# multimodallearning/convexAdam

Hardware: AMD Instinct MI355X
Metric: volume-pairs/sec (160x192x224 MIND convex+Adam(80it)) (higher is better)
Workload: dtype f32

## Files before the change

### convexadam_amd/csrc/certify.hip

```cpp
#include <hip/hip_runtime.h>
#include <stdlib.h>

#include "cvx_common.h"

namespace cvx {

#define CERT_CLO ((float)((1.0 - 1.0 / 65536.0) / 729.0))
#define CERT_CHI ((float)((1.0 + 1.0 / 65536.0) / 729.0))
#define CERT_TINY 1.0e-40f
__device__ __forceinline__ float cert_lower(float s) { return fmaxf(__builtin_fmaf(s, CERT_CLO, -CERT_TINY), 0.0f); }
__device__ __forceinline__ float cert_upper(float s) { return __builtin_fmaf(s, CERT_CHI, fminf(s, CERT_TINY)); }

__device__ __forceinline__ unsigned ordered_bits(float v) {
    unsigned b = __float_as_uint(v);
    b = (b & 0x80000000u) ? ~b : (b | 0x80000000u);
    if (v != v) b = 0u;
    return b;
}
__device__ __forceinline__ float from_ordered_bits(unsigned b) { return __uint_as_float((b & 0x80000000u) ? (b & 0x7fffffffu) : ~b); }

struct CertRec { unsigned x, box; int kp; float bound, slo, uc, ub, ua; };

struct CertProb {
    const float* ssdu; const float* fix; const float* mov; const float* tail;
    unsigned long long* key; unsigned* sec;
    int* idx0; int* idxA; int* idxB;
    float* smin;
    unsigned* list; int* counts;
    unsigned long long* work; unsigned work_cap;
    struct CertRec* rec;
    float* u;
    int64_t* argmin_out;
};
struct CertGeo { int C, h, w, d, hw, n, K, ntail; long long tail_from; };
struct CertArgs { CertProb p[2]; CertGeo g; const float* mesh; float coef; int pass; };

template <bool WAVE>
__device__ __forceinline__ void cert_sync() {
    if (WAVE) { __builtin_amdgcn_fence(__ATOMIC_RELEASE, "wavefront"); __builtin_amdgcn_s_waitcnt(0xC07F); __builtin_amdgcn_wave_barrier(); __builtin_amdgcn_fence(__ATOMIC_ACQUIRE, "wavefront"); }
    else __syncthreads();
}
template <bool WAVE>
__device__ float cert_exact_entry_t(const CertGeo& G, const CertProb& P, int k, int xlin, float* sm, int lane) {
    const int n = G.n, nn = n * n, h = G.h, w = G.w, d = G.d, hw = G.hw;
    const int iH = k % n, iW = (k / n) % n, iD = k / nn;
    const int x = xlin % d, y = (xlin / d) % w, z = xlin / (d * w);
    const size_t v = (size_t)h * w * d;
    for (int t = lane; t < 125; t += 64) {
        const int a = t / 25 - 2, b = (t / 5) % 5 - 2, c = t % 5 - 2;
        const int pz = z + a, py = y + b, px = x + c;
        float val = 0.0f;
        if (pz >= 0 && pz < h && py >= 0 && py < w && px >= 0 && px < d) {
            const long long flat = (((long long)pz * nn + iW * n + iD) * w + py) * d + px;
            if (G.ntail > 0 && flat >= G.tail_from) val = P.tail[iH * 32 + (int)(flat - G.tail_from)];
            else {
                const int mz = pz + iH - hw, my = py + iW - hw, mx = px + iD - hw;
                const bool inb = mz >= 0 && mz < h && my >= 0 && my < w && mx >= 0 && mx < d;
                const float* fp = P.fix + ((size_t)pz * w + py) * d + px;
                const float* mp = P.mov + ((size_t)(inb ? mz : 0) * w + (inb ? my : 0)) * d + (inb ? mx : 0);
                float a0 = 0.0f, a1 = 0.0f;
                for (int c0 = 0; c0 < G.C; c0 += 16) {
                    float fv[16], mv[16];
#pragma unroll
                    for (int i = 0; i < 16; ++i) {
                        const bool on = c0 + i < G.C;
                        fv[i] = on ? fp[(size_t)(c0 + i) * v] : 0.0f;
                        mv[i] = (on && inb) ? mp[(size_t)(c0 + i) * v] : 0.0f;
                    }
#pragma unroll
                    for (int i = 0; i < 16; ++i) {
                        if (c0 + i < G.C) {
                            const float df = fv[i] - mv[i];
                            a0 += df * df;
                        }
                    }
                    if (c0 + 16 <= G.C) { a1 += a0; a0 = 0.0f; }
                }
                val = G.C >= 16 ? a0 + a1 : a0;
            }
        }
        sm[t] = val;
    }
    cert_sync<WAVE>();
    if (lane < 27) {
        const int a = lane / 9 - 1, b = (lane / 3) % 3 - 1, c = lane % 3 - 1;
        const int pz = z + a, py = y + b, px = x + c;
        float s = 0.0f;
        const bool in = pz >= 0 && pz < h && py >= 0 && py < w && px >= 0 && px < d;
        if (in) {
            for (int aa = -1; aa <= 1; ++aa)
                for (int bb = -1; bb <= 1; ++bb)
                    for (int cc = -1; cc <= 1; ++cc) {
                        const int qz = pz + aa, qy = py + bb, qx = px + cc;
                        if (qz >= 0 && qz < h && qy >= 0 && qy < w && qx >= 0 && qx < d) s += sm[((a + aa + 2) * 5 + (b + bb + 2)) * 5 + (c + cc + 2)];
                    }
            s = div_exact<27>(s);
        }
        sm[128 + lane] = in ? s : -1.0f;
    }
    cert_sync<WAVE>();
    float s = 0.0f;
    for (int t = 0; t < 27; ++t) {
        const float b = sm[128 + t];
        if (b >= 0.0f || b != b) s += b;
    }
    cert_sync<WAVE>();
    return div_exact<27>(s);
}

__device__ float cert_exact_entry(const CertGeo& G, const CertProb& P, int k, int xlin, float* sm, int lane) { return cert_exact_entry_t<false>(G, P, k, xlin, sm, lane); }
__device__ float cert_exact_entry_wave(const CertGeo& G, const CertProb& P, int k, int xlin, float* sm, int lane) { return cert_exact_entry_t<true>(G, P, k, xlin, sm, lane); }

__global__ __launch_bounds__(256) void k_cert_plain_stream(CertArgs A, int kslice, int vec4) {
    const CertProb& P = A.p[blockIdx.z];
    const size_t v = (size_t)A.g.h * A.g.w * A.g.d;
    const int K = A.g.K;
    const size_t x0 = ((size_t)blockIdx.x * blockDim.x + threadIdx.x) * 4;
    const int k0 = blockIdx.y * kslice, k1 = min(k0 + kslice, K);
    if (x0 >= v) return;
    const int nv = (int)min((size_t)4, v - x0);
    const float INF = __uint_as_float(0x7f800000u);
    float best[4], second[4];
    int bi[4];
    bool tiny[4] = {false, false, false, false};
    const float* p = P.ssdu + (size_t)k0 * v + x0;
    auto load4 = [&](const float* q, float (&c4)[4]) {
        if (vec4) { const float4 t = *reinterpret_cast<const float4*>(q); c4[0] = t.x; c4[1] = t.y; c4[2] = t.z; c4[3] = t.w; }
        else {
#pragma unroll
            for (int j = 0; j < 4; ++j) c4[j] = j < nv ? q[j] : 0.0f;
        }
    };
    {
        float c4[4];
        load4(p, c4);
#pragma unroll
        for (int j = 0; j < 4; ++j) { best[j] = c4[j]; bi[j] = k0; second[j] = INF; tiny[j] = (c4[j] > 0.0f) & (c4[j] < 1.0e-36f); }
        p += v;
    }
#pragma unroll 8
    for (int k = k0 + 1; k < k1; ++k, p += v) {
        float c4[4];
        load4(p, c4);
#pragma unroll
        for (int j = 0; j < 4; ++j) {
            const float c = c4[j];
            tiny[j] = tiny[j] | ((c > 0.0f) & (c < 1.0e-36f));
            const bool lt = argmin_better(c, best[j]);
            second[j] = fminf(second[j], lt ? best[j] : c);
            best[j] = lt ? c : best[j];
            bi[j] = lt ? k : bi[j];
        }
    }
#pragma unroll
    for (int j = 0; j < 4; ++j) {
        if (j >= nv) continue;
        const unsigned long long mine = pack_min_key(best[j], (unsigned)bi[j]);
        const unsigned long long old = atomicMin(&P.key[x0 + j], mine);
        unsigned cand = second[j] == INF ? 0xffffffffu : ordered_bits(second[j]);
        if (old != ~0ull) {
            const unsigned loser = (unsigned)((old < mine ? mine : old) >> 32);
            cand = loser < cand ? loser : cand;
        }
        if (tiny[j]) cand = 0u;
        if (cand != 0xffffffffu) atomicMin(&P.sec[x0 + j], cand);
    }
}

__global__ __launch_bounds__(256) void k_cert_plain_finalize(CertArgs A) {
    const CertProb& P = A.p[blockIdx.y];
    const size_t v = (size_t)A.g.h * A.g.w * A.g.d;
    const size_t x = (size_t)blockIdx.x * blockDim.x + threadIdx.x;
    if (x >= v) return;
    const unsigned long long key = P.key[x];
    const unsigned b1 = (unsigned)(key >> 32), b2 = P.sec[x];
    const int k1 = (int)(unsigned)(key & 0xffffffffull);
    const float s1 = b1 == 0u ? __uint_as_float(0x7fc00000u) : from_ordered_bits(b1);
    P.smin[x] = s1;
    P.idx0[x] = k1;
    if (P.argmin_out) P.argmin_out[x] = k1;
    bool certain = b1 == 0u || b2 == 0xffffffffu;
    if (!certain && b2 != 0u) certain = s1 == 0.0f || cert_lower(from_ordered_bits(b2)) > cert_upper(s1);
    if (!certain) P.list[atomicAdd(&P.counts[0], 1)] = (unsigned)x;
}

__global__ __launch_bounds__(64) void k_cert_plain_resolve(CertArgs A) {
    __shared__ float sm[160];
    const CertProb& P = A.p[blockIdx.y];
    const size_t v = (size_t)A.g.h * A.g.w * A.g.d;
    const int K = A.g.K, lane = threadIdx.x;
    const int cnt = P.counts[0];
    for (int e = blockIdx.x; e < cnt; e += gridDim.x) {
        const unsigned x = P.list[e];
        const float* col = P.ssdu + x;
        const float U = cert_upper(P.smin[x]);
        unsigned long long bestkey = ~0ull;
        for (int kb = 0; kb < K; kb += 1024) {
            float s[16];
#pragma unroll
            for (int i = 0; i < 16; ++i) { const int k = kb + 64 * i + lane; s[i] = k < K ? col[(size_t)k * v] : __uint_as_float(0x7f800000u); }
#pragma unroll
            for (int i = 0; i < 16; ++i) {
                const unsigned long long mz = __ballot(s[i] == 0.0f);
                if (mz) {
                    const unsigned long long key = pack_min_key(0.0f, (unsigned)(kb + 64 * i + __ffsll((long long)mz) - 1));
                    bestkey = key < bestkey ? key : bestkey;
                }
                const bool mine = s[i] != 0.0f && cert_lower(s[i]) <= U;
                const unsigned long long m = __ballot(mine);
                if (m) {
                    const int nm = __popcll(m);
                    int base = 0;
                    if (lane == 0) base = atomicAdd(&P.counts[8], nm);
                    base = __shfl(base, 0);
                    const int slot = base + __popcll(m & ((1ull << lane) - 1ull));
                    if (mine && (unsigned)slot < P.work_cap) P.work[slot] = ((unsigned long long)x << 32) | (unsigned)(kb + 64 * i + lane);
                    unsigned long long rest = __ballot(mine && (unsigned)slot >= P.work_cap);
                    while (rest) {
                        const int l = __ffsll((long long)rest) - 1;
                        rest &= rest - 1;
                        const int kk = kb + 64 * i + l;
                        const float ex = cert_exact_entry(A.g, P, kk, (int)x, sm, lane);
                        const unsigned long long key = pack_min_key(ex, (unsigned)kk);
                        bestkey = key < bestkey ? key : bestkey;
                    }
                }
            }
        }
        if (lane == 0) P.key[x] = bestkey;
    }
}
__global__ __launch_bounds__(256) void k_cert_plain_eval(CertArgs A) {
    __shared__ float smem[4][160];
    const CertProb& P = A.p[blockIdx.y];
    const int lane = threadIdx.x & 63, wv = threadIdx.x >> 6;
    const int n = min(P.counts[8], (int)P.work_cap);
    for (int e = blockIdx.x * 4 + wv; e < n; e += gridDim.x * 4) {
        const unsigned long long it = P.work[e];
        const unsigned x = (unsigned)(it >> 32);
        const int kk = (int)(unsigned)(it & 0xffffffffull);
        const float ex = cert_exact_entry_wave(A.g, P, kk, (int)x, smem[wv], lane);
        if (lane == 0) atomicMin(&P.key[x], pack_min_key(ex, (unsigned)kk));
    }
}
__global__ __launch_bounds__(256) void k_cert_plain_commit(CertArgs A) {
    const CertProb& P = A.p[blockIdx.y];
    const int cnt = P.counts[0];
    for (int e = blockIdx.x * blockDim.x + threadIdx.x; e < cnt; e += gridDim.x * blockDim.x) {
        const unsigned x = P.list[e];
        const int kw = (int)(unsigned)(P.key[x] & 0xffffffffull);
        P.idx0[x] = kw;
        if (P.argmin_out) P.argmin_out[x] = kw;
    }
}

struct CertMesh {
    const float* ax;
    int n; float rn;
    __device__ __forceinline__ void split(int k, int& ic, int& ib, int& ia) const {
        const int q = (int)(((float)k + 0.5f) * rn);
        ic = k - q * n;
        ia = (int)(((float)q + 0.5f) * rn);
        ib = q - ia * n;
    }
};
__device__ __forceinline__ CertMesh cert_mesh_load(float* lds96, const float* __restrict__ mesh, int K, int n) {
    const int t = threadIdx.x;
    if (t < n) { lds96[t] = mesh[t]; lds96[32 + t] = mesh[K + t * n]; lds96[64 + t] = mesh[2 * K + t * n * n]; }
    __syncthreads();
    return CertMesh{lds96, n, 1.0f / (float)n};
}

__device__ __forceinline__ void cert_smooth_winner(const int* __restrict__ idx, const CertMesh& M, int h, int w, int d, size_t i,
                                                   float& o0, float& o1, float& o2) {
    const int x = (int)(i % d), y = (int)((i / d) % w), z = (int)(i / ((size_t)d * w));
    float s0 = 0.f, s1 = 0.f, s2 = 0.f;
#pragma unroll
    for (int a = -1; a <= 1; ++a) {
        const int za = z + a;
        const bool zok = za >= 0 && za < h;
        const int zc = zok ? za : z;
        int kk[9];
        bool ok[9];
#pragma unroll
        for (int b = -1; b <= 1; ++b)
#pragma unroll
            for (int c = -1; c <= 1; ++c) {
                const int yb = y + b, xc = x + c;
                const bool in = zok && yb >= 0 && yb < w && xc >= 0 && xc < d;
                const int t = (b + 1) * 3 + (c + 1);
                ok[t] = in;
                kk[t] = idx[((size_t)zc * w + (in ? yb : y)) * d + (in ? xc : x)];
            }
        float m0[9], m1[9], m2[9];
#pragma unroll
        for (int t = 0; t < 9; ++t) {
            int ic, ib, ia;
            M.split(kk[t], ic, ib, ia);
            m0[t] = M.ax[ic]; m1[t] = M.ax[32 + ib]; m2[t] = M.ax[64 + ia];
        }
#pragma unroll
        for (int t = 0; t < 9; ++t) {
            s0 += ok[t] ? m0[t] : 0.0f;
            s1 += ok[t] ? m1[t] : 0.0f;
            s2 += ok[t] ? m2[t] : 0.0f;
        }
    }
    o0 = fdiv(s0, 27.0f);
    o1 = fdiv(s1, 27.0f);
    o2 = fdiv(s2, 27.0f);
}

__device__ __forceinline__ float cert_pen(const CertMesh& M, int k, float uc, float ub, float ua, float coef) {
    int ic, ib, ia;
    M.split(k, ic, ib, ia);
    const float e0 = M.ax[ic] - uc, e1 = M.ax[32 + ib] - ub, e2 = M.ax[64 + ia] - ua;
    float q = e0 * e0;
    q += e1 * e1;
    q += e2 * e2;
    return coef * q;
}

struct CertBox {
    float uc, ub, ua, slo, bound;
    int c_lo, c_hi, b_lo, b_hi, a_lo, a_hi;
    long long vol;
    bool degenerate;
};
__device__ __forceinline__ CertBox cert_box(const CertMesh& M, float uc, float ub, float ua, float coef, int K, int n, int kp,
                                            float ssdu_kp, float smin_u, const float* __restrict__ col, size_t v, int refine_above) {
    CertBox c;
    c.uc = uc; c.ub = ub; c.ua = ua;
    c.slo = cert_lower(smin_u);
    c.bound = cert_upper(ssdu_kp) + cert_pen(M, kp, uc, ub, ua, coef);
    const float hwf = (float)((n - 1) / 2);
    auto close_box = [&]() {
        const float qmax = fdiv((c.bound - c.slo) + fabsf(c.bound) * 2.384185791015625e-07f, coef) * 1.00001f;
        const float R = fsqrt(fmaxf(qmax, 0.0f)) * 1.00001f + 1.0e-4f;
        c.c_lo = max((int)ceilf(c.uc - R + hwf), 0); c.c_hi = min((int)floorf(c.uc + R + hwf), n - 1);
        c.b_lo = max((int)ceilf(c.ub - R + hwf), 0); c.b_hi = min((int)floorf(c.ub + R + hwf), n - 1);
        c.a_lo = max((int)ceilf(c.ua - R + hwf), 0); c.a_hi = min((int)floorf(c.ua + R + hwf), n - 1);
        c.vol = (long long)max(c.c_hi - c.c_lo + 1, 0) * max(c.b_hi - c.b_lo + 1, 0) * max(c.a_hi - c.a_lo + 1, 0);
        c.degenerate = !(coef > 0.0f) || !(R == R) || c.vol <= 0;
    };
    close_box();
    if (!c.degenerate && c.vol > refine_above && uc == uc && ub == ub && ua == ua) {
        const int kn = (min(max((int)rintf(ua + hwf), 0), n - 1) * n + min(max((int)rintf(ub + hwf), 0), n - 1)) * n + min(max((int)rintf(uc + hwf), 0), n - 1);
        if (kn != kp) {
            const float near_hi = cert_upper(col[(size_t)kn * v]) + cert_pen(M, kn, uc, ub, ua, coef);
            if (near_hi < c.bound) { c.bound = near_hi; close_box(); }
        }
    }
    if (c.degenerate) { c.c_lo = c.b_lo = c.a_lo = 0; c.c_hi = c.b_hi = c.a_hi = n - 1; c.vol = (long long)n * n * n; }
    return c;
}

__global__ __launch_bounds__(64) void k_cert_voxel(CertArgs A, int refine) {
    const CertProb& P = A.p[blockIdx.y];
    const int h = A.g.h, w = A.g.w, d = A.g.d, K = A.g.K, n = A.g.n;
    const size_t v = (size_t)h * w * d;
    const size_t x = (size_t)blockIdx.x * blockDim.x + threadIdx.x;
    __shared__ float axes[96];
    const CertMesh M = cert_mesh_load(axes, A.mesh, K, n);
    if (x >= v) return;
    const int* prev = A.pass == 1 ? P.idx0 : ((A.pass & 1) ? P.idxB : P.idxA);
    int* next = (A.pass & 1) ? P.idxA : P.idxB;
    const int kp = prev[x];
    const float s_kp = P.ssdu[(size_t)kp * v + x];
    const float sm_x = P.smin[x];
    float uc, ub, ua;
    cert_smooth_winner(prev, M, h, w, d, x, uc, ub, ua);
    P.u[x] = uc; P.u[v + x] = ub; P.u[2 * v + x] = ua;
    if (sm_x != sm_x) { next[x] = P.idx0[x]; return; }
    const CertBox c = cert_box(M, uc, ub, ua, A.coef, K, n, kp, s_kp, sm_x, P.ssdu + x, v, refine);
    constexpr int NB = 8;
    const unsigned boxpack = (unsigned)c.c_lo | ((unsigned)c.c_hi << 5) | ((unsigned)c.b_lo << 10) | ((unsigned)c.b_hi << 15) | ((unsigned)c.a_lo << 20) | ((unsigned)c.a_hi << 25) | (c.degenerate ? 1u << 30 : 0u);
    const CertRec rec = {(unsigned)x, boxpack, kp, c.bound, c.slo, c.uc, c.ub, c.ua};
    if (c.vol > NB) { P.rec[atomicAdd(&P.counts[A.pass], 1)] = rec; return; }
    int kk[NB];
    float pen[NB], val[NB];
    bool need[NB];
    {
        int ic = c.c_lo, ib = c.b_lo, ia = c.a_lo;
#pragma unroll
        for (int j = 0; j < NB; ++j) {
            const bool in = j < (int)c.vol;
            kk[j] = (ia * n + ib) * n + ic;
            pen[j] = cert_pen(M, kk[j], c.uc, c.ub, c.ua, A.coef);
            need[j] = in && !(c.slo + pen[j] > c.bound);
            if (j + 1 < (int)c.vol) {
                if (++ic > c.c_hi) { ic = c.c_lo; if (++ib > c.b_hi) { ib = c.b_lo; ++ia; } }
            }
        }
    }
#pragma unroll
    for (int j = 0; j < NB; ++j) val[j] = need[j] ? P.ssdu[(size_t)kk[j] * v + x] : 0.0f;
    float lo1 = 0.f, lo2 = 0.f, U = __uint_as_float(0x7f800000u);
    int k1 = -1, cnt = 0;
#pragma unroll
    for (int j = 0; j < NB; ++j) {
        if (!need[j]) continue;
        const float lo = cert_lower(val[j]) + pen[j], hi = cert_upper(val[j]) + pen[j];
        U = fminf(U, hi);
        if (cnt == 0) { lo1 = lo; k1 = kk[j]; }
        else if (lo < lo1) { lo2 = lo1; lo1 = lo; k1 = kk[j]; }
        else if (cnt == 1 || lo < lo2) lo2 = lo;
        ++cnt;
    }
    if (cnt == 0) { next[x] = kp; return; }
    if (cnt == 1 || lo2 > U) { next[x] = k1; return; }
    P.rec[atomicAdd(&P.counts[A.pass], 1)] = rec;
}

__global__ __launch_bounds__(256) void k_cert_wave(CertArgs A) {
    __shared__ float smem[4][160];
    __shared__ float axes[96];
    const CertProb& P = A.p[blockIdx.y];
    const int h = A.g.h, w = A.g.w, d = A.g.d, K = A.g.K, n = A.g.n;
    const size_t v = (size_t)h * w * d;
    const int lane = threadIdx.x & 63, wv = threadIdx.x >> 6;
    float* sm = smem[wv];
    const CertMesh M = cert_mesh_load(axes, A.mesh, K, n);
    int* next = (A.pass & 1) ? P.idxA : P.idxB;
    const int cnt = P.counts[A.pass];
    const float INF = __uint_as_float(0x7f800000u);
    for (int e = blockIdx.x * 4 + wv; e < cnt; e += gridDim.x * 4) {
        const CertRec r = P.rec[e];
        const size_t x = r.x;
        const int kp = r.kp;
        const float* col = P.ssdu + x;
        CertBox c;
        c.uc = r.uc; c.ub = r.ub; c.ua = r.ua; c.slo = r.slo; c.bound = r.bound;
        c.c_lo = r.box & 31; c.c_hi = (r.box >> 5) & 31; c.b_lo = (r.box >> 10) & 31; c.b_hi = (r.box >> 15) & 31; c.a_lo = (r.box >> 20) & 31; c.a_hi = (r.box >> 25) & 31;
        c.degenerate = ((r.box >> 30) & 1u) != 0;
        c.vol = (long long)(c.c_hi - c.c_lo + 1) * (c.b_hi - c.b_lo + 1) * (c.a_hi - c.a_lo + 1);
        const int nc = c.c_hi - c.c_lo + 1, nb = c.b_hi - c.b_lo + 1, ncb = nc * nb;
        const float rc = 1.0f / (float)nc, rab = 1.0f / (float)ncb;
        unsigned long long key = ~0ull;
        float lo2 = INF, U = INF;
        constexpr int NL = 12;
        for (long long i0 = 0; i0 < c.vol; i0 += 64 * NL) {
            int kk[NL];
            float pen[NL], val[NL];
            bool need[NL];
#pragma unroll
            for (int j = 0; j < NL; ++j) {
                need[j] = false; kk[j] = 0; pen[j] = 0.0f;
                if (i0 + 64 * j < c.vol) {
                    const int i = (int)i0 + lane + 64 * j;
                    need[j] = i < (int)c.vol;
                    const int ii = need[j] ? i : 0;
                    const int qa = (int)(((float)ii + 0.5f) * rab), ra = ii - qa * ncb;
                    const int qb = (int)(((float)ra + 0.5f) * rc);
                    const int ic = c.c_lo + ra - qb * nc, ib = c.b_lo + qb, ia = c.a_lo + qa;
                    kk[j] = (ia * n + ib) * n + ic;
                    pen[j] = cert_pen(M, kk[j], c.uc, c.ub, c.ua, A.coef);
                    need[j] = need[j] && (c.degenerate || !(c.slo + pen[j] > c.bound));
                }
            }
#pragma unroll
            for (int j = 0; j < NL; ++j) val[j] = need[j] ? col[(size_t)kk[j] * v] : 0.0f;
#pragma unroll
            for (int j = 0; j < NL; ++j) {
                if (!need[j]) continue;
                const float lo = cert_lower(val[j]) + pen[j], hi = cert_upper(val[j]) + pen[j];
                U = fminf(U, hi);
                const unsigned long long kx = pack_min_key(lo, (unsigned)kk[j]);
                if (kx < key) { if (key != ~0ull) lo2 = fminf(lo2, from_ordered_bits((unsigned)(key >> 32))); key = kx; }
                else lo2 = fminf(lo2, lo);
            }
        }
        unsigned long long gkey = key;
        for (int o = 32; o > 0; o >>= 1) { const unsigned long long t = __shfl_xor(gkey, o); gkey = t < gkey ? t : gkey; }
        float mine2 = key == gkey ? lo2 : fminf(lo2, key != ~0ull ? from_ordered_bits((unsigned)(key >> 32)) : INF);
        for (int o = 32; o > 0; o >>= 1) { mine2 = fminf(mine2, __shfl_xor(mine2, o)); U = fminf(U, __shfl_xor(U, o)); }
        if (gkey == ~0ull) { if (lane == 0) next[x] = kp; continue; }
        if (mine2 > U) { if (lane == 0) next[x] = (int)(unsigned)(gkey & 0xffffffffull); continue; }
        if (lane == 0) atomicAdd(&P.counts[7], 1);
        unsigned long long bestkey = ~0ull;
        for (long long i0 = 0; i0 < c.vol; i0 += 64 * NL) {
            int kk[NL];
            float pen[NL], val[NL];
            bool need[NL];
#pragma unroll
            for (int j = 0; j < NL; ++j) {
                need[j] = false; kk[j] = 0; pen[j] = 0.0f;
                if (i0 + 64 * j < c.vol) {
                    const int i = (int)i0 + lane + 64 * j;
                    need[j] = i < (int)c.vol;
                    const int ii = need[j] ? i : 0;
                    const int qa = (int)(((float)ii + 0.5f) * rab), ra = ii - qa * ncb;
                    const int qb = (int)(((float)ra + 0.5f) * rc);
                    kk[j] = ((c.a_lo + qa) * n + c.b_lo + qb) * n + c.c_lo + ra - qb * nc;
                    pen[j] = cert_pen(M, kk[j], c.uc, c.ub, c.ua, A.coef);
                    need[j] = need[j] && (c.degenerate || !(c.slo + pen[j] > c.bound));
                }
            }
#pragma unroll
            for (int j = 0; j < NL; ++j) val[j] = need[j] ? col[(size_t)kk[j] * v] : 0.0f;
#pragma unroll
            for (int j = 0; j < NL; ++j) {
                if (!(i0 + 64 * j < c.vol)) continue;
                unsigned long long m = __ballot(need[j] && cert_lower(val[j]) + pen[j] <= U);
                while (m) {
                    const int l = __ffsll((long long)m) - 1;
                    m &= m - 1;
                    const int k2 = __shfl(kk[j], l);
                    const float sk = __shfl(val[j], l), pk = __shfl(pen[j], l);
                    const float ex = sk == 0.0f ? 0.0f : cert_exact_entry_wave(A.g, P, k2, (int)x, sm, lane);
                    const unsigned long long kx = pack_min_key(ex + pk, (unsigned)k2);
                    bestkey = kx < bestkey ? kx : bestkey;
                }
            }
        }
        if (lane == 0) next[x] = (int)(unsigned)(bestkey & 0xffffffffull);
    }
}

__global__ __launch_bounds__(256) void k_cert_gather(CertArgs A) {
    const CertProb& P = A.p[blockIdx.y];
    const size_t v = (size_t)A.g.h * A.g.w * A.g.d;
    const size_t i = (size_t)blockIdx.x * blockDim.x + threadIdx.x;
    __shared__ float axes[96];
    const CertMesh M = cert_mesh_load(axes, A.mesh, A.g.K, A.g.n);
    if (i >= v) return;
    const int* prev = A.pass == 1 ? P.idx0 : ((A.pass & 1) ? P.idxB : P.idxA);
    float o0, o1, o2;
    cert_smooth_winner(prev, M, A.g.h, A.g.w, A.g.d, i, o0, o1, o2);
    P.u[i] = o0; P.u[v + i] = o1; P.u[2 * v + i] = o2;
}

__global__ __launch_bounds__(256) void k_cert_arm(CertArgs A, int nprob) {
    const size_t v = (size_t)A.g.h * A.g.w * A.g.d;
    const size_t i = (size_t)blockIdx.x * blockDim.x + threadIdx.x;
    for (int q = 0; q < nprob; ++q) {
        if (i < v) { A.p[q].key[i] = ~0ull; A.p[q].sec[i] = 0xffffffffu; }
        if (i < 16) A.p[q].counts[i] = 0;
    }
}

void launch_corr_tail_compact(const float* fix, const float* mov, int C, int h, int w, int d, int hw, int sad, float* tail, hipStream_t s);

static size_t cert_work_cap(size_t v) { return 4 * v + 65536; }
struct CertCarve { unsigned long long* key; unsigned* sec; int* idx0; int* idxA; int* idxB; float* smin; unsigned* list; CertRec* rec; int* counts; float* tail; unsigned long long* work; unsigned work_cap; };
static CertCarve cert_layout(Carver& cv, int h, int w, int d, int hw, bool plain) {
    const size_t v = (size_t)h * w * d;
    const int n = 2 * hw + 1;
    CertCarve c{};
    c.key = cv.take<unsigned long long>(v);
    c.sec = cv.take<unsigned>(v);
    c.idx0 = cv.take<int>(v);
    c.smin = cv.take<float>(v);
    c.list = cv.take<unsigned>(v);
    c.counts = cv.take<int>(16);
    c.work_cap = (unsigned)cert_work_cap(v);
    c.work = cv.take<unsigned long long>(c.work_cap);
    c.tail = cv.take<float>((size_t)32 * n);
    if (!plain) {
        c.idxA = cv.take<int>(v); c.idxB = cv.take<int>(v);
        c.rec = cv.take<CertRec>(v);
    }
    return c;
}
size_t corr_certify_workspace_bytes(int, int h, int w, int d, int hw, bool plain) { Carver m; cert_layout(m, h, w, d, hw, plain); return ws_query(m); }
static CertGeo cert_geo(int C, int h, int w, int d, int hw) {
    CertGeo g;
    g.C = C; g.h = h; g.w = w; g.d = d; g.hw = hw; g.n = 2 * hw + 1; g.K = g.n * g.n * g.n;
    const long long ncols = (long long)h * g.n * g.n * w * d;
    g.tail_from = (ncols / 32) * 32;
    g.ntail = (int)(ncols - g.tail_from);
    return g;
}
static CertProb cert_prob(const float* ssdu, const float* fix, const float* mov, const CertCarve& c, float* u, int64_t* argmin_out) {
    return CertProb{ssdu, fix, mov, c.tail, c.key, c.sec, c.idx0, c.idxA, c.idxB, c.smin, c.list, c.counts, c.work, c.work_cap, c.rec, u, argmin_out};
}

static void cert_arm(CertArgs& A, int nprob, hipStream_t s) {
    const CertGeo& g = A.g;
    const size_t v = (size_t)g.h * g.w * g.d;
    hipLaunchKernelGGL(k_cert_arm, dim3((unsigned)cdiv64((int64_t)(v > 16 ? v : 16), 256)), dim3(256), 0, s, A, nprob);
    for (int q = 0; q < nprob; ++q)
        if (g.ntail > 0) launch_corr_tail_compact(A.p[q].fix, A.p[q].mov, g.C, g.h, g.w, g.d, g.hw, 0, const_cast<float*>(A.p[q].tail), s);
}
static void cert_stream(CertArgs A, int q0, int nq, hipStream_t s) {
    const CertGeo& g = A.g;
    const size_t v = (size_t)g.h * g.w * g.d;
    const int K = g.K;
    if (q0) { A.p[0] = A.p[q0]; }
    bool vec4 = v % 4 == 0;
    for (int q = 0; q < nq; ++q) vec4 = vec4 && (reinterpret_cast<uintptr_t>(A.p[q].ssdu) & 15) == 0;
    const int xb = (int)cdiv64((int64_t)cdiv64((int64_t)v, 4), 256);
    int nslices = cdiv(512, xb);
    if (nslices > K) nslices = K;
    if (nslices < 1) nslices = 1;
    const int kslice = cdiv(K, nslices);
    nslices = cdiv(K, kslice);
    hipLaunchKernelGGL(k_cert_plain_stream, dim3(xb, nslices, nq), dim3(256), 0, s, A, kslice, vec4 ? 1 : 0);
}
static int cert_finish(CertArgs& A, int nprob, hipStream_t s) {
    const size_t v = (size_t)A.g.h * A.g.w * A.g.d;
    hipLaunchKernelGGL(k_cert_plain_finalize, dim3((unsigned)cdiv64((int64_t)v, 256), nprob), dim3(256), 0, s, A);
    hipLaunchKernelGGL(k_cert_plain_resolve, dim3(256, nprob), dim3(64), 0, s, A);
    hipLaunchKernelGGL(k_cert_plain_eval, dim3(256, nprob), dim3(256), 0, s, A);
    hipLaunchKernelGGL(k_cert_plain_commit, dim3(8, nprob), dim3(256), 0, s, A);
    return check_last("certified argmin");
}
static int cert_plain(CertArgs& A, int nprob, bool arm, hipStream_t s) {
    if (arm) cert_arm(A, nprob, s);
    cert_stream(A, 0, nprob, s);
    return cert_finish(A, nprob, s);
}

int corr_certified_argmin(const float* ssdu, const float* fix, const float* mov, int C, int h, int w, int d, int hw, int64_t* argmin,
                          void* workspace, size_t workspace_bytes, hipStream_t s) {
    if (workspace_bytes < corr_certify_workspace_bytes(C, h, w, d, hw, true)) return fail(CVX_ERR_WORKSPACE, "certified argmin: workspace too small");
    Carver cv(workspace);
    const CertCarve c = cert_layout(cv, h, w, d, hw, true);
    CertArgs A{};
    A.g = cert_geo(C, h, w, d, hw);
    A.p[0] = cert_prob(ssdu, fix, mov, c, nullptr, argmin);
    A.p[1] = A.p[0];
    return cert_plain(A, 1, true, s);
}

int coupled_convex_cert_impl(const float* ssduA, const float* fixA, const float* movA, float* outA, void* wsA, const float* ssduB, const float* fixB,
                             const float* movB, float* outB, void* wsB, const float* mesh, int C, int h, int w, int d, int hw, size_t workspace_bytes,
                             hipStream_t s, int stage) {
    if (workspace_bytes < corr_certify_workspace_bytes(C, h, w, d, hw, false)) return fail(CVX_ERR_WORKSPACE, "certified coupled convex: workspace too small");
    const int nprob = ssduB ? 2 : 1;
    CertArgs A{};
    A.g = cert_geo(C, h, w, d, hw);
    A.mesh = mesh;
    Carver cva(wsA), cvb(wsB);
    const CertCarve ca = cert_layout(cva, h, w, d, hw, false);
    A.p[0] = cert_prob(ssduA, fixA, movA, ca, outA, nullptr);
    A.p[1] = A.p[0];
    if (ssduB) { const CertCarve cb = cert_layout(cvb, h, w, d, hw, false); A.p[1] = cert_prob(ssduB, fixB, movB, cb, outB, nullptr); }
    if (stage == 1) { cert_arm(A, nprob, s); return check_last("certified argmin"); }
    if (stage == 2) { cert_stream(A, 0, 1, s); return check_last("certified argmin"); }
    if (stage == 3) { if (nprob > 1) cert_stream(A, 1, 1, s); return check_last("certified argmin"); }
    if (stage == 4) return cert_finish(A, nprob, s);
    if (stage == 0) { const int rc = cert_plain(A, nprob, true, s); if (rc) return rc; }
    const size_t v = (size_t)h * w * d;
    const int refine = options().prune_refine != 0 ? 8 : 0x7fffffff;
    static const float coeffs[6] = {0.003f, 0.01f, 0.03f, 0.1f, 0.3f, 1.0f};
    for (int it = 0; it < 6; ++it) {
        A.coef = coeffs[it]; A.pass = it + 1;
        hipLaunchKernelGGL(k_cert_voxel, dim3((unsigned)cdiv64((int64_t)v, 64), nprob), dim3(64), 0, s, A, refine);
        hipLaunchKernelGGL(k_cert_wave, dim3(512, nprob), dim3(256), 0, s, A);
    }
    if (getenv("CVX_CERT_TRACE")) {
        for (int q = 0; q < nprob; ++q) {
            int cnt[8];
            (void)hipStreamSynchronize(s);
            (void)hipMemcpy(cnt, A.p[q].counts, sizeof(cnt), hipMemcpyDeviceToHost);
            fprintf(stderr, "cert trace: problem %d: plain flagged %d; listed per coupled pass %d %d %d %d %d %d, %d of them evaluated exactly (of %zu voxels)\n", q, cnt[0], cnt[1], cnt[2], cnt[3], cnt[4], cnt[5], cnt[6], cnt[7], v);
        }
    }
    A.pass = 7;
    hipLaunchKernelGGL(k_cert_gather, dim3((unsigned)cdiv64((int64_t)v, 256), nprob), dim3(256), 0, s, A);
    return check_last("certified coupled convex");
}

}
```

### convexadam_amd/csrc/correlate.hip

```cpp

#include <algorithm>

#include "cvx_common.h"

namespace cvx {

struct CorrGeom {
    int C, h, w, d, hw, n;
    int px;
    int PL;
    int dq;
    int hq, wq;
    int mpad;
};
static CorrGeom corr_geom(int C, int h, int w, int d, int hw) {
    CorrGeom g;
    g.C = C; g.h = h; g.w = w; g.d = d; g.hw = hw; g.n = 2 * hw + 1;
    g.px = (d + 3 + 3) / 4 * 4;
    g.PL = (hw + 3) / 4 * 4;
    g.dq = g.px + 2 * g.PL;
    g.hq = h + 2 * hw; g.wq = w + 2 * hw;
    g.mpad = 0;
    return g;
}

__global__ __launch_bounds__(256) void k_corr_prep(const float* __restrict__ fix, const float* __restrict__ mov, CorrGeom g,
                                                   float* __restrict__ Fp, float* __restrict__ Mp) {
    const size_t nF = (size_t)g.C * g.h * g.w * g.px, nM = (size_t)g.C * g.hq * g.wq * g.dq;
    const size_t i = (size_t)blockIdx.x * blockDim.x + threadIdx.x;
    if (i < nF) {
        const int x = (int)(i % g.px) - 1;
        const size_t r = i / g.px;
        Fp[i] = (x >= 0 && x < g.d) ? fix[r * g.d + x] : 0.0f;
    }
    if (i < nM) {
        const int xq = (int)(i % g.dq), yq = (int)((i / g.dq) % g.wq), zq = (int)((i / ((size_t)g.dq * g.wq)) % g.hq);
        const int c = (int)(i / ((size_t)g.dq * g.wq * g.hq));
        const int x = xq - g.PL - 1, y = yq - g.hw, z = zq - g.hw;
        const bool in = x >= 0 && x < g.d && y >= 0 && y < g.w && z >= 0 && z < g.h;
        Mp[i] = in ? mov[(((size_t)c * g.h + z) * g.w + y) * g.d + x] : 0.0f;
    } else if (i < nM + (size_t)g.mpad) Mp[i] = 0.0f;
}

template <int HW, bool CASCADE, bool FAST = false>
__global__ __launch_bounds__(256) void k_corr_raw(const float* __restrict__ Fp, const float* __restrict__ Mp, CorrGeom g,
                                                  float* __restrict__ raw) {
    static_assert(!(CASCADE && FAST), "the fast arithmetic has no cascade");
    constexpr int N = 2 * HW + 1;
    constexpr int PL = (HW + 3) / 4 * 4;
    constexpr int NCH = (2 * PL + 4) / 4;
    const int runs_per_row = g.px / 4;
    const int nruns = g.h * g.w * runs_per_row;
    const int r = blockIdx.x * blockDim.x + threadIdx.x;
    if (r >= nruns) return;
    const int i0 = 4 * (r % runs_per_row), y = (r / runs_per_row) % g.w, z = r / (runs_per_row * g.w);
    const int iH = blockIdx.y % N, iW = blockIdx.y / N;

    float acc[N][4];
    float acc1[CASCADE ? N : 1][4];
#pragma unroll
    for (int k = 0; k < N; ++k)
#pragma unroll
        for (int j = 0; j < 4; ++j) acc[k][j] = 0.0f;
    if (CASCADE) {
#pragma unroll
        for (int k = 0; k < N; ++k)
#pragma unroll
            for (int j = 0; j < 4; ++j) acc1[k][j] = 0.0f;
    }
    const size_t fstride = (size_t)g.h * g.w * g.px, mstride = (size_t)g.hq * g.wq * g.dq;
    const float* fp = Fp + ((size_t)z * g.w + y) * g.px + i0;
    const float* mp = Mp + ((size_t)(z + iH) * g.wq + (y + iW)) * g.dq + i0;

    float4 fq[2];
    float4 mq[2][NCH];
    fq[0] = *reinterpret_cast<const float4*>(fp);
#pragma unroll
    for (int q = 0; q < NCH; ++q) mq[0][q] = *reinterpret_cast<const float4*>(mp + 4 * q);
    auto consume = [&](const float4& f4, const float4 (&mv)[NCH], int c) {
        const float f[4] = {f4.x, f4.y, f4.z, f4.w};
        float m[4 * NCH];
#pragma unroll
        for (int q = 0; q < NCH; ++q) { m[4 * q] = mv[q].x; m[4 * q + 1] = mv[q].y; m[4 * q + 2] = mv[q].z; m[4 * q + 3] = mv[q].w; }
#pragma unroll
        for (int k = 0; k < N; ++k)
#pragma unroll
            for (int j = 0; j < 4; ++j) {
                const float df = f[j] - m[PL + j + k - HW];
                if (FAST) acc[k][j] = __builtin_fmaf(df, df, acc[k][j]);
                else acc[k][j] += df * df;
            }
        if (CASCADE && ((c & 15) == 15)) {
#pragma unroll
            for (int k = 0; k < N; ++k)
#pragma unroll
                for (int j = 0; j < 4; ++j) { acc1[k][j] += acc[k][j]; acc[k][j] = 0.0f; }
        }
    };
#pragma unroll 1
    for (int c = 0; c < g.C; c += 2) {
        if (c + 1 < g.C) {
            fq[1] = *reinterpret_cast<const float4*>(fp + (size_t)(c + 1) * fstride);
#pragma unroll
            for (int q = 0; q < NCH; ++q) mq[1][q] = *reinterpret_cast<const float4*>(mp + (size_t)(c + 1) * mstride + 4 * q);
        }
        consume(fq[0], mq[0], c);
        if (c + 1 < g.C) {
            if (c + 2 < g.C) {
                fq[0] = *reinterpret_cast<const float4*>(fp + (size_t)(c + 2) * fstride);
#pragma unroll
                for (int q = 0; q < NCH; ++q) mq[0][q] = *reinterpret_cast<const float4*>(mp + (size_t)(c + 2) * mstride + 4 * q);
            }
            consume(fq[1], mq[1], c + 1);
        }
    }
    const size_t v = (size_t)g.h * g.w * g.px;
    bool inx[4];
#pragma unroll
    for (int j = 0; j < 4; ++j) inx[j] = (i0 + j >= 1) && (i0 + j <= g.d);
#pragma unroll
    for (int k = 0; k < N; ++k) {
        float o[4];
#pragma unroll
        for (int j = 0; j < 4; ++j) {
            const float s = CASCADE ? acc[k][j] + acc1[k][j] : acc[k][j];
            o[j] = inx[j] ? s : 0.0f;
        }
        const size_t kk = ((size_t)k * N + iW) * N + iH;
        *reinterpret_cast<float4*>(raw + kk * v + ((size_t)z * g.w + y) * g.px + i0) = make_float4(o[0], o[1], o[2], o[3]);
    }
}

__device__ float sum_cascade_strided(const float* v, int stride, int size) {
    float a0 = 0.f, a1 = 0.f;
    int i = 0;
    for (; i + 16 <= size; i += 16) {
        for (int j = 0; j < 16; ++j) a0 += v[(i + j) * stride];
        a1 += a0; a0 = 0.f;
    }
    for (; i < size; ++i) a0 += v[i * stride];
    return a0 + a1;
}
__global__ void k_corr_tail(const float* __restrict__ fix, const float* __restrict__ mov, CorrGeom g, int64_t tail_from,
                            int ntail, float* __restrict__ raw) {
    const int t = blockIdx.x * blockDim.x + threadIdx.x;
    if (t >= ntail * g.n) return;
    const int iH = t / ntail;
    const int64_t flat = tail_from + (t % ntail);
    const int x = (int)(flat % g.d), y = (int)((flat / g.d) % g.w);
    const int jj = (int)((flat / ((int64_t)g.d * g.w)) % (g.n * g.n)), z = (int)(flat / ((int64_t)g.d * g.w * g.n * g.n));
    const int iW = jj / g.n, iD = jj % g.n;
    const int mz = z + iH - g.hw, my = y + iW - g.hw, mx = x + iD - g.hw;
    const bool inb = mz >= 0 && mz < g.h && my >= 0 && my < g.w && mx >= 0 && mx < g.d;
    const size_t v = (size_t)g.h * g.w * g.d;
    float sq[256];
    for (int c = 0; c < g.C; ++c) {
        const float f = fix[(size_t)c * v + ((size_t)z * g.w + y) * g.d + x];
        const float m = inb ? mov[(size_t)c * v + ((size_t)mz * g.w + my) * g.d + mx] : 0.0f;
        const float df = f - m;
        sq[c] = df * df;
    }
    const int n4 = g.C / 4;
    float p[4];
    for (int k = 0; k < 4; ++k) p[k] = sum_cascade_strided(sq + k, 4, n4);
    for (int i = n4 * 4; i < g.C; ++i) p[0] += sq[i];
    p[0] += p[1]; p[0] += p[2]; p[0] += p[3];
    const size_t kk = ((size_t)iD * g.n + iW) * g.n + iH;
    raw[kk * ((size_t)g.h * g.w * g.px) + ((size_t)z * g.w + y) * g.px + x + 1] = p[0];
}

__global__ void k_corr_tail_compact(const float* __restrict__ fix, const float* __restrict__ mov, CorrGeom g, int64_t tail_from,
                                    int ntail, int sad, float* __restrict__ tail) {
    const int t = blockIdx.x * blockDim.x + threadIdx.x;
    if (t >= ntail * g.n) return;
    const int iH = t / ntail;
    const int64_t flat = tail_from + (t % ntail);
    const int x = (int)(flat % g.d), y = (int)((flat / g.d) % g.w);
    const int jj = (int)((flat / ((int64_t)g.d * g.w)) % (g.n * g.n)), z = (int)(flat / ((int64_t)g.d * g.w * g.n * g.n));
    const int iW = jj / g.n, iD = jj % g.n;
    const int mz = z + iH - g.hw, my = y + iW - g.hw, mx = x + iD - g.hw;
    const bool inb = mz >= 0 && mz < g.h && my >= 0 && my < g.w && mx >= 0 && mx < g.d;
    const size_t v = (size_t)g.h * g.w * g.d;
    float sq[256];
    for (int c = 0; c < g.C; ++c) {
        const float f = fix[(size_t)c * v + ((size_t)z * g.w + y) * g.d + x];
        const float m = inb ? mov[(size_t)c * v + ((size_t)mz * g.w + my) * g.d + mx] : 0.0f;
        const float df = f - m;
        sq[c] = sad ? fabsf(df) : df * df;
    }
    const int n4 = g.C / 4;
    float p[4];
    for (int k = 0; k < 4; ++k) p[k] = sum_cascade_strided(sq + k, 4, n4);
    for (int i = n4 * 4; i < g.C; ++i) p[0] += sq[i];
    p[0] += p[1]; p[0] += p[2]; p[0] += p[3];
    tail[iH * 32 + (t % ntail)] = p[0];
}

void launch_corr_prep_generic(const float* fix, const float* mov, int C, int h, int w, int d, int hw, int px, int PL, int dq, float* Fp,
                              float* Mp, hipStream_t s) {
    CorrGeom g = corr_geom(C, h, w, d, hw);
    g.px = px; g.PL = PL; g.dq = dq; g.mpad = 8;
    const size_t nprep = std::max((size_t)C * g.hq * g.wq * g.dq + g.mpad, (size_t)C * h * w * g.px);
    hipLaunchKernelGGL(k_corr_prep, dim3((unsigned)cdiv64((int64_t)nprep, 256)), dim3(256), 0, s, fix, mov, g, Fp, Mp);
}

void launch_corr_tail_compact(const float* fix, const float* mov, int C, int h, int w, int d, int hw, int sad, float* tail, hipStream_t s) {
    const CorrGeom g = corr_geom(C, h, w, d, hw);
    const int64_t ncols = (int64_t)h * g.n * g.n * w * d, tail_from = (ncols / 32) * 32;
    const int ntail = (int)(ncols - tail_from);
    if (ntail > 0) hipLaunchKernelGGL(k_corr_tail_compact, dim3(cdiv(ntail * g.n, 64)), dim3(64), 0, s, fix, mov, g, tail_from, ntail, sad, tail);
}

template <int HW>
static void corr_raw_dispatch(const float* Fp, const float* Mp, const CorrGeom& g, float* raw, hipStream_t s, bool fast = false) {
    const int nruns = g.h * g.w * (g.px / 4);
    const dim3 grid(cdiv(nruns, 256), g.n * g.n);
    if (fast) hipLaunchKernelGGL((k_corr_raw<HW, false, true>), grid, dim3(256), 0, s, Fp, Mp, g, raw);
    else if (g.C >= 16) hipLaunchKernelGGL((k_corr_raw<HW, true>), grid, dim3(256), 0, s, Fp, Mp, g, raw);
    else hipLaunchKernelGGL((k_corr_raw<HW, false>), grid, dim3(256), 0, s, Fp, Mp, g, raw);
}

CorrPlan corr_plan(int C, int h, int w, int d, int hw, CorrUse use) {
    const Options& o = options();
    const CorrGeom g = corr_geom(C, h, w, d, hw);
    const double K = (double)g.n * g.n * g.n;
    const bool fused_ok = corr_fused_supported(C, h, w, d, hw), staged_ok = corr_cert_supported(C, h, w, d, hw);
    const bool round1_fits = hw <= 8 && corr_box2_supported(h, w, d, g.px) && (size_t)g.n * g.n * g.n * h * w * g.px * sizeof(float) <= ((size_t)2 << 30);
    const bool role_good = fused_ok && C <= 32 && corr_fused_items(C, h, w, d, hw) >= 384 && !corr_fused_tiled(C, h, w, d, hw);
    const bool role_ok = fused_ok && C <= 128;
    const bool unfused_ok = C >= 16 && C <= 128 && round1_fits && o.corr_cert != 2 && o.cert_unfused != 0 && (K * h * w * d * C >= 1e9 || o.cert_unfused == 2);

    CorrPlan p{};
    p.exact = (!fused_ok || (!use.variant && o.corr_fused_all == 0 && C >= 16 && round1_fits)) ? CorrKernel::Round1 : CorrKernel::Fused;
    p.cert = unfused_ok && !role_good                            ? CorrKernel::CertRound1
             : staged_ok && (o.corr_cert == 2 || !role_ok)       ? CorrKernel::CertStaged
             : role_ok                                           ? CorrKernel::CertRole
                                                                 : CorrKernel::None;
    p.cert_supported = staged_ok || role_ok || unfused_ok;
    p.fused_ws = fused_ok; p.staged_ws = staged_ok; p.cert_round1_ws = unfused_ok;
    p.pair_cert = o.corr_cert != 0 && !use.variant && !use.no_prune && p.cert_supported &&
                  (o.corr_cert == 2 || C < 16 || p.cert == CorrKernel::CertRound1 || role_good);
    p.pair_dual = use.ic && o.corr_dual != 0 && p.exact == CorrKernel::Fused;
    p.pair_dual_ws = use.ic && o.corr_dual != 0 && fused_ok;
    return p;
}

struct Round1Ws { float *Fp, *Mp, *raw; unsigned long long* keys; };
static Round1Ws round1_layout(Carver& cv, int C, int h, int w, int d, int hw, bool keys) {
    const CorrGeom g = corr_geom(C, h, w, d, hw);
    Round1Ws r{};
    r.Fp = cv.take<float>((size_t)C * h * w * g.px);
    r.Mp = cv.take<float>((size_t)C * g.hq * g.wq * g.dq);
    r.raw = cv.take<float>((size_t)g.n * g.n * g.n * h * w * g.px);
    if (keys) r.keys = cv.take<unsigned long long>((size_t)h * w * d);
    return r;
}
static int launch_round1(const float* fix, const float* mov, const CorrGeom& g, const Round1Ws& r, bool fast, float* ssd, hipStream_t s) {
    const size_t nprep = (size_t)g.C * g.hq * g.wq * g.dq;
    hipLaunchKernelGGL(k_corr_prep, dim3((unsigned)cdiv64((int64_t)nprep, 256)), dim3(256), 0, s, fix, mov, g, r.Fp, r.Mp);
    if (fast) corr_call_prep_hook(s);
    switch (g.hw) {
        case 0: corr_raw_dispatch<0>(r.Fp, r.Mp, g, r.raw, s, fast); break;
        case 1: corr_raw_dispatch<1>(r.Fp, r.Mp, g, r.raw, s, fast); break;
        case 2: corr_raw_dispatch<2>(r.Fp, r.Mp, g, r.raw, s, fast); break;
        case 3: corr_raw_dispatch<3>(r.Fp, r.Mp, g, r.raw, s, fast); break;
        case 4: corr_raw_dispatch<4>(r.Fp, r.Mp, g, r.raw, s, fast); break;
        case 5: corr_raw_dispatch<5>(r.Fp, r.Mp, g, r.raw, s, fast); break;
        case 6: corr_raw_dispatch<6>(r.Fp, r.Mp, g, r.raw, s, fast); break;
        case 7: corr_raw_dispatch<7>(r.Fp, r.Mp, g, r.raw, s, fast); break;
        default: corr_raw_dispatch<8>(r.Fp, r.Mp, g, r.raw, s, fast); break;
    }
    const int64_t ncols = (int64_t)g.h * g.n * g.n * g.w * g.d, tail_from = (ncols / 32) * 32;
    const int ntail = (int)(ncols - tail_from);
    if (!fast && ntail > 0)
        hipLaunchKernelGGL(k_corr_tail, dim3(cdiv(ntail * g.n, 64)), dim3(64), 0, s, fix, mov, g, tail_from, ntail, r.raw);
    return launch_corr_box2(r.raw, g.n * g.n * g.n, g.h, g.w, g.d, g.px, ssd, s, fast);
}

size_t corr_certfast_workspace_bytes(int C, int h, int w, int d, int hw) {
    const CorrPlan p = corr_plan(C, h, w, d, hw);
    Carver round1;
    if (p.cert_round1_ws) round1_layout(round1, C, h, w, d, hw, false);
    return std::max({p.staged_ws ? corr_cert_workspace_bytes(C, h, w, d, hw) : 0, p.fused_ws ? corr_fused_workspace_bytes(C, h, w, d, hw) : 0, ws_query(round1)});
}
int launch_corr_certfast(const float* fix, const float* mov, int C, int h, int w, int d, int hw, float* ssdu, void* workspace, size_t workspace_bytes,
                         hipStream_t s) {
    switch (corr_plan(C, h, w, d, hw).cert) {
        case CorrKernel::CertRound1: {
            Carver cv(workspace);
            const Round1Ws r = round1_layout(cv, C, h, w, d, hw, false);
            if (workspace_bytes < ws_query(cv)) return fail(CVX_ERR_WORKSPACE, "correlate (certified-fast, two kernels): workspace too small");
            return launch_round1(fix, mov, corr_geom(C, h, w, d, hw), r, true, ssdu, s);
        }
        case CorrKernel::CertStaged: return launch_corr_cert(fix, mov, C, h, w, d, hw, ssdu, workspace, workspace_bytes, s);
        default:
            return launch_corr_fused(fix, mov, C, h, w, d, hw, 0, 2, 2, 0, ssdu, workspace, workspace_bytes, s);
    }
}

}

using namespace cvx;

struct PartsWs { void* a; size_t a_bytes; void* b; size_t b_bytes; };
static PartsWs parts_layout(Carver& cv, size_t a_bytes, size_t b_bytes) {
    PartsWs p{nullptr, a_bytes, nullptr, b_bytes};
    p.a = cv.take<char>(a_bytes);
    p.b = cv.take<char>(b_bytes);
    return p;
}
static PartsWs fused_keys_layout(Carver& cv, int C, int h, int w, int d, int hw) {
    return parts_layout(cv, corr_fused_workspace_bytes(C, h, w, d, hw), sizeof(unsigned long long) * (size_t)h * w * d);
}
static PartsWs certified_layout(Carver& cv, int C, int h, int w, int d, int hw) {
    return parts_layout(cv, corr_certfast_workspace_bytes(C, h, w, d, hw), corr_certify_workspace_bytes(C, h, w, d, hw, true));
}
extern "C" size_t cvx_correlate_workspace_bytes(int C, int h, int w, int d, int disp_hw) {
    const CorrPlan p = corr_plan(C, h, w, d, disp_hw);
    Carver fused, round1, cert;
    if (p.fused_ws) fused_keys_layout(fused, C, h, w, d, disp_hw);
    if (p.exact == CorrKernel::Round1) round1_layout(round1, C, h, w, d, disp_hw, true);
    if (p.cert_supported) certified_layout(cert, C, h, w, d, disp_hw);
    return std::max({ws_query(fused), ws_query(round1), ws_query(cert)});
}

extern "C" int cvx_correlate_f32(const float* fix, const float* mov, int C, int h, int w, int d, int disp_hw, float* ssd,
                                 int64_t* argmin, void* workspace, size_t workspace_bytes, void* stream) {
    return cvx_correlate_ex_f32(fix, mov, C, h, w, d, disp_hw, nullptr, ssd, argmin, workspace, workspace_bytes, stream);
}

extern "C" int cvx_correlate_ex_f32(const float* fix, const float* mov, int C, int h, int w, int d, int disp_hw, const cvx_corr_opts* opts,
                                    float* ssd, int64_t* argmin, void* workspace, size_t workspace_bytes, void* stream) {
    const int cost = opts ? opts->cost : 0, n_box = opts ? opts->n_box : 2, fast = opts ? opts->fast : 0, f16 = opts ? opts->f16 : 0;
    CVX_REQUIRE((cost == 0 || cost == 1) && (n_box == 1 || n_box == 2) && (fast == 0 || fast == 1 || fast == 2) && f16 >= 0 && f16 <= 2, "cvx_correlate_ex_f32: bad options");
    CVX_REQUIRE(!(f16 && (cost != 0 || n_box != 2)), "cvx_correlate_ex_f32: fp16 storage exists for the SSD cost with two boxes only");
    CVX_REQUIRE(!(fast && (cost != 0 || n_box != 2)), "cvx_correlate_ex_f32: the fast mode exists for the SSD cost with two boxes only");
    CVX_REQUIRE(fix && mov && ssd && workspace, "cvx_correlate_f32: null pointer");
    CVX_REQUIRE(C > 0 && C < 256 && h > 0 && w > 0 && d > 0, "cvx_correlate_f32: bad extent C=%d %dx%dx%d", C, h, w, d);
    CVX_REQUIRE(disp_hw >= 0, "cvx_correlate_f32: negative disp_hw");
    if (disp_hw > CVX_MAX_DISP_HW) return fail(CVX_ERR_UNSUPPORTED, "cvx_correlate_f32: disp_hw %d > %d not built", disp_hw, CVX_MAX_DISP_HW);
    if (workspace_bytes < cvx_correlate_workspace_bytes(C, h, w, d, disp_hw))
        return fail(CVX_ERR_WORKSPACE, "cvx_correlate_f32: workspace too small");
    hipStream_t s = as_stream(stream);
    const CorrGeom g = corr_geom(C, h, w, d, disp_hw);
    const size_t K = (size_t)g.n * g.n * g.n;
    const bool variant = cost != 0 || n_box != 2 || fast || f16;
    const CorrPlan plan = corr_plan(C, h, w, d, disp_hw, CorrUse{variant, false, false});
    Carver cv(workspace);
    if (fast == 2) {
        if (f16) return fail(CVX_ERR_UNSUPPORTED, "cvx_correlate_ex_f32: the certified-fast volume is float32");
        if (!plan.cert_supported) return fail(CVX_ERR_UNSUPPORTED, "cvx_correlate_ex_f32: certified-fast correlation not built for this geometry");
        const PartsWs c = certified_layout(cv, C, h, w, d, disp_hw);
        int rc = launch_corr_certfast(fix, mov, C, h, w, d, disp_hw, ssd, c.a, c.a_bytes, s);
        if (rc || !argmin) return rc;
        return corr_certified_argmin(ssd, fix, mov, C, h, w, d, disp_hw, argmin, c.b, c.b_bytes, s);
    }
    if (plan.exact == CorrKernel::Fused) {
        const PartsWs f = fused_keys_layout(cv, C, h, w, d, disp_hw);
        int rc = launch_corr_fused(fix, mov, C, h, w, d, disp_hw, cost, n_box, fast, f16, ssd, f.a, f.a_bytes, s);
        if (rc) return rc;
        if (argmin)
            return launch_argmin(ssd, f16 == 2, nullptr, nullptr, 0.0f, false, (int)K, (size_t)h * w * d, static_cast<unsigned long long*>(f.b), argmin, s);
        return CVX_OK;
    }
    if (variant)
        return fail(CVX_ERR_UNSUPPORTED, "cvx_correlate_ex_f32: cost / n_box / fast / fp16 variants need the fused kernel (option corr_unfused is set, or the grid is outside its range: the fused kernel covers rows of d <= ~1270 voxels when the plane has w <= 320 / ceil((d + 6) / 4) rows, else (y tiles) d <= ~250)");
    if (disp_hw > 8) return fail(CVX_ERR_UNSUPPORTED, "cvx_correlate_f32: disp_hw %d > 8 needs the fused kernel (option corr_unfused is set, or the grid is outside its range: the fused kernel covers rows of d <= ~1270 voxels when the plane has w <= 320 / ceil((d + 6) / 4) rows, else (y tiles) d <= ~250)", disp_hw);
    if (!corr_box2_supported(h, w, d, g.px))
        return fail(CVX_ERR_UNSUPPORTED, "cvx_correlate_f32: coarse rows of %d voxels are too long for the LDS box kernel", d);
    const Round1Ws r = round1_layout(cv, C, h, w, d, disp_hw, true);
    int rc = launch_round1(fix, mov, g, r, false, ssd, s);
    if (rc) return rc;
    if (argmin) return launch_argmin(ssd, false, nullptr, nullptr, 0.0f, false, (int)K, (size_t)h * w * d, r.keys, argmin, s);
    return CVX_OK;
}
```

### convexadam_amd/csrc/cvx_common.h

```cpp
#pragma once
#include <hip/hip_runtime.h>
#include <stdint.h>
#include <stdio.h>
#include <stdarg.h>

#include <mutex>

#include "convexadam_hip.h"

namespace cvx {

void set_error(const char* fmt, ...);
int fail(int code, const char* fmt, ...);
int check_last(const char* what);

#define CVX_REQUIRE(cond, ...)                                      \
    do {                                                            \
        if (!(cond)) return ::cvx::fail(CVX_ERR_INVALID_ARG, __VA_ARGS__); \
    } while (0)

static inline hipStream_t as_stream(void* s) { return reinterpret_cast<hipStream_t>(s); }
static inline size_t align_up(size_t v, size_t a) { return (v + a - 1) / a * a; }
static inline int cdiv(int a, int b) { return (a + b - 1) / b; }
static inline int64_t cdiv64(int64_t a, int64_t b) { return (a + b - 1) / b; }

template <typename KernelT>
static inline void ensure_dynamic_lds(KernelT kernel, size_t bytes, size_t& granted) {
    static std::mutex mu;
    std::lock_guard<std::mutex> lock(mu);
    if (bytes > granted) {
        (void)hipFuncSetAttribute(reinterpret_cast<const void*>(kernel), hipFuncAttributeMaxDynamicSharedMemorySize, (int)bytes);
        (void)hipGetLastError();
        granted = bytes;
    }
}

struct Carver {
    char* base = nullptr;
    size_t used = 0;
    Carver() = default;
    explicit Carver(void* p) : base(static_cast<char*>(p)) {}
    size_t take_bytes(size_t bytes) { const size_t off = align_up(used, 256); used = off + bytes; return off; }
    template <typename T> T* take(size_t count) { const size_t off = take_bytes(count * sizeof(T)); return base ? reinterpret_cast<T*>(base + off) : nullptr; }
};
static inline size_t ws_query(const Carver& m) { return m.used ? m.used + 256 : 0; }

#define CVX_OPTIONS(X) \
    X(mind_tiled,          "CVX_MIND_TILED",            0)   \
    X(mind_overlap,        "CVX_MIND_OVERLAP",          0)   \
    X(mm_tx,               "CVX_MM_TX",                 0)   \
    X(mm_slots,            "CVX_MM_SLOTS",            512)   \
    X(box_tiled,           "CVX_BOX_TILED",             0)   \
    X(no_prune,            "CVX_NO_PRUNE",              0)   \
    X(corr_unfused,        "CVX_CORR_UNFUSED",          0)   \
    X(corr_fused_all,      "CVX_CORR_FUSED_ALL",        0)   \
    X(prune_stream_above,  "CVX_PRUNE_STREAM_ABOVE",   -1)   \
    X(cf_census,           "CVX_CF_CENSUS",             0)   \
    X(cf_prio,             "CVX_CF_PRIO",             136)   \
    X(warp_flat,           "CVX_WARP_FLAT",             0)   \
    X(box_yt,              "CVX_BOX_YT",                8)   \
    X(box_wg_target,       "CVX_BOX_WG_TARGET",         0)   \
    X(box_xsplit,          "CVX_BOX_XSPLIT",           -1)   \
    X(box_cpt,             "CVX_BOX_CPT",               4)   \
    X(box_uneven,          "CVX_BOX_UNEVEN",          200)   \
    X(box_adam_role,       "CVX_BOX_ADAM_ROLE",         0)   \
    X(box_dpp,             "CVX_BOX_DPP",               0)   \
    X(box_pk,              "CVX_BOX_PK",                0)   \
    X(box_prio,            "CVX_BOX_PRIO",              0)   \
    X(label_pow_block,     "CVX_LABEL_POW_BLOCK",      32)   \
    X(census_ptr,          nullptr,                     0)   \
    X(mind_mean_threads,   "CVX_MIND_MEAN_THREADS",     0)   \
    X(edt_sequential,      "CVX_EDT_SEQUENTIAL",        0)   \
    X(warp_octant,         "CVX_WARP_OCTANT",           4)   \
    X(box_fwd_tile,        "CVX_BOX_FWD_TILE",         -1)   \
    X(box_bwd_tile,        "CVX_BOX_BWD_TILE",         -1)   \
    X(box_walk,            "CVX_BOX_WALK",              1)   \
    X(corr_dual,           "CVX_CORR_DUAL",             0)   \
    X(prune_refine,        "CVX_PRUNE_REFINE",          1)   \
    X(mind_records,        "CVX_MIND_RECORDS",          1)   \
    X(resize_up2,          "CVX_RESIZE_UP2",            1)   \
    X(mind_blocked,        "CVX_MIND_BLOCKED",          1)   \
    X(corr_cert,           "CVX_CORR_CERT",             1)   \
    X(cc_debug,            "CVX_CC_DEBUG",              0)   \
    X(ic_fused,            "CVX_IC_FUSED",              0)   \
    X(mind_single,         "CVX_MIND_SINGLE",           0)   \
    X(ms_zlen,             "CVX_MS_ZLEN",               0)   \
    X(cf_map,              "CVX_CF_MAP",                1)   \
    X(cert_unfused,        "CVX_CERT_UNFUSED",          0)   \
    X(fbox_tile,           "CVX_FBOX_TILE",             0)   \
    X(box_tile_sync,       "CVX_BOX_TILE_SYNC",         0)   \
    X(box_prediv,          "CVX_BOX_PREDIV",            1)   \
    X(tile_census_ptr,     nullptr,                     0)   \
    X(adam_wt,             "CVX_ADAM_WT",               1)
#define X(name, env, dflt) long long name;
struct Options { CVX_OPTIONS(X) };
#undef X
Options& options();
const unsigned* adam_sqrt_table();
class ContextScope {
public:
    explicit ContextScope(const cvx_context* c);
    ~ContextScope();
    ContextScope(const ContextScope&) = delete;
    ContextScope& operator=(const ContextScope&) = delete;
private:
    void* prev_;
    bool active_;
};

#ifdef CVX_RACE_JITTER
__device__ __forceinline__ void cvx_jitter() {
    unsigned t = (unsigned)__builtin_amdgcn_s_memtime();
    t ^= (unsigned)__builtin_amdgcn_s_getreg((4 << 0) | (0 << 6) | (31 << 11)) * 2654435761u;
    t ^= t >> 13; t *= 0x9E3779B1u; t ^= t >> 15;
    const int n = (int)(t & 15);
    for (int i = 0; i < n; ++i) __builtin_amdgcn_s_sleep(1);
}
__device__ __forceinline__ void cvx_barrier() { cvx_jitter(); __syncthreads(); cvx_jitter(); }
#else
__device__ __forceinline__ void cvx_barrier() { __syncthreads(); }
#endif

__device__ __forceinline__ int clampi(int v, int lo, int hi) { return v < lo ? lo : (v > hi ? hi : v); }

__device__ __forceinline__ float fdiv(float a, float b) { return __fdiv_rn(a, b); }
__device__ __forceinline__ float fsqrt(float a) { return sqrtf(a); }

__device__ __forceinline__ float cvx_expf(float d) {
    const float R_LN2f = 1.442695040888963407359924681001892137426645954152985934135449406931f;
    const float L2Uf = 0.693145751953125f, L2Lf = 1.428606765330187045e-06f;
    const float qf = rintf(d * R_LN2f);
    const int q = (int)qf;
    float s = __builtin_fmaf(qf, -L2Uf, d);
    s = __builtin_fmaf(qf, -L2Lf, s);
    float u = 0.000198527617612853646278381f;
    u = __builtin_fmaf(u, s, 0.00139304355252534151077271f);
    u = __builtin_fmaf(u, s, 0.00833336077630519866943359f);
    u = __builtin_fmaf(u, s, 0.0416664853692054748535156f);
    u = __builtin_fmaf(u, s, 0.166666671633720397949219f);
    u = __builtin_fmaf(u, s, 0.5f);
    u = 1.0f + __builtin_fmaf(s * s, u, s);
    u = __builtin_ldexpf(u, q);
    if (d < -104.0f) u = 0.0f;
    if (d > 100.0f) u = __int_as_float(0x7f800000);
    return u;
}

struct ExpTable { const unsigned char* tbl; unsigned first, count; };
ExpTable mind_exp_table();

typedef float f32x4 __attribute__((ext_vector_type(4)));
typedef __attribute__((address_space(3))) f32x4 lds_f32x4;
__device__ __forceinline__ f32x4 lds_load4(const float* p) { return *(const volatile lds_f32x4*)p; }
__device__ __forceinline__ void lds_store4(float* p, f32x4 v) { *(volatile lds_f32x4*)p = v; }

typedef int i32x4 __attribute__((ext_vector_type(4)));
typedef unsigned u32x4 __attribute__((ext_vector_type(4)));
__device__ __forceinline__ float4 buffer_load16(__amdgpu_buffer_rsrc_t rsrc, unsigned lane_off, unsigned uni_off) {
    const i32x4 v = __builtin_bit_cast(i32x4, __builtin_amdgcn_raw_buffer_load_b128(rsrc, (int)lane_off, (int)uni_off, 0));
    return make_float4(__int_as_float(v.x), __int_as_float(v.y), __int_as_float(v.z), __int_as_float(v.w));
}

template <bool WT>
__device__ __forceinline__ void buffer_store16(__amdgpu_buffer_rsrc_t rsrc, unsigned lane_off, unsigned uni_off, float4 v) {
    __builtin_amdgcn_raw_buffer_store_b128(__builtin_bit_cast(u32x4, v), rsrc, (int)lane_off, (int)uni_off, WT ? 16 : 0);
}
template <bool WT>
__device__ __forceinline__ void buffer_store4(__amdgpu_buffer_rsrc_t rsrc, unsigned lane_off, unsigned uni_off, float v) {
    __builtin_amdgcn_raw_buffer_store_b32(__float_as_uint(v), rsrc, (int)lane_off, (int)uni_off, WT ? 16 : 0);
}
__device__ __forceinline__ void global_store16_wt(float* p, float4 v) {
    asm volatile("global_store_dwordx4 %0, %1, off sc1\n\ts_nop 1" : : "v"(p), "v"(__builtin_bit_cast(f32x4, v)) : "memory");
}

typedef float f32x2 __attribute__((ext_vector_type(2)));
typedef __attribute__((address_space(3))) f32x2 lds_f32x2;
__device__ __forceinline__ f32x2 lds_load2(const float* p) { return *(const volatile lds_f32x2*)p; }
__device__ __forceinline__ void lds_store2(float* p, f32x2 v) { *(volatile lds_f32x2*)p = v; }

template <int D>
__device__ __forceinline__ float div_exact(float x) {
    static_assert(D == 8 || D == 27 || D == 64 || D == 125 || D == 343, "divisor not verified");
    constexpr float r = 1.0f / (float)D;
    const float q = x * r;
    const float e = __builtin_fmaf(-(float)D, q, x);
    return __builtin_fmaf(e, r, q);
}
template <int D>
__device__ __forceinline__ float div_exact_inf(float x) { return __builtin_isinf(x) ? x : div_exact<D>(x); }

struct ConstDiv { float d, r; int ok; };
constexpr float kConstDivLo = 0x1p-76f, kConstDivHi = 0x1p76f;
ConstDiv const_div_ieee(float d);
ConstDiv const_div_make(float d);
ConstDiv const_div(float d);
ConstDiv const_div_if_proven(float d);
bool const_div_enumerate(float d, float r);
void const_div_prove(const float* ds, int n, int budget);
__device__ __forceinline__ float div_const_seq(float x, const ConstDiv& cd) {
    const float q = x * cd.r;
    const float e = __builtin_fmaf(-cd.d, q, x);
    return __builtin_fmaf(e, cd.r, q);
}
__device__ __forceinline__ bool div_const_inside(float x) { const float a = __builtin_fabsf(x); return a >= kConstDivLo && a <= kConstDivHi; }
__device__ __forceinline__ bool div_const_inside_root(float x) { return x <= kConstDivHi; }
__device__ __forceinline__ bool wave_all(bool inside) { return __builtin_amdgcn_ballot_w64(!inside) == 0; }
__device__ __forceinline__ float div_const(float x, const ConstDiv& cd) {
    if (cd.ok && wave_all(div_const_inside(x))) return div_const_seq(x, cd);
    return fdiv(x, cd.d);
}

template <int N>
__device__ __forceinline__ float cascade_seq(const float (&v)[N]) {
    static_assert(N < 256, "two cascade levels");
    float a0 = 0.f, a1 = 0.f;
    int i = 0;
#pragma unroll
    for (; i + 16 <= N; i += 16) {
#pragma unroll
        for (int j = 0; j < 16; ++j) a0 += v[i + j];
        a1 += a0;
        a0 = 0.f;
    }
#pragma unroll
    for (; i < N; ++i) a0 += v[i];
    a0 += a1;
    return a0;
}
template <int N>
__device__ __forceinline__ float outer_sum_ilp(const float (&v)[N]) {
    static_assert(N / 4 < 16, "single cascade level inside the interleaved sums");
    float p[4] = {0.f, 0.f, 0.f, 0.f};
#pragma unroll
    for (int i = 0; i < N / 4; ++i)
#pragma unroll
        for (int k = 0; k < 4; ++k) p[k] += v[4 * i + k];
#pragma unroll
    for (int i = (N / 4) * 4; i < N; ++i) p[0] += v[i];
    p[0] += p[1];
    p[0] += p[2];
    p[0] += p[3];
    return p[0];
}

__device__ __forceinline__ unsigned long long pack_min_key(float v, unsigned idx) {
    unsigned b = __float_as_uint(v);
    b = (b & 0x80000000u) ? ~b : (b | 0x80000000u);
    if (v != v) b = 0u;
    return ((unsigned long long)b << 32) | idx;
}

struct Tri {
    float ix, iy, iz;
    int x0, y0, z0;
    float tnw, tne, tsw, tse, bnw, bne, bsw, bse;
};
__device__ __forceinline__ float unnormalize(float g, int S) { return ((g + 1.0f) * (float)S - 1.0f) * 0.5f; }
__device__ __forceinline__ void tri_setup(Tri& t, float gx, float gy, float gz, int h, int w, int d) {
    t.ix = unnormalize(gx, d);
    t.iy = unnormalize(gy, w);
    t.iz = unnormalize(gz, h);
    const float fx = floorf(t.ix), fy = floorf(t.iy), fz = floorf(t.iz);
    t.x0 = (int)fmaxf(fminf(fx, 1.0e9f), -1.0e9f);
    t.y0 = (int)fmaxf(fminf(fy, 1.0e9f), -1.0e9f);
    t.z0 = (int)fmaxf(fminf(fz, 1.0e9f), -1.0e9f);
    const float x1 = (float)(t.x0 + 1), y1 = (float)(t.y0 + 1), z1 = (float)(t.z0 + 1);
    const float x0f = (float)t.x0, y0f = (float)t.y0, z0f = (float)t.z0;
    t.tnw = (x1 - t.ix) * (y1 - t.iy) * (z1 - t.iz);
    t.tne = (t.ix - x0f) * (y1 - t.iy) * (z1 - t.iz);
    t.tsw = (x1 - t.ix) * (t.iy - y0f) * (z1 - t.iz);
    t.tse = (t.ix - x0f) * (t.iy - y0f) * (z1 - t.iz);
    t.bnw = (x1 - t.ix) * (y1 - t.iy) * (t.iz - z0f);
    t.bne = (t.ix - x0f) * (y1 - t.iy) * (t.iz - z0f);
    t.bsw = (x1 - t.ix) * (t.iy - y0f) * (t.iz - z0f);
    t.bse = (t.ix - x0f) * (t.iy - y0f) * (t.iz - z0f);
}
__device__ __forceinline__ bool inb3(int z, int y, int x, int h, int w, int d) {
    return z >= 0 && z < h && y >= 0 && y < w && x >= 0 && x < d;
}
__device__ __forceinline__ float tri_sample(const Tri& t, const float* __restrict__ vol, int h, int w, int d) {
    const int x0 = t.x0, y0 = t.y0, z0 = t.z0, x1 = x0 + 1, y1 = y0 + 1, z1 = z0 + 1;
    const bool zi0 = (unsigned)z0 < (unsigned)h, zi1 = (unsigned)z1 < (unsigned)h, yi0 = (unsigned)y0 < (unsigned)w,
               yi1 = (unsigned)y1 < (unsigned)w, xi0 = (unsigned)x0 < (unsigned)d, xi1 = (unsigned)x1 < (unsigned)d;
    const int zc0 = clampi(z0, 0, h - 1), zc1 = clampi(z1, 0, h - 1), yc0 = clampi(y0, 0, w - 1), yc1 = clampi(y1, 0, w - 1),
              xc0 = clampi(x0, 0, d - 1), xc1 = clampi(x1, 0, d - 1);
    const size_t r00 = ((size_t)zc0 * w + yc0) * d, r01 = ((size_t)zc0 * w + yc1) * d, r10 = ((size_t)zc1 * w + yc0) * d,
                 r11 = ((size_t)zc1 * w + yc1) * d;
    const float v0 = vol[r00 + xc0], v1 = vol[r00 + xc1], v2 = vol[r01 + xc0], v3 = vol[r01 + xc1], v4 = vol[r10 + xc0],
                v5 = vol[r10 + xc1], v6 = vol[r11 + xc0], v7 = vol[r11 + xc1];
    float o = 0.0f, n;
    n = o + v0 * t.tnw; o = (zi0 && yi0 && xi0) ? n : o;
    n = o + v1 * t.tne; o = (zi0 && yi0 && xi1) ? n : o;
    n = o + v2 * t.tsw; o = (zi0 && yi1 && xi0) ? n : o;
    n = o + v3 * t.tse; o = (zi0 && yi1 && xi1) ? n : o;
    n = o + v4 * t.bnw; o = (zi1 && yi0 && xi0) ? n : o;
    n = o + v5 * t.bne; o = (zi1 && yi0 && xi1) ? n : o;
    n = o + v6 * t.bsw; o = (zi1 && yi1 && xi0) ? n : o;
    n = o + v7 * t.bse; o = (zi1 && yi1 && xi1) ? n : o;
    return o;
}

__device__ __forceinline__ void lin_coef(int o, int in, int out, int& i0, int& i1, float& l0, float& l1) {
    if (in == out) { i0 = o; i1 = o; l0 = 1.0f; l1 = 0.0f; return; }
    const float ratio = fdiv((float)in, (float)out);
    float src = __builtin_fmaf(ratio, (float)o + 0.5f, -0.5f);
    src = src < 0.0f ? 0.0f : src;
    int a = (int)floorf(src);
    a = a > in - 1 ? in - 1 : a;
    float l = src - (float)a;
    l = l < 0.f ? 0.f : (l > 1.f ? 1.f : l);
    i0 = a;
    i1 = a + ((a < in - 1) ? 1 : 0);
    l1 = l;
    l0 = 1.0f - l;
}
__device__ __forceinline__ float resize_chain(const float (&v)[8], float pre_mul, float lx0, float lx1, float ly0, float ly1, float lz0,
                                              float lz1) {
    const float a0 = __builtin_fmaf(v[0] * pre_mul, lx0, (v[1] * pre_mul) * lx1);
    const float a1 = __builtin_fmaf(v[2] * pre_mul, lx0, (v[3] * pre_mul) * lx1);
    const float b0 = __builtin_fmaf(v[4] * pre_mul, lx0, (v[5] * pre_mul) * lx1);
    const float b1 = __builtin_fmaf(v[6] * pre_mul, lx0, (v[7] * pre_mul) * lx1);
    const float l0 = __builtin_fmaf(a0, ly0, a1 * ly1);
    const float l1 = __builtin_fmaf(b0, ly0, b1 * ly1);
    return __builtin_fmaf(l0, lz0, l1 * lz1);
}

struct FastDiv { unsigned d, m; };
static inline FastDiv fastdiv_make(int d) { FastDiv f; f.d = (unsigned)d; f.m = d <= 1 ? 0u : (unsigned)((((unsigned long long)1 << 32) + (unsigned)d - 1) / (unsigned)d); return f; }
__device__ __forceinline__ int fastdiv(int n, FastDiv f) { return f.d <= 1 ? n : (int)__umulhi((unsigned)n, f.m); }

void profile_mark_kernel(const char* name, hipStream_t s);

int launch_box_zero(const float* in, float* out, int C, int H, int W, int D, int k, bool backward, hipStream_t s);
int launch_smoother(const float* in, float* out, float* tmp, int C, int H, int W, int D, const cvx_smoother& sm, bool backward,
                    hipStream_t s);
int launch_argmin_keys(const void* ssd, bool f16, int K, size_t v, unsigned long long* keys, bool arm, hipStream_t s);
struct CoupledWs { unsigned long long* keys[3]; int* idx; float* smin; unsigned long long* list; int* counts; };
CoupledWs coupled_layout(Carver& cv, int h, int w, int d, int disp_hw);
int launch_argmin(const void* ssd, bool f16, const float* mesh, const float* u, float coef, bool coupled, int K, size_t v,
                  unsigned long long* keys, int64_t* argmin_out, hipStream_t s);
int launch_resize(const float* in, int C, int h, int w, int d, float* out, int H, int W, int D, float pre_mul,
                  float post_div, hipStream_t s);
int launch_resize2(const float* in, int C, int h, int w, int d, int H, int W, int D, float* scratch, float* out, int h2, int w2,
                   int d2, float post_div, hipStream_t s);
struct AdamConsts { float w1, b2, omb2; ConstDiv bc2s; float neg_step; const unsigned* sqrt_tbl; };
__device__ __forceinline__ float adam_sqrt(float x, const unsigned* __restrict__ tbl) {
    float r = fsqrt(x);
    if (tbl) {
        const unsigned b = __float_as_uint(x), e = b >> 23, mant = b & 0x7fffffu;
        if (b != 0 && e < 255) {
            const unsigned key = e ? (((e & 1u) << 23) | mant) : ((1u << 24) | mant);
            const unsigned code = (tbl[key >> 4] >> ((key & 15u) * 2u)) & 3u;
            if (code) r = __uint_as_float(__float_as_uint(r) + (code == 1u ? 1u : 0xffffffffu));
        }
    }
    return r;
}
__device__ __forceinline__ bool argmin_better(float cost, float best) { return (cost < best) | ((cost != cost) & (best == best)); }
template <int N>
__device__ __forceinline__ void adam_update_n(const float (&g)[N], float (&P)[N], float (&m)[N], float (&v)[N], const AdamConsts& ac) {
    float root[N];
    bool inside = true;
#pragma unroll
    for (int j = 0; j < N; ++j) {
        m[j] = __builtin_fmaf(ac.w1, g[j] - m[j], m[j]);
        float vv = v[j] * ac.b2;
        vv = __builtin_fmaf(ac.omb2 * g[j], g[j], vv);
        v[j] = vv;
        root[j] = adam_sqrt(vv, ac.sqrt_tbl);
        inside &= div_const_inside_root(root[j]);
    }
    if (ac.bc2s.ok && wave_all(inside)) {
#pragma unroll
        for (int j = 0; j < N; ++j) root[j] = div_const_seq(root[j], ac.bc2s);
    } else {
#pragma unroll
        for (int j = 0; j < N; ++j) root[j] = fdiv(root[j], ac.bc2s.d);
    }
#pragma unroll
    for (int j = 0; j < N; ++j) {
        const float den = root[j] + 1e-8f;
        P[j] = P[j] + fdiv(ac.neg_step * m[j], den);
    }
}
__device__ __forceinline__ void adam_update(float g, float& P, float& m, float& v, const AdamConsts& ac) {
    const float g1[1] = {g};
    float P1[1] = {P}, m1[1] = {m}, v1[1] = {v};
    adam_update_n<1>(g1, P1, m1, v1, ac);
    P = P1[0]; m = m1[0]; v = v1[0];
}
struct AdamRun {
    const float *F2, *M2; int C, h, w, d; float *P, *m, *v; float lambda_weight; int niter, step0; float cost_scale;
    const float *base_h, *base_w, *base_d; float *U, *grad_out; const int* snapshot_iters_host; int n_snap; float* snapshots;
    void* workspace; size_t workspace_bytes; void* stream;
    const cvx_smoother* sm = nullptr;
    bool keep_state = true;
    bool f16_features = false;
    int fast = 0;
    bool features_are_records = false;
    bool ieee_div = false;
};
int adam_run_impl(const AdamRun& r);
size_t adam_record_floats(int C, size_t V);
int coupled_convex_impl(const void* ssd, bool f16, const int64_t* argmin, const float* mesh, int h, int w, int d, int disp_hw, float* out,
                        bool argmin_is_exact, void* workspace, size_t workspace_bytes, void* stream,
                        const unsigned char* cmask = nullptr);
int coupled_convex_dual_impl(const void* ssdA, const int64_t* argminA, float* outA, void* wsA, const void* ssdB, bool f16, const int64_t* argminB,
                             float* outB, void* wsB, const float* mesh, int h, int w, int d, int disp_hw, size_t workspace_bytes,
                             void* stream, bool counts_zeroed = false);
int launch_label_pooled(const float* lab, int H, int W, int D, int C, const int* present, const float* weights, float mult, int g1, float* out1,
                        int g2, float* out2, hipStream_t s);
bool corr_box2_supported(int h, int w, int d, int px);
int launch_corr_box2(const float* raw, int K, int h, int w, int d, int px, float* ssd, hipStream_t s, bool fast = false);
bool corr_fused_supported(int C, int h, int w, int d, int hw);
void corr_fused_set_prep_hook(void (*hook)(hipStream_t));
int corr_fused_items(int C, int h, int w, int d, int hw);
bool corr_fused_tiled(int C, int h, int w, int d, int hw);
void corr_call_prep_hook(hipStream_t s);
size_t corr_fused_workspace_bytes(int C, int h, int w, int d, int hw);
int launch_corr_fused(const float* fix, const float* mov, int C, int h, int w, int d, int hw, int cost, int n_box, int fast, int f16,
                      void* ssd, void* workspace, size_t workspace_bytes, hipStream_t s);
int launch_corr_fused_dual(const float* fix, const float* mov, int C, int h, int w, int d, int hw, int cost, int n_box, int fast, int f16,
                           void* ssd, void* ssd_rev, void* workspace, size_t workspace_bytes, void* workspace_rev, hipStream_t s);
bool corr_cert_supported(int C, int h, int w, int d, int hw);
size_t corr_cert_workspace_bytes(int C, int h, int w, int d, int hw);
int launch_corr_cert(const float* fix, const float* mov, int C, int h, int w, int d, int hw, float* ssdu, void* workspace, size_t workspace_bytes,
                     hipStream_t s);
enum class CorrKernel { None, Fused, Round1, CertRole, CertStaged, CertRound1 };
struct CorrUse { bool variant, ic, no_prune; };
struct CorrPlan {
    CorrKernel exact;
    CorrKernel cert;
    bool cert_supported;
    bool fused_ws, staged_ws, cert_round1_ws;
    bool pair_cert;
    bool pair_dual, pair_dual_ws;
};
CorrPlan corr_plan(int C, int h, int w, int d, int hw, CorrUse use = CorrUse{false, false, false});
size_t corr_certfast_workspace_bytes(int C, int h, int w, int d, int hw);
int launch_corr_certfast(const float* fix, const float* mov, int C, int h, int w, int d, int hw, float* ssdu, void* workspace, size_t workspace_bytes,
                         hipStream_t s);
size_t corr_certify_workspace_bytes(int C, int h, int w, int d, int hw, bool plain = false);
int corr_certified_argmin(const float* ssdu, const float* fix, const float* mov, int C, int h, int w, int d, int hw, int64_t* argmin,
                          void* workspace, size_t workspace_bytes, hipStream_t s);
int coupled_convex_cert_impl(const float* ssduA, const float* fixA, const float* movA, float* outA, void* wsA, const float* ssduB, const float* fixB,
                             const float* movB, float* outB, void* wsB, const float* mesh, int C, int h, int w, int d, int hw, size_t workspace_bytes,
                             hipStream_t s, int stage = 0);
bool box3_march_supported(int d);
int launch_box3_march(const float* in, float* out, int h, int w, int d, bool backward, float* P, float* m, float* v,
                      AdamConsts ac, float* gsave, hipStream_t s);
bool box3_tile_fwd_supported(const float* in, const float* out, int h, int w, int d);
int launch_box3_tile_fwd(const float* in, float* out, int h, int w, int d, int variant, hipStream_t s);
int box3_tile_fwd_auto(int h, int w, int d);
bool box3_tile_supported(const float* in, const float* out, int h, int w, int d, const float* P, const float* m, const float* v, const float* gsave);
int launch_box3_tile(const float* in, float* out, int h, int w, int d, int variant, bool backward, float* P, float* m, float* v, AdamConsts ac,
                     float* gsave, bool prediv, bool wt, hipStream_t s);
int launch_to_chunked(const float* in, int C, size_t V, float* out, bool half, hipStream_t s);
int launch_warp_grad(const float* Fcl, const float* Mcl, int C, int h, int w, int d, const float* U, const float* bh,
                     const float* bw, const float* bd, float gsc, float cH, float cW, float cD, float* gU, bool half, bool prediv, bool wt, bool constdiv, hipStream_t s);
int launch_warp_grad_fast(const float* Fcl, const float* Mcl, int C, int h, int w, int d, const float* U, const float* bh,
                          const float* bw, const float* bd, float gsc, float cH, float cW, float cD, float* gU, bool half, bool wt, hipStream_t s);
int launch_box3_fast(const float* in, float* out, int h, int w, int d, float* P, float* m, float* v, double bc1, double bc2,
                     float* gsave, bool wt, hipStream_t s);
bool boxchain_fast_supported(const cvx_smoother& sm, int h, int w, int d);
int launch_boxchain_fast(const float* in, float* out, int h, int w, int d, const cvx_smoother& sm, bool reverse, hipStream_t s);
int launch_adam_update_fast(const float* G, float* P, float* m, float* v, size_t n, double bc1, double bc2, hipStream_t s);

}
```

### convexadam_amd/csrc/pipeline.hip

```cpp
#include <vector>

#include "cvx_common.h"
#include "mind_common.h"

namespace cvx {

__device__ __forceinline__ float linspace_pm1_at(int S, int i) {
    if (S == 1) return -1.0f;
    const float step = fdiv(1.0f - (-1.0f), (float)(S - 1));
    return (i < S / 2) ? __builtin_fmaf(step, (float)i, -1.0f) : __builtin_fmaf(-step, (float)(S - 1 - i), 1.0f);
}
struct BaseTables { int S[6]; float* out[6]; };
__global__ void k_affine_bases(BaseTables t) {
    const int S = t.S[blockIdx.y];
    float* out = t.out[blockIdx.y];
    for (int i = blockIdx.x * blockDim.x + threadIdx.x; out && i < S; i += gridDim.x * blockDim.x)
        out[i] = fdiv(linspace_pm1_at(S, i) * (float)(S - 1), (float)S);
}
__global__ void k_disp_mesh(int hw, float* out) {
    const int n = 2 * hw + 1, K = n * n * n;
    const int k = blockIdx.x * blockDim.x + threadIdx.x;
    if (k >= K) return;
    const int c = k % n, b = (k / n) % n, a = k / (n * n);
    const float la = n == 1 ? 0.f : linspace_pm1_at(n, a), lb = n == 1 ? 0.f : linspace_pm1_at(n, b),
                lc = n == 1 ? 0.f : linspace_pm1_at(n, c);
    out[k] = lc * (float)hw;
    out[K + k] = lb * (float)hw;
    out[2 * K + k] = la * (float)hw;
}

struct PairSetup {
    BaseTables t;
    int hw; float* mesh;
    unsigned long long* keys[2]; size_t v;
    int* counts[2];
    float4* zero[2]; size_t nzero4;
};
__global__ __launch_bounds__(256) void k_pair_setup(PairSetup a) {
    const size_t gid = (size_t)blockIdx.x * blockDim.x + threadIdx.x, gsz = (size_t)gridDim.x * blockDim.x;
#pragma unroll
    for (int t = 0; t < 6; ++t) {
        const int S = a.t.S[t];
        float* out = a.t.out[t];
        for (size_t i = gid; out && i < (size_t)S; i += gsz) out[i] = fdiv(linspace_pm1_at(S, (int)i) * (float)(S - 1), (float)S);
    }
    const int n = 2 * a.hw + 1, K = n * n * n;
    for (size_t k = gid; k < (size_t)K; k += gsz) {
        const int c = (int)k % n, b = ((int)k / n) % n, aa = (int)k / (n * n);
        const float la = n == 1 ? 0.f : linspace_pm1_at(n, aa), lb = n == 1 ? 0.f : linspace_pm1_at(n, b), lc = n == 1 ? 0.f : linspace_pm1_at(n, c);
        a.mesh[k] = lc * (float)a.hw;
        a.mesh[K + k] = lb * (float)a.hw;
        a.mesh[2 * K + k] = la * (float)a.hw;
    }
#pragma unroll
    for (int q = 0; q < 2; ++q) {
        if (a.keys[q]) for (size_t x = gid; x < a.v; x += gsz) a.keys[q][x] = ~0ull;
        if (a.counts[q] && gid < 2) a.counts[q][gid] = 0;
        if (a.zero[q]) for (size_t i = gid; i < a.nzero4; i += gsz) a.zero[q][i] = make_float4(0.f, 0.f, 0.f, 0.f);
    }
}

__global__ __launch_bounds__(256) void k_ic_prepare(const float* __restrict__ soft, const float* __restrict__ soft_rev, int h, int w, int d,
                                                    float* __restrict__ out, float* __restrict__ out_rev) {
    const size_t v = (size_t)h * w * d;
    const size_t p = (size_t)blockIdx.x * blockDim.x + threadIdx.x;
    if (p >= v) return;
    if (blockIdx.y) { soft = soft_rev; out = out_rev; }
    const float sc[3] = {(float)(h - 1) / 2.0f, (float)(w - 1) / 2.0f, (float)(d - 1) / 2.0f};
#pragma unroll
    for (int c = 0; c < 3; ++c) out[(size_t)c * v + p] = fdiv(soft[(size_t)(2 - c) * v + p], sc[2 - c]);
}
__global__ __launch_bounds__(256) void k_ic_finish(const float* __restrict__ ice, int h, int w, int d, float gs, float* __restrict__ out) {
    const size_t v = (size_t)h * w * d;
    const size_t p = (size_t)blockIdx.x * blockDim.x + threadIdx.x;
    if (p >= v) return;
    const float sc[3] = {(float)(h - 1) / 2.0f, (float)(w - 1) / 2.0f, (float)(d - 1) / 2.0f};
#pragma unroll
    for (int a = 0; a < 3; ++a) out[(size_t)a * v + p] = (ice[(size_t)(2 - a) * v + p] * sc[a]) * gs;
}

struct PairLayout {
    int H, W, D, h, w, d, h2, w2, d2, C, K;
    size_t V, v, V2;
    size_t featF, featM, mind_ws, mind_ws2, fs, ms, corr_ws, corr_ws2, ssd, argmin, mesh, conv_ws, ssd2, argmin2, conv_ws2, cert_ws, cert_ws2, soft, soft2, in1, in2, ic1, ic2, ic_ws,
        upin, disp_hr, F2, M2, P, m, v_, U, adam_ws, smooth_ws, smooth_ws2, snaps, bh, bw, bd, bh2, bw2, bd2, total;
};

static PairLayout pair_layout(const cvx_pair_params& p, int n_snap = 0, int max_smooth = 0) {
    PairLayout L{};
    L.H = p.H; L.W = p.W; L.D = p.D;
    L.h = p.H / p.grid_sp; L.w = p.W / p.grid_sp; L.d = p.D / p.grid_sp;
    L.h2 = p.H / p.grid_sp_adam; L.w2 = p.W / p.grid_sp_adam; L.d2 = p.D / p.grid_sp_adam;
    L.C = p.n_feat > 0 ? p.n_feat : 12;
    const int n = 2 * p.disp_hw + 1;
    L.K = n * n * n;
    L.V = (size_t)p.H * p.W * p.D; L.v = (size_t)L.h * L.w * L.d; L.V2 = (size_t)L.h2 * L.w2 * L.d2;
    Carver cv; cv.take_bytes(1);
    const size_t f = sizeof(float);
    if (p.n_feat == 0) {
        const size_t raw_floats = mind_plan(MindUse{p.H, p.W, p.D, p.mind_r, p.mind_d, p.grid_sp, p.lambda_weight > 0 ? p.grid_sp_adam : 0, 0, true, true}).raw_floats;
        L.featF = cv.take_bytes(f * raw_floats);
        L.featM = cv.take_bytes(f * raw_floats);
        L.mind_ws = cv.take_bytes(cvx_mindssc_workspace_bytes(p.H, p.W, p.D, p.mind_r, p.mind_d));
        L.mind_ws2 = cv.take_bytes(cvx_mindssc_workspace_bytes(p.H, p.W, p.D, p.mind_r, p.mind_d));
    }
    L.fs = cv.take_bytes(f * L.C * L.v);
    L.ms = cv.take_bytes(f * L.C * L.v);
    const size_t convex_scratch = align_up(cv.used, 256);
    L.corr_ws = cv.take_bytes(cvx_correlate_workspace_bytes(L.C, L.h, L.w, L.d, p.disp_hw));
    L.corr_ws2 = corr_plan(L.C, L.h, L.w, L.d, p.disp_hw, CorrUse{false, p.ic != 0, false}).pair_dual_ws ? cv.take_bytes(corr_fused_workspace_bytes(L.C, L.h, L.w, L.d, p.disp_hw)) : 0;
    const size_t ssd_elem = p.fp16_storage ? 2 : f;
    L.ssd = cv.take_bytes(ssd_elem * (size_t)L.K * L.v);
    L.argmin = cv.take_bytes(sizeof(int64_t) * L.v);
    L.mesh = cv.take_bytes(f * 3 * (size_t)L.K);
    L.conv_ws = cv.take_bytes(cvx_coupled_convex_workspace_bytes(L.h, L.w, L.d, p.disp_hw));
    L.cert_ws = cv.take_bytes(corr_certify_workspace_bytes(L.C, L.h, L.w, L.d, p.disp_hw));
    if (p.ic) {
        L.cert_ws2 = cv.take_bytes(corr_certify_workspace_bytes(L.C, L.h, L.w, L.d, p.disp_hw));
        L.ssd2 = cv.take_bytes(ssd_elem * (size_t)L.K * L.v);
        L.argmin2 = cv.take_bytes(sizeof(int64_t) * L.v);
        L.conv_ws2 = cv.take_bytes(cvx_coupled_convex_workspace_bytes(L.h, L.w, L.d, p.disp_hw));
    }
    if (p.lambda_weight > 0) {
        Carver over; over.used = convex_scratch;
        L.adam_ws = over.take_bytes(cvx_adam_workspace_bytes(L.C, L.h2, L.w2, L.d2));
        if (over.used > cv.used) cv.used = over.used;
    }
    L.soft = cv.take_bytes(f * 3 * L.v);
    L.bh = cv.take_bytes(f * L.h); L.bw = cv.take_bytes(f * L.w); L.bd = cv.take_bytes(f * L.d);
    if (p.ic) {
        L.soft2 = cv.take_bytes(f * 3 * L.v);
        L.in1 = cv.take_bytes(f * 3 * L.v); L.in2 = cv.take_bytes(f * 3 * L.v);
        L.ic1 = cv.take_bytes(f * 3 * L.v); L.ic2 = cv.take_bytes(f * 3 * L.v);
        L.ic_ws = cv.take_bytes(cvx_inverse_consistency_workspace_bytes(L.h, L.w, L.d));
        L.upin = cv.take_bytes(f * 3 * L.v);
        L.disp_hr = cv.take_bytes(f * 3 * L.V);
    }
    if (p.lambda_weight > 0) {
        const size_t f2_bytes = f * adam_record_floats(L.C, L.V2);
        L.F2 = cv.take_bytes(f2_bytes);
        L.M2 = cv.take_bytes(f2_bytes);
        L.P = cv.take_bytes(f * 3 * L.V2); L.m = cv.take_bytes(f * 3 * L.V2); L.v_ = cv.take_bytes(f * 3 * L.V2); L.U = cv.take_bytes(f * 3 * L.V2);
        L.bh2 = cv.take_bytes(f * L.h2); L.bw2 = cv.take_bytes(f * L.w2); L.bd2 = cv.take_bytes(f * L.d2);
        if (p.selected_smooth > 0 || max_smooth > 0) { L.smooth_ws = cv.take_bytes(f * 3 * L.V); L.smooth_ws2 = cv.take_bytes(f * 3 * L.V); }
        if (n_snap > 0) L.snaps = cv.take_bytes(f * 3 * L.V2 * (size_t)n_snap);
    }
    L.total = ws_query(cv);
    return L;
}

static thread_local int g_profiling = 0;
struct StageMark { const char* name; hipEvent_t ev; };
static thread_local std::vector<StageMark> g_marks;
static thread_local std::vector<hipEvent_t> g_pool;
static thread_local size_t g_pool_used = 0;

static void mark(const char* name, hipStream_t s) {
    if (!g_profiling) return;
    if (g_pool_used == g_pool.size()) {
        hipEvent_t e;
        if (hipEventCreate(&e) != hipSuccess) return;
        g_pool.push_back(e);
    }
    hipEvent_t e = g_pool[g_pool_used++];
    (void)hipEventRecord(e, s);
    g_marks.push_back({name, e});
}
void profile_mark_kernel(const char* name, hipStream_t s) {
    if (g_profiling == 3) mark(name, s);
}

struct SidePool {
    std::vector<hipStream_t> streams;
    std::vector<hipEvent_t> fork, join;
    int device = -1;
};
static thread_local SidePool g_side;
static thread_local int g_side_slot = 0;
static bool side_stream(hipStream_t* side, hipEvent_t* fork, hipEvent_t* join) {
    int dev = 0;
    (void)hipGetDevice(&dev);
    SidePool& P = g_side;
    if (P.device != dev) { P.streams.clear(); P.fork.clear(); P.join.clear(); P.device = dev; }
    while ((int)P.streams.size() <= g_side_slot) {
        hipStream_t st; hipEvent_t a, b;
        if (hipStreamCreateWithFlags(&st, hipStreamNonBlocking) != hipSuccess || hipEventCreateWithFlags(&a, hipEventDisableTiming) != hipSuccess ||
            hipEventCreateWithFlags(&b, hipEventDisableTiming) != hipSuccess) { (void)hipGetLastError(); return false; }
        P.streams.push_back(st); P.fork.push_back(a); P.join.push_back(b);
    }
    *side = P.streams[g_side_slot]; *fork = P.fork[g_side_slot]; *join = P.join[g_side_slot];
    return true;
}

static int validate(const cvx_pair_params* p) {
    CVX_REQUIRE(p, "cvx_register_pair: null params");
    CVX_REQUIRE(p->H > 0 && p->W > 0 && p->D > 0, "cvx_register_pair: bad extent");
    CVX_REQUIRE(p->grid_sp >= 1 && p->grid_sp_adam >= 1, "cvx_register_pair: grid spacing must be >= 1");
    CVX_REQUIRE(p->H / p->grid_sp >= 2 && p->W / p->grid_sp >= 2 && p->D / p->grid_sp >= 2,
                "cvx_register_pair: volume too small for grid_sp %d", p->grid_sp);
    CVX_REQUIRE(p->disp_hw >= 0 && p->disp_hw <= CVX_MAX_DISP_HW, "cvx_register_pair: disp_hw %d not in 0..%d", p->disp_hw, CVX_MAX_DISP_HW);
    CVX_REQUIRE(p->n_feat >= 0 && p->n_feat < 256, "cvx_register_pair: n_feat out of range");
    CVX_REQUIRE(p->selected_smooth == 0 || (p->selected_smooth & 1), "cvx_register_pair: selected_smooth must be odd "
                "(an even kernel changes the volume size in the reference, convex_adam_MIND.py:185-191)");
    CVX_REQUIRE((p->cost == 0 || p->cost == 1) && (p->n_box == 0 || p->n_box == 1 || p->n_box == 2) &&
                (p->n_spline_pools == 0 || p->n_spline_pools == 2 || p->n_spline_pools == 3) && (p->corr_fast == 0 || p->corr_fast == 1) &&
                (p->fp16_storage == 0 || p->fp16_storage == 1), "cvx_register_pair: bad variant fields (cost, n_box, n_spline_pools, corr_fast, fp16_storage)");
    CVX_REQUIRE((p->adam_fast == 0 || p->adam_fast == 1 || p->adam_fast == 2) && p->reserved_[0] == 0 && p->reserved_[1] == 0 && p->reserved_[2] == 0,
                "cvx_register_pair: adam_fast must be 0, 1 or 2 and the reserved fields zero (struct laid out by an older header? check cvx_version())");
    CVX_REQUIRE(!p->adam_fast || p->n_spline_pools != 2, "cvx_register_pair: adam_fast needs the packaged smoother (three 3^3 boxes)");
    if (p->lambda_weight > 0) {
        CVX_REQUIRE(p->selected_niter >= 1, "cvx_register_pair: selected_niter must be >= 1 when lambda_weight > 0 "
                    "(the reference raises UnboundLocalError, convex_adam_MIND.py:181)");
        CVX_REQUIRE(p->H / p->grid_sp_adam >= 2 && p->W / p->grid_sp_adam >= 2 && p->D / p->grid_sp_adam >= 2,
                    "cvx_register_pair: volume too small for grid_sp_adam %d", p->grid_sp_adam);
    }
    return CVX_OK;
}

}

using namespace cvx;

extern "C" int cvx_disp_mesh_f32(int disp_hw, float* out_device, void* stream) {
    CVX_REQUIRE(out_device && disp_hw >= 0 && disp_hw <= CVX_MAX_DISP_HW, "cvx_disp_mesh_f32: bad arguments (disp_hw 0 .. %d)", CVX_MAX_DISP_HW);
    const int n = 2 * disp_hw + 1, K = n * n * n;
    hipLaunchKernelGGL(k_disp_mesh, dim3(cdiv(K, 256)), dim3(256), 0, as_stream(stream), disp_hw, out_device);
    return check_last("disp_mesh");
}
extern "C" int cvx_affine_base_f32(int S, float* out_device, void* stream) {
    CVX_REQUIRE(out_device && S >= 1, "cvx_affine_base_f32: bad arguments");
    BaseTables t = {{S, 0, 0, 0, 0, 0}, {out_device, nullptr, nullptr, nullptr, nullptr, nullptr}};
    hipLaunchKernelGGL(k_affine_bases, dim3(cdiv(S, 64) > 4 ? cdiv(S, 64) : 4, 6), dim3(64), 0, as_stream(stream), t);
    return check_last("affine_base");
}

extern "C" void cvx_set_profiling(int enabled) {
    g_profiling = enabled < 0 ? 0 : (enabled > 3 ? 3 : enabled);
    g_marks.clear();
    g_pool_used = 0;
}

extern "C" int cvx_last_pair_profile(const char** names_host, float* ms_host, int max_stages) {
    if (g_marks.size() < 2) return 0;
    (void)hipEventSynchronize(g_marks.back().ev);
    int n = 0;
    for (size_t i = 1; i < g_marks.size() && n < max_stages; ++i) {
        if (g_marks[i].name[0] == 's' && g_marks[i].name[1] == 't' && g_marks[i].name[2] == 'a') continue;
        float ms = 0.f;
        (void)hipEventElapsedTime(&ms, g_marks[i - 1].ev, g_marks[i].ev);
        names_host[n] = g_marks[i].name;
        ms_host[n] = ms;
        ++n;
    }
    return n;
}

extern "C" size_t cvx_register_pair_workspace_bytes(const cvx_pair_params* p) {
    if (validate(p) != CVX_OK) return 0;
    const ContextScope scope(p->ctx);
    return pair_layout(*p).total;
}

namespace cvx {
static int smooth_max(const int* smooth_host, int n_smooth) {
    int m = 0;
    for (int i = 0; i < n_smooth; ++i) m = smooth_host[i] > m ? smooth_host[i] : m;
    return m;
}

struct IcScratch { float *in1, *in2, *ic1, *ic2; void* ws; size_t ws_bytes; };
static int ic_tail(const float* soft, const float* soft2, int h, int w, int d, int iters, const float* bh, const float* bw, const float* bd,
                   const IcScratch& t, float gs, float* dst, hipStream_t s) {
    const dim3 gv((unsigned)cdiv64((int64_t)h * w * d, 256));
    hipLaunchKernelGGL(k_ic_prepare, dim3(gv.x, 2), dim3(256), 0, s, soft, soft2, h, w, d, t.in1, t.in2);
    const int rc = cvx_inverse_consistency_f32(t.in1, t.in2, h, w, d, iters, bh, bw, bd, t.ic1, t.ic2, t.ws, t.ws_bytes, s);
    if (rc) return rc;
    hipLaunchKernelGGL(k_ic_finish, gv, dim3(256), 0, s, t.ic1, h, w, d, gs, dst);
    return CVX_OK;
}

struct LabelPair { const float *fixed, *moving; const int* present; const float* weights; float mult; };

namespace {
struct PairRun {
    const cvx_pair_params* p;
    const PairLayout& L;
    char* ws;
    hipStream_t s;
    const float *featF, *featM;
    const LabelPair* labels;
    bool pooled_mind = false, mind_records = false;
    CoupledWs cw1{}, cw2{};

    bool pooled() const { return pooled_mind || labels != nullptr; }
    bool no_prune() const { return options().no_prune != 0; }
    bool f16() const { return p->fp16_storage != 0; }
    float* F(size_t off) const { return reinterpret_cast<float*>(ws + off); }
    int64_t* am() const { return reinterpret_cast<int64_t*>(ws + L.argmin); }
    int64_t* am2() const { return p->ic ? reinterpret_cast<int64_t*>(ws + L.argmin2) : nullptr; }

    int features(const float* img_fixed, const float* img_moving) {
        int rc;
        const bool adam = p->lambda_weight > 0;
        const int g2 = adam ? p->grid_sp_adam : 0, want_records = adam && options().mind_records != 0 ? (p->fp16_storage ? 2 : 1) : 0;
        if (p->n_feat == 0) {
            auto plan_of = [&](const float* img, const float* raw) {
                return mind_plan(MindUse{p->H, p->W, p->D, p->mind_r, p->mind_d, p->grid_sp, g2, want_records, aligned16(img), aligned16(raw)});
            };
            const MindPlan plF = plan_of(img_fixed, F(L.featF)), plM = plan_of(img_moving, F(L.featM));
            pooled_mind = plF.T != 0; mind_records = plF.records != 0;
            const size_t mws = cvx_mindssc_workspace_bytes(p->H, p->W, p->D, p->mind_r, p->mind_d);
            if (pooled_mind) {
                hipStream_t side = s; hipEvent_t ev_fork = nullptr, ev_join = nullptr;
                const bool overlap = options().mind_overlap != 0 && side_stream(&side, &ev_fork, &ev_join);
                if (overlap) { (void)hipEventRecord(ev_fork, s); (void)hipStreamWaitEvent(side, ev_fork, 0); }
                else side = s;
                if ((rc = launch_mind_pooled(plF, img_fixed, F(L.fs), adam ? F(L.F2) : nullptr, F(L.featF), ws + L.mind_ws, mws, s))) return rc;
                rc = launch_mind_pooled(plM, img_moving, F(L.ms), adam ? F(L.M2) : nullptr, F(L.featM), ws + (overlap ? L.mind_ws2 : L.mind_ws), mws, side);
                if (overlap) { (void)hipEventRecord(ev_join, side); (void)hipStreamWaitEvent(s, ev_join, 0); }
                if (rc) return rc;
            } else {
                if ((rc = cvx_mindssc_f32(img_fixed, p->H, p->W, p->D, p->mind_r, p->mind_d, F(L.featF), ws + L.mind_ws, mws, s))) return rc;
                if ((rc = cvx_mindssc_f32(img_moving, p->H, p->W, p->D, p->mind_r, p->mind_d, F(L.featM), ws + L.mind_ws, mws, s))) return rc;
            }
            featF = F(L.featF); featM = F(L.featM);
        }
        if (labels) {
            if ((rc = launch_label_pooled(labels->fixed, p->H, p->W, p->D, L.C, labels->present, labels->weights, labels->mult, p->grid_sp, F(L.fs), g2,
                                          adam ? F(L.F2) : nullptr, s))) return rc;
            if ((rc = launch_label_pooled(labels->moving, p->H, p->W, p->D, L.C, labels->present, labels->weights, labels->mult, p->grid_sp, F(L.ms), g2,
                                          adam ? F(L.M2) : nullptr, s))) return rc;
        }
        mark(labels ? "label_features" : "mind", s);
        if (!pooled()) {
            if ((rc = cvx_avgpool_f32(featF, L.C, p->H, p->W, p->D, p->grid_sp, F(L.fs), s))) return rc;
            if ((rc = cvx_avgpool_f32(featM, L.C, p->H, p->W, p->D, p->grid_sp, F(L.ms), s))) return rc;
        }
        return CVX_OK;
    }
    void setup() {
        Carver cv1(ws + L.conv_ws), cv2(p->ic ? ws + L.conv_ws2 : nullptr);
        cw1 = coupled_layout(cv1, L.h, L.w, L.d, p->disp_hw); cw2 = coupled_layout(cv2, L.h, L.w, L.d, p->disp_hw);
        const bool adam_tables = p->lambda_weight > 0;
        const bool zero_state = adam_tables && (3 * L.V2) % 4 == 0;
        PairSetup a = {{{L.h, L.w, L.d, L.h2, L.w2, L.d2},
                        {F(L.bh), F(L.bw), F(L.bd), adam_tables ? F(L.bh2) : nullptr, adam_tables ? F(L.bw2) : nullptr, adam_tables ? F(L.bd2) : nullptr}},
                       p->disp_hw, F(L.mesh), {cw1.keys[0], cw2.keys[0]}, L.v,
                       {no_prune() ? nullptr : cw1.counts, no_prune() ? nullptr : cw2.counts},
                       {zero_state ? reinterpret_cast<float4*>(ws + L.m) : nullptr, zero_state ? reinterpret_cast<float4*>(ws + L.v_) : nullptr}, 3 * L.V2 / 4};
        hipLaunchKernelGGL(k_pair_setup, dim3(zero_state ? 1024 : 64), dim3(256), 0, s, a);
        if (adam_tables && !zero_state) {
            (void)hipMemsetAsync(F(L.m), 0, sizeof(float) * 3 * L.V2, s);
            (void)hipMemsetAsync(F(L.v_), 0, sizeof(float) * 3 * L.V2, s);
        }
    }
    int plain_argmin(const float* ssd, unsigned long long* keys, int64_t* argmin, const char* done) {
        const int rc = no_prune() ? launch_argmin(ssd, f16(), nullptr, nullptr, 0.0f, false, L.K, L.v, keys, argmin, s)
                                : launch_argmin_keys(ssd, f16(), L.K, L.v, keys, false, s);
        if (rc == CVX_OK) mark(done, s);
        return rc;
    }
    int exact_direction(const float* fix, const float* mov, const cvx_corr_opts* copt, float* ssd, unsigned long long* keys, int64_t* argmin,
                        const char* correlated, const char* done) {
        const int rc = cvx_correlate_ex_f32(fix, mov, L.C, L.h, L.w, L.d, p->disp_hw, copt, ssd, nullptr, ws + L.corr_ws,
                                            cvx_correlate_workspace_bytes(L.C, L.h, L.w, L.d, p->disp_hw), s);
        if (rc) return rc;
        mark(correlated, s);
        return plain_argmin(ssd, keys, argmin, done);
    }
    int convex() {
        int rc;
        const cvx_corr_opts copt = {p->cost, p->n_box == 1 ? 1 : 2, p->corr_fast, f16() ? 2 : 0};
        const bool variant = copt.cost || copt.n_box == 1 || copt.fast || copt.f16;
        if (p->fp16_storage) {
            if ((rc = cvx_round_f16_f32(F(L.fs), (int64_t)L.C * L.v, s)) || (rc = cvx_round_f16_f32(F(L.ms), (int64_t)L.C * L.v, s))) return rc;
        }
        const CorrPlan plan = corr_plan(L.C, L.h, L.w, L.d, p->disp_hw, CorrUse{variant, p->ic != 0, no_prune()});
        if (plan.pair_cert) {
            const size_t fws = corr_certfast_workspace_bytes(L.C, L.h, L.w, L.d, p->disp_hw), qws = corr_certify_workspace_bytes(L.C, L.h, L.w, L.d, p->disp_hw);
            auto cert_stage = [&](int stage) {
                return coupled_convex_cert_impl(F(L.ssd), F(L.fs), F(L.ms), F(L.soft), ws + L.cert_ws, p->ic ? F(L.ssd2) : nullptr, F(L.ms), F(L.fs),
                                                p->ic ? F(L.soft2) : nullptr, p->ic ? ws + L.cert_ws2 : nullptr, F(L.mesh), L.C, L.h, L.w, L.d, p->disp_hw, qws, s, stage);
            };
            if ((rc = cert_stage(1))) return rc;
            if ((rc = launch_corr_certfast(F(L.fs), F(L.ms), L.C, L.h, L.w, L.d, p->disp_hw, F(L.ssd), ws + L.corr_ws, fws, s))) return rc;
            mark("correlate", s);
            if ((rc = cert_stage(2))) return rc;
            mark("argmin", s);
            if (p->ic) {
                if ((rc = launch_corr_certfast(F(L.ms), F(L.fs), L.C, L.h, L.w, L.d, p->disp_hw, F(L.ssd2), ws + L.corr_ws, fws, s))) return rc;
                mark("correlate_rev", s);
                if ((rc = cert_stage(3))) return rc;
                mark("argmin_rev", s);
            }
            if ((rc = cert_stage(4))) return rc;
            return cert_stage(5);
        }
        if (plan.pair_dual) {
            const size_t fws = corr_fused_workspace_bytes(L.C, L.h, L.w, L.d, p->disp_hw);
            if ((rc = launch_corr_fused_dual(F(L.fs), F(L.ms), L.C, L.h, L.w, L.d, p->disp_hw, copt.cost, copt.n_box, copt.fast, copt.f16, F(L.ssd), F(L.ssd2),
                                             ws + L.corr_ws, fws, ws + L.corr_ws2, s))) return rc;
            mark("correlate", s);
            if ((rc = plain_argmin(F(L.ssd), cw1.keys[0], am(), "argmin"))) return rc;
            if ((rc = plain_argmin(F(L.ssd2), cw2.keys[0], am2(), "argmin_rev"))) return rc;
        } else {
            if ((rc = exact_direction(F(L.fs), F(L.ms), variant ? &copt : nullptr, F(L.ssd), cw1.keys[0], am(), "correlate", "argmin"))) return rc;
            if (p->ic && (rc = exact_direction(F(L.ms), F(L.fs), variant ? &copt : nullptr, F(L.ssd2), cw2.keys[0], am2(), "correlate_rev", "argmin_rev"))) return rc;
        }
        return coupled_convex_dual_impl(F(L.ssd), no_prune() ? am() : nullptr, F(L.soft), ws + L.conv_ws, p->ic ? F(L.ssd2) : nullptr, f16(), no_prune() ? am2() : nullptr,
                                        p->ic ? F(L.soft2) : nullptr, p->ic ? ws + L.conv_ws2 : nullptr, F(L.mesh), L.h, L.w, L.d,
                                        p->disp_hw, cvx_coupled_convex_workspace_bytes(L.h, L.w, L.d, p->disp_hw), s, !no_prune());
    }
    int upsample_smoothed(const float* src, int k, float* dst) {
        int rc;
        if (k <= 0) return launch_resize(src, 3, L.h2, L.w2, L.d2, dst, p->H, p->W, p->D, (float)p->grid_sp_adam, 1.0f, s);
        float *tmp = F(L.smooth_ws), *tmp2 = F(L.smooth_ws2);
        if ((rc = launch_resize(src, 3, L.h2, L.w2, L.d2, tmp, p->H, p->W, p->D, (float)p->grid_sp_adam, 1.0f, s))) return rc;
        if ((rc = launch_box_zero(tmp, tmp2, 3, p->H, p->W, p->D, k, false, s))) return rc;
        if ((rc = launch_box_zero(tmp2, tmp, 3, p->H, p->W, p->D, k, false, s))) return rc;
        return launch_box_zero(tmp, dst, 3, p->H, p->W, p->D, k, false, s);
    }
    int adam_and_output(const int* snap_iters_host, int n_snap, const int* smooth_host, int n_smooth, float* out_field) {
        int rc;
        if (!pooled()) {
            if ((rc = cvx_avgpool_f32(featF, L.C, p->H, p->W, p->D, p->grid_sp_adam, F(L.F2), s))) return rc;
            if ((rc = cvx_avgpool_f32(featM, L.C, p->H, p->W, p->D, p->grid_sp_adam, F(L.M2), s))) return rc;
        }
        if (p->ic) rc = launch_resize2(F(L.upin), 3, L.h, L.w, L.d, p->H, p->W, p->D, F(L.disp_hr), F(L.P), L.h2, L.w2, L.d2, (float)p->grid_sp_adam, s);
        else rc = launch_resize(F(L.soft), 3, L.h, L.w, L.d, F(L.P), L.h2, L.w2, L.d2, 1.0f, (float)p->grid_sp_adam, s);
        if (rc) return rc;
        mark("adam_setup", s);
        const cvx_smoother two_pools = {0, 2, {3, 3, 0, 0}, {0.f, 0.f, 0.f, 0.f, 0.f}};
        if ((rc = adam_run_impl({.F2 = F(L.F2), .M2 = F(L.M2), .C = L.C, .h = L.h2, .w = L.w2, .d = L.d2, .P = F(L.P), .m = F(L.m), .v = F(L.v_),
                                 .lambda_weight = p->lambda_weight, .niter = p->selected_niter, .step0 = 0, .cost_scale = p->cost_scale,
                                 .base_h = F(L.bh2), .base_w = F(L.bw2), .base_d = F(L.bd2), .U = F(L.U), .grad_out = nullptr,
                                 .snapshot_iters_host = snap_iters_host, .n_snap = n_snap, .snapshots = n_snap ? F(L.snaps) : nullptr,
                                 .workspace = ws + L.adam_ws, .workspace_bytes = cvx_adam_workspace_bytes(L.C, L.h2, L.w2, L.d2), .stream = s,
                                 .sm = p->n_spline_pools == 2 ? &two_pools : nullptr, .keep_state = false, .f16_features = f16(),
                                 .fast = p->adam_fast, .features_are_records = mind_records}))) return rc;
        mark("adam", s);
        if (n_snap > 0) {
            for (int i = 0; i < n_snap; ++i)
                for (int j = 0; j < n_smooth; ++j)
                    if ((rc = upsample_smoothed(F(L.snaps) + (size_t)i * 3 * L.V2, smooth_host[j], out_field + ((size_t)i * n_smooth + j) * 3 * L.V))) return rc;
        } else if ((rc = upsample_smoothed(F(L.U), p->selected_smooth, out_field))) return rc;
        mark("upsample", s);
        return CVX_OK;
    }
};
}

static int register_pair_core(const float* img_fixed, const float* img_moving, const float* feat_fixed, const float* feat_moving,
                              const cvx_pair_params* p, float* out_field, int* out_dims_host, const int* snap_iters_host, int n_snap,
                              const int* smooth_host, int n_smooth, void* workspace, size_t workspace_bytes, void* stream, const LabelPair* labels = nullptr) {
    int rc = validate(p);
    if (rc) return rc;
    const ContextScope scope(p->ctx);
    CVX_REQUIRE(out_field && workspace, "cvx_register_pair_f32: null pointer");
    if (labels) CVX_REQUIRE(p->n_feat >= 1 && labels->fixed && labels->moving && labels->present && labels->weights,
                            "cvx_register_label_pair_f32: label maps, channel labels or weights missing, or n_feat == 0 (n_feat = number of channels)");
    else if (p->n_feat == 0) CVX_REQUIRE(img_fixed && img_moving, "cvx_register_pair_f32: images missing");
    else CVX_REQUIRE(feat_fixed && feat_moving, "cvx_register_pair_f32: feature volumes missing");
    const PairLayout L = pair_layout(*p, n_snap, n_snap ? smooth_max(smooth_host, n_smooth) : 0);
    if (workspace_bytes < L.total) return fail(CVX_ERR_WORKSPACE, "cvx_register_pair_f32: workspace %zu < %zu", workspace_bytes, L.total);
    hipStream_t s = as_stream(stream);
    if (g_profiling < 2) { g_marks.clear(); g_pool_used = 0; }
    mark("start", s);
    corr_fused_set_prep_hook(g_profiling ? +[](hipStream_t st) { mark("correlate_prep", st); } : nullptr);
    struct HookReset { ~HookReset() { corr_fused_set_prep_hook(nullptr); } } hook_reset;

    PairRun run = {p, L, static_cast<char*>(workspace), s, feat_fixed, feat_moving, labels};
    const bool adam = p->lambda_weight > 0;
    if ((rc = run.features(img_fixed, img_moving))) return rc;
    run.setup();
    mark("pool", s);
    if ((rc = run.convex())) return rc;
    mark("coupled_convex", s);
    if (p->ic) {
        const IcScratch t = {run.F(L.in1), run.F(L.in2), run.F(L.ic1), run.F(L.ic2), run.ws + L.ic_ws, cvx_inverse_consistency_workspace_bytes(L.h, L.w, L.d)};
        if ((rc = ic_tail(run.F(L.soft), run.F(L.soft2), L.h, L.w, L.d, 15, run.F(L.bh), run.F(L.bw), run.F(L.bd), t, (float)p->grid_sp, run.F(L.upin), s))) return rc;
        if (!adam && (rc = launch_resize(run.F(L.upin), 3, L.h, L.w, L.d, out_field, p->H, p->W, p->D, 1.0f, 1.0f, s))) return rc;
        mark("inverse_consistency", s);
    }
    if (adam) {
        if ((rc = run.adam_and_output(snap_iters_host, n_snap, smooth_host, n_smooth, out_field))) return rc;
    } else if (!p->ic) {
        (void)hipMemcpyAsync(out_field, run.F(L.soft), sizeof(float) * 3 * L.v, hipMemcpyDeviceToDevice, s);
    }
    const bool full = p->ic || adam;
    if (out_dims_host) { out_dims_host[0] = full ? p->H : L.h; out_dims_host[1] = full ? p->W : L.w; out_dims_host[2] = full ? p->D : L.d; }
    return check_last("register_pair");
}
}

extern "C" int cvx_register_pair_f32(const float* img_fixed, const float* img_moving, const float* feat_fixed,
                                     const float* feat_moving, const cvx_pair_params* p, float* out_field,
                                     int* out_dims_host, void* workspace, size_t workspace_bytes, void* stream) {
    return register_pair_core(img_fixed, img_moving, feat_fixed, feat_moving, p, out_field, out_dims_host, nullptr, 0, nullptr, 0, workspace,
                              workspace_bytes, stream);
}

extern "C" size_t cvx_register_label_pair_workspace_bytes(const cvx_pair_params* p) {
    if (validate(p) != CVX_OK) return 0;
    if (p->n_feat < 1) { fail(CVX_ERR_INVALID_ARG, "cvx_register_label_pair: n_feat must be the number of channels (>= 1)"); return 0; }
    const ContextScope scope(p->ctx);
    return pair_layout(*p).total;
}

extern "C" int cvx_register_label_pair_f32(const float* lab_fixed, const float* lab_moving, const int* present, const float* weights, float mult,
                                           const cvx_pair_params* p, float* out_field, int* out_dims_host, void* workspace, size_t workspace_bytes,
                                           void* stream) {
    const LabelPair labels = {lab_fixed, lab_moving, present, weights, mult};
    return register_pair_core(nullptr, nullptr, nullptr, nullptr, p, out_field, out_dims_host, nullptr, 0, nullptr, 0, workspace, workspace_bytes, stream,
                              &labels);
}

extern "C" size_t cvx_register_pair_snapshots_workspace_bytes(const cvx_pair_params* p, int n_snap, const int* smooth_host, int n_smooth) {
    if (validate(p) != CVX_OK || n_snap < 1 || n_smooth < 1 || !smooth_host) return 0;
    const ContextScope scope(p->ctx);
    return pair_layout(*p, n_snap, smooth_max(smooth_host, n_smooth)).total;
}

extern "C" int cvx_register_pair_snapshots_f32(const float* img_fixed, const float* img_moving, const float* feat_fixed,
                                               const float* feat_moving, const cvx_pair_params* p, const int* snapshot_iters_host, int n_snap,
                                               const int* smooth_host, int n_smooth, float* out_fields, void* workspace,
                                               size_t workspace_bytes, void* stream) {
    int rc = validate(p);
    if (rc) return rc;
    CVX_REQUIRE(snapshot_iters_host && n_snap >= 1 && smooth_host && n_smooth >= 1, "cvx_register_pair_snapshots_f32: snapshot / smoothing lists missing");
    CVX_REQUIRE(p->lambda_weight > 0, "cvx_register_pair_snapshots_f32: snapshots exist only with the Adam stage (lambda_weight > 0)");
    for (int i = 0; i < n_snap; ++i)
        CVX_REQUIRE(snapshot_iters_host[i] >= 1 && snapshot_iters_host[i] <= p->selected_niter && (i == 0 || snapshot_iters_host[i] > snapshot_iters_host[i - 1]),
                    "cvx_register_pair_snapshots_f32: snapshot iterations must be ascending and within 1..selected_niter");
    for (int i = 0; i < n_smooth; ++i)
        CVX_REQUIRE(smooth_host[i] == 0 || (smooth_host[i] & 1), "cvx_register_pair_snapshots_f32: smoothing sizes must be 0 or odd");
    return register_pair_core(img_fixed, img_moving, feat_fixed, feat_moving, p, out_fields, nullptr, snapshot_iters_host, n_snap, smooth_host,
                              n_smooth, workspace, workspace_bytes, stream);
}

namespace cvx {
struct StreamPool {
    std::vector<hipStream_t> streams;
    std::vector<hipEvent_t> done;
    hipEvent_t fork = nullptr;
    int device = -1;
};
static thread_local StreamPool g_pool_streams;
static int ensure_streams(int n) {
    int dev = 0;
    (void)hipGetDevice(&dev);
    StreamPool& P = g_pool_streams;
    if (P.device != dev) { P.streams.clear(); P.done.clear(); P.fork = nullptr; P.device = dev; }
    if (!P.fork && hipEventCreateWithFlags(&P.fork, hipEventDisableTiming) != hipSuccess) return fail(CVX_ERR_LAUNCH, "event create failed");
    while ((int)P.streams.size() < n) {
        hipStream_t s; hipEvent_t e;
        if (hipStreamCreateWithFlags(&s, hipStreamNonBlocking) != hipSuccess) return fail(CVX_ERR_LAUNCH, "stream create failed");
        if (hipEventCreateWithFlags(&e, hipEventDisableTiming) != hipSuccess) return fail(CVX_ERR_LAUNCH, "event create failed");
        P.streams.push_back(s); P.done.push_back(e);
    }
    return CVX_OK;
}
}

extern "C" int cvx_register_pairs_f32(int n_pairs, const float* const* img_fixed, const float* const* img_moving,
                                      const float* const* feat_fixed, const float* const* feat_moving,
                                      const cvx_pair_params* p, float* const* out_fields, int* out_dims_host, void* workspace,
                                      size_t workspace_bytes, int n_streams, void* stream) {
    CVX_REQUIRE(n_pairs >= 1 && out_fields && workspace, "cvx_register_pairs_f32: bad arguments");
    CVX_REQUIRE(n_streams >= 1 && n_streams <= 8, "cvx_register_pairs_f32: n_streams must be 1..8");
    if (n_streams > n_pairs) n_streams = n_pairs;
    const size_t per = cvx_register_pair_workspace_bytes(p);
    if (per == 0) return CVX_ERR_INVALID_ARG;
    const size_t per_al = align_up(per, 4096);
    if (workspace_bytes < per_al * (size_t)n_streams) return fail(CVX_ERR_WORKSPACE, "cvx_register_pairs_f32: workspace %zu < %zu", workspace_bytes, per_al * (size_t)n_streams);
    int rc = ensure_streams(n_streams);
    if (rc) return rc;
    StreamPool& P = g_pool_streams;
    hipStream_t user = as_stream(stream);
    const int saved_prof = g_profiling;
    g_profiling = 0;
    (void)hipEventRecord(P.fork, user);
    for (int s = 0; s < n_streams; ++s) (void)hipStreamWaitEvent(P.streams[s], P.fork, 0);
    for (int i = 0; i < n_pairs && rc == CVX_OK; ++i) {
        const int s = i % n_streams;
        g_side_slot = s;
        rc = cvx_register_pair_f32(img_fixed ? img_fixed[i] : nullptr, img_moving ? img_moving[i] : nullptr,
                                   feat_fixed ? feat_fixed[i] : nullptr, feat_moving ? feat_moving[i] : nullptr, p, out_fields[i],
                                   out_dims_host, static_cast<char*>(workspace) + per_al * (size_t)s, per, P.streams[s]);
    }
    for (int s = 0; s < n_streams; ++s) {
        (void)hipEventRecord(P.done[s], P.streams[s]);
        (void)hipStreamWaitEvent(user, P.done[s], 0);
    }
    g_profiling = saved_prof;
    g_side_slot = 0;
    return rc;
}

namespace cvx {
struct StageWs {
    float *ssd, *mesh, *soft, *soft2, *in1, *in2, *ic1, *ic2, *upin, *bh, *bw, *bd;
    int64_t* argmin;
    char *corr_ws, *conv_ws, *ic_ws;
    size_t corr_bytes, conv_bytes, ic_bytes;
};
static StageWs stage_layout(Carver& cv, const cvx_convex_stage_params& p) {
    const int n = 2 * p.disp_hw + 1;
    const size_t v = (size_t)p.h * p.w * p.d, K = (size_t)n * n * n;
    StageWs s{};
    s.ssd = cv.take<float>(K * v);
    s.argmin = cv.take<int64_t>(v);
    s.mesh = cv.take<float>(3 * K);
    s.soft = cv.take<float>(3 * v);
    s.corr_bytes = cvx_correlate_workspace_bytes(p.C, p.h, p.w, p.d, p.disp_hw);
    s.corr_ws = cv.take<char>(s.corr_bytes);
    s.conv_bytes = cvx_coupled_convex_workspace_bytes(p.h, p.w, p.d, p.disp_hw);
    s.conv_ws = cv.take<char>(s.conv_bytes);
    if (p.ic_iters > 0) {
        s.soft2 = cv.take<float>(3 * v);
        s.in1 = cv.take<float>(3 * v); s.in2 = cv.take<float>(3 * v);
        s.ic1 = cv.take<float>(3 * v); s.ic2 = cv.take<float>(3 * v);
        s.upin = cv.take<float>(3 * v);
        s.bh = cv.take<float>(p.h); s.bw = cv.take<float>(p.w); s.bd = cv.take<float>(p.d);
        s.ic_bytes = cvx_inverse_consistency_workspace_bytes(p.h, p.w, p.d);
        s.ic_ws = cv.take<char>(s.ic_bytes);
    }
    return s;
}
static int stage_params_ok(const cvx_convex_stage_params* p) {
    CVX_REQUIRE(p, "cvx_convex_stage_f32: null parameters");
    CVX_REQUIRE(p->reserved_[0] == 0 && p->reserved_[1] == 0 && p->reserved_[2] == 0 && p->reserved_[3] == 0,
                "cvx_convex_stage_f32: reserved fields must be zero (struct laid out by a different header?)");
    CVX_REQUIRE(p->C >= 1 && p->h >= 1 && p->w >= 1 && p->d >= 1 && p->disp_hw >= 0 && p->grid_sp >= 1 && p->ic_iters >= 0,
                "cvx_convex_stage_f32: bad extent, search width, grid spacing or iteration count");
    CVX_REQUIRE((double)(2 * p->disp_hw + 1) * (2 * p->disp_hw + 1) * (2 * p->disp_hw + 1) * ((double)p->h * p->w * p->d) < 2.0e9,
                "cvx_convex_stage_f32: cost volume of more than 2e9 entries");
    return CVX_OK;
}
}

extern "C" size_t cvx_convex_stage_workspace_bytes(const cvx_convex_stage_params* p) {
    if (stage_params_ok(p) != CVX_OK) return 0;
    Carver m;
    stage_layout(m, *p);
    return ws_query(m);
}

extern "C" int cvx_convex_stage_f32(const float* feat_fix, const float* feat_mov, const unsigned char* mask_fix, const unsigned char* mask_mov,
                                    const cvx_convex_stage_params* p, float* coarse_field, float* disp_hr, void* workspace,
                                    size_t workspace_bytes, void* stream) {
    int rc = stage_params_ok(p);
    if (rc) return rc;
    CVX_REQUIRE(feat_fix && feat_mov && workspace && (coarse_field || disp_hr), "cvx_convex_stage_f32: null pointer");
    CVX_REQUIRE(!disp_hr || (p->H >= 1 && p->W >= 1 && p->D >= 1), "cvx_convex_stage_f32: bad full-resolution extent");
    if (workspace_bytes < cvx_convex_stage_workspace_bytes(p)) return fail(CVX_ERR_WORKSPACE, "cvx_convex_stage_f32: workspace too small");
    const ContextScope scope(p->ctx);
    hipStream_t s = as_stream(stream);
    Carver cv(workspace);
    const StageWs L = stage_layout(cv, *p);
    const int h = p->h, w = p->w, d = p->d;
    if ((rc = cvx_disp_mesh_f32(p->disp_hw, L.mesh, stream))) return rc;
    auto direction = [&](const float* a, const float* b, const unsigned char* mask, float* soft) -> int {
        int r = cvx_correlate_ex_f32(a, b, p->C, h, w, d, p->disp_hw, nullptr, L.ssd, L.argmin, L.corr_ws, L.corr_bytes, stream);
        if (r) return r;
        return coupled_convex_impl(L.ssd, false, L.argmin, L.mesh, h, w, d, p->disp_hw, soft, false, L.conv_ws, L.conv_bytes,
                                   stream, mask);
    };
    if (p->ic_iters == 0) {
        float* soft = coarse_field ? coarse_field : L.soft;
        if ((rc = direction(feat_fix, feat_mov, mask_fix, soft))) return rc;
        if (disp_hr && (rc = launch_resize(soft, 3, h, w, d, disp_hr, p->H, p->W, p->D, (float)p->grid_sp, 1.0f, s))) return rc;
        return check_last("convex_stage");
    }
    if ((rc = direction(feat_fix, feat_mov, mask_fix, L.soft))) return rc;
    if ((rc = direction(feat_mov, feat_fix, mask_mov, L.soft2))) return rc;
    if ((rc = cvx_affine_base_f32(h, L.bh, stream)) || (rc = cvx_affine_base_f32(w, L.bw, stream)) || (rc = cvx_affine_base_f32(d, L.bd, stream))) return rc;
    float* up = coarse_field ? coarse_field : L.upin;
    if ((rc = ic_tail(L.soft, L.soft2, h, w, d, p->ic_iters, L.bh, L.bw, L.bd, {L.in1, L.in2, L.ic1, L.ic2, L.ic_ws, L.ic_bytes}, (float)p->grid_sp, up, s))) return rc;
    if (disp_hr && (rc = launch_resize(up, 3, h, w, d, disp_hr, p->H, p->W, p->D, 1.0f, 1.0f, s))) return rc;
    return check_last("convex_stage");
}
```

### convexadam_amd/csrc/pool.hip

```cpp
#include <hip/hip_fp16.h>
#include <math.h>
#include <string.h>

#include "cvx_common.h"

namespace cvx {

__global__ __launch_bounds__(256) void k_avgpool(const float* __restrict__ in, int C, int H, int W, int D, int g,
                                                 float* __restrict__ out) {
    const int Ho = H / g, Wo = W / g, Do = D / g;
    const size_t n = (size_t)C * Ho * Wo * Do;
    const size_t i = (size_t)blockIdx.x * blockDim.x + threadIdx.x;
    if (i >= n) return;
    const int d = (int)(i % Do), w = (int)((i / Do) % Wo), h = (int)((i / ((size_t)Do * Wo)) % Ho);
    const int c = (int)(i / ((size_t)Do * Wo * Ho));
    const float* base = in + (((size_t)c * H + (size_t)h * g) * W + (size_t)w * g) * D + (size_t)d * g;
    float s = 0.0f;
    for (int z = 0; z < g; ++z)
        for (int y = 0; y < g; ++y) {
            const float* row = base + ((size_t)z * W + y) * D;
            for (int x = 0; x < g; ++x) s += row[x];
        }
    out[i] = fdiv(s, (float)(g * g * g));
}

template <int G>
__global__ __launch_bounds__(256) void k_avgpool_even(const float* __restrict__ in, int C, int H, int W, int D,
                                                      float* __restrict__ out) {
    static_assert(G % 2 == 0, "even windows only");
    const int Ho = H / G, Wo = W / G, Do = D / G;
    const size_t n = (size_t)C * Ho * Wo * Do;
    const size_t i = (size_t)blockIdx.x * blockDim.x + threadIdx.x;
    if (i >= n) return;
    const int d = (int)(i % Do), w = (int)((i / Do) % Wo), h = (int)((i / ((size_t)Do * Wo)) % Ho);
    const int c = (int)(i / ((size_t)Do * Wo * Ho));
    const float* base = in + (((size_t)c * H + (size_t)h * G) * W + (size_t)w * G) * D + (size_t)d * G;
    float s = 0.0f;
#pragma unroll
    for (int z = 0; z < G; ++z) {
        float2 v[G][G / 2];
#pragma unroll
        for (int y = 0; y < G; ++y)
#pragma unroll
            for (int x = 0; x < G / 2; ++x) v[y][x] = *reinterpret_cast<const float2*>(base + ((size_t)z * W + y) * D + 2 * x);
#pragma unroll
        for (int y = 0; y < G; ++y)
#pragma unroll
            for (int x = 0; x < G / 2; ++x) { s += v[y][x].x; s += v[y][x].y; }
    }
    out[i] = fdiv(s, (float)(G * G * G));
}

template <bool BACKWARD>
__global__ __launch_bounds__(256) void k_box_zero(const float* __restrict__ in, float* __restrict__ out, int C, int H,
                                                  int W, int D, int k) {
    const size_t n = (size_t)C * H * W * D;
    const size_t i = (size_t)blockIdx.x * blockDim.x + threadIdx.x;
    if (i >= n) return;
    const int d = (int)(i % D), w = (int)((i / D) % W), h = (int)((i / ((size_t)D * W)) % H);
    const int c = (int)(i / ((size_t)D * W * H));
    const int p = k / 2;
    const float div = (float)(k * k * k);
    const int h0 = max(h - p, 0), h1 = min(h + p, H - 1), w0 = max(w - p, 0), w1 = min(w + p, W - 1),
              d0 = max(d - p, 0), d1 = min(d + p, D - 1);
    const float* ic = in + (size_t)c * H * W * D;
    float s = 0.0f;
    for (int z = h0; z <= h1; ++z)
        for (int y = w0; y <= w1; ++y)
            for (int x = d0; x <= d1; ++x) {
                const float v = ic[((size_t)z * W + y) * D + x];
                s += BACKWARD ? fdiv(v, div) : v;
            }
    out[i] = BACKWARD ? s : fdiv(s, div);
}

__global__ __launch_bounds__(256) void k_box_grow(const float* __restrict__ in, float* __restrict__ out, int C, int H, int W, int D, int k) {
    const int Ho = H + 1, Wo = W + 1, Do = D + 1;
    const size_t n = (size_t)C * Ho * Wo * Do;
    const size_t i = (size_t)blockIdx.x * blockDim.x + threadIdx.x;
    if (i >= n) return;
    const int d = (int)(i % Do), w = (int)((i / Do) % Wo), h = (int)((i / ((size_t)Do * Wo)) % Ho);
    const int c = (int)(i / ((size_t)Do * Wo * Ho));
    const int p = k / 2;
    const int h0 = max(h - p, 0), h1 = min(h - p + k, H), w0 = max(w - p, 0), w1 = min(w - p + k, W), d0 = max(d - p, 0), d1 = min(d - p + k, D);
    const float* ic = in + (size_t)c * H * W * D;
    float s = 0.0f;
    for (int z = h0; z < h1; ++z)
        for (int y = w0; y < w1; ++y)
            for (int x = d0; x < d1; ++x) s += ic[((size_t)z * W + y) * D + x];
    out[i] = fdiv(s, (float)(k * k * k));
}

template <int R, int CPT>
__global__ __launch_bounds__(256) void k_box_walk(const float* __restrict__ in, float* __restrict__ out, int C, int H, int W, int D, int L, int nq) {
    constexpr int K = 2 * R + 1, WC = CPT + 2 * R;
    const size_t item = (size_t)blockIdx.x * blockDim.x + threadIdx.x;
    if (item >= (size_t)C * W * nq) return;
    const int lane = threadIdx.x & 63;
    const int q = (int)(item % nq), y = (int)((item / nq) % W), c = (int)(item / ((size_t)nq * W));
    const int x0 = q * CPT, z0 = (int)blockIdx.y * L, zend = min(z0 + L, H);
    const size_t plane = (size_t)W * D;
    const float* ic = in + (size_t)c * H * plane;
    float* oc = out + (size_t)c * H * plane;
    bool rok[K];
    unsigned roff[K];
#pragma unroll
    for (int i = 0; i < K; ++i) { const int yy = y - R + i; rok[i] = yy >= 0 && yy < W; roff[i] = (unsigned)((rok[i] ? yy : 0) * D + x0); }
    bool cl[R], cr[R];
#pragma unroll
    for (int t = 0; t < R; ++t) { cl[t] = x0 - R + t >= 0; cr[t] = x0 + CPT + t < D; }
    float sum[K][CPT];
#pragma unroll
    for (int r = 0; r < K; ++r)
#pragma unroll
        for (int j = 0; j < CPT; ++j) sum[r][j] = 0.0f;
    constexpr float DIVF = (float)(K * K * K);
    for (int p = z0 - R; p < zend + R; ++p) {
        if (p >= 0 && p < H) {
            const float* pp = ic + (size_t)p * plane;
            float w[K][WC];
#pragma unroll
            for (int i = 0; i < K; ++i) {
                const float* rp = pp + roff[i];
                if (CPT == 4) {
                    const float4 a = rok[i] ? *reinterpret_cast<const float4*>(rp) : make_float4(0.f, 0.f, 0.f, 0.f);
                    w[i][R] = a.x; w[i][R + 1] = a.y; w[i][R + 2] = a.z; w[i][R + 3] = a.w;
                } else {
                    const float2 a = rok[i] ? *reinterpret_cast<const float2*>(rp) : make_float2(0.f, 0.f);
                    w[i][R] = a.x; w[i][R + 1] = a.y;
                }
                if (R <= CPT) {
#pragma unroll
                    for (int t = 0; t < R; ++t) {
                        const float fromL = __int_as_float(__builtin_amdgcn_update_dpp(0, __float_as_int(w[i][CPT + t]), 0x138, 0xf, 0xf, true));
                        const float fromR = __int_as_float(__builtin_amdgcn_update_dpp(0, __float_as_int(w[i][R + t]), 0x130, 0xf, 0xf, true));
                        float hl = fromL, hr = fromR;
                        if (lane == 0 && rok[i] && cl[t]) hl = rp[t - R];
                        if (lane == 63 && rok[i] && cr[t]) hr = rp[CPT + t];
                        w[i][t] = cl[t] ? hl : 0.0f;
                        w[i][R + CPT + t] = cr[t] ? hr : 0.0f;
                    }
                } else {
#pragma unroll
                    for (int t = 0; t < R; ++t) {
                        w[i][t] = (rok[i] && cl[t]) ? rp[t - R] : 0.0f;
                        w[i][R + CPT + t] = (rok[i] && cr[t]) ? rp[CPT + t] : 0.0f;
                    }
                }
            }
#pragma unroll
            for (int i = 0; i < K; ++i)
#pragma unroll
                for (int t = 0; t < K; ++t)
#pragma unroll
                    for (int r = 0; r < K; ++r)
#pragma unroll
                        for (int j = 0; j < CPT; ++j) sum[r][j] += w[i][j + t];
        }
        const int o = p - R;
        if (o >= z0 && o < zend) {
            float* op = oc + ((size_t)o * W + y) * D + x0;
            float v[CPT];
#pragma unroll
            for (int j = 0; j < CPT; ++j) v[j] = (K == 3 || K == 5 || K == 7) ? div_exact_inf<(K == 3 || K == 5 || K == 7) ? K * K * K : 27>(sum[0][j]) : fdiv(sum[0][j], DIVF);
            if (CPT == 4) *reinterpret_cast<float4*>(op) = make_float4(v[0], v[1], v[CPT - 2], v[CPT - 1]);
            else *reinterpret_cast<float2*>(op) = make_float2(v[0], v[1]);
        }
#pragma unroll
        for (int r = 0; r + 1 < K; ++r)
#pragma unroll
            for (int j = 0; j < CPT; ++j) sum[r][j] = sum[r + 1][j];
#pragma unroll
        for (int j = 0; j < CPT; ++j) sum[K - 1][j] = 0.0f;
    }
}

template <int R>
static int launch_box_walk_r(const float* in, float* out, int C, int H, int W, int D, hipStream_t s) {
    const size_t quads4 = (size_t)C * W * (D / 4);
    const bool cpt2 = quads4 * H < ((size_t)1 << 22);
    const int cpt = cpt2 ? 2 : 4, nq = D / cpt;
    const size_t items = (size_t)C * W * nq;
    int L = 16;
    while (L > 4 && items * (size_t)cdiv(H, L) < (size_t)256 * 256 * 6) L -= 4;
    const dim3 grid((unsigned)cdiv64((int64_t)items, 256), (unsigned)cdiv(H, L));
    if (cpt2) hipLaunchKernelGGL((k_box_walk<R, 2>), grid, dim3(256), 0, s, in, out, C, H, W, D, L, nq);
    else hipLaunchKernelGGL((k_box_walk<R, 4>), grid, dim3(256), 0, s, in, out, C, H, W, D, L, nq);
    return check_last("box_walk");
}

int launch_box_zero(const float* in, float* out, int C, int H, int W, int D, int k, bool backward, hipStream_t s) {
    const size_t n = (size_t)C * H * W * D;
    const bool al = ((reinterpret_cast<uintptr_t>(in) | reinterpret_cast<uintptr_t>(out)) & 15) == 0;
    if (!backward && al && D % 4 == 0 && in != out && options().box_walk != 0) {
        if (k == 3) return launch_box_walk_r<1>(in, out, C, H, W, D, s);
        if (k == 5) return launch_box_walk_r<2>(in, out, C, H, W, D, s);
        if (k == 7) return launch_box_walk_r<3>(in, out, C, H, W, D, s);
    }
    const dim3 grid((unsigned)cdiv64((int64_t)n, 256));
    if (backward) hipLaunchKernelGGL(k_box_zero<true>, grid, dim3(256), 0, s, in, out, C, H, W, D, k);
    else hipLaunchKernelGGL(k_box_zero<false>, grid, dim3(256), 0, s, in, out, C, H, W, D, k);
    return check_last("box_zero");
}

struct GaussW { float w[5]; };
template <bool BACKWARD>
__global__ __launch_bounds__(256) void k_gauss1d(const float* __restrict__ in, float* __restrict__ out, size_t total, int n,
                                                 size_t stride, GaussW gw, bool fused_bwd) {
    const size_t i = (size_t)blockIdx.x * blockDim.x + threadIdx.x;
    if (i >= total) return;
    const int a = (int)((i / stride) % n);
    const float* base = in + (i - (size_t)a * stride);
    if (!BACKWARD) {
        float acc = gw.w[0] * base[(size_t)clampi(a - 2, 0, n - 1) * stride];
#pragma unroll
        for (int t = 1; t < 5; ++t) acc = __builtin_fmaf(gw.w[t], base[(size_t)clampi(a + t - 2, 0, n - 1) * stride], acc);
        out[i] = acc;
    } else {
        float r = 0.0f;
        const int j0 = a == 0 ? 0 : a + 2, j1 = a == n - 1 ? n + 3 : a + 2;
        for (int j = j0; j <= j1; ++j) {
            float g0 = (j >= 0 && j < n) ? base[(size_t)j * stride] : 0.0f;
            float acc = gw.w[0] * g0;
#pragma unroll
            for (int t = 1; t < 5; ++t) {
                const int q = j - t;
                const float gq = (q >= 0 && q < n) ? base[(size_t)q * stride] : 0.0f;
                acc = fused_bwd ? __builtin_fmaf(gw.w[t], gq, acc) : acc + gw.w[t] * gq;
            }
            r += acc;
        }
        out[i] = r;
    }
}
static int launch_gauss1d(const float* in, float* out, int C, int H, int W, int D, int axis, const float* w5, bool backward,
                          hipStream_t s) {
    const size_t total = (size_t)C * H * W * D;
    const int n = axis == 0 ? H : (axis == 1 ? W : D);
    const size_t stride = axis == 0 ? (size_t)W * D : (axis == 1 ? (size_t)D : 1);
    GaussW gw;
    for (int t = 0; t < 5; ++t) gw.w[t] = w5[t];
    const dim3 grid((unsigned)cdiv64((int64_t)total, 256));
    if (backward) hipLaunchKernelGGL(k_gauss1d<true>, grid, dim3(256), 0, s, in, out, total, n, stride, gw, C > 1);
    else hipLaunchKernelGGL(k_gauss1d<false>, grid, dim3(256), 0, s, in, out, total, n, stride, gw, C > 1);
    return check_last("gauss1d");
}

int launch_smoother(const float* in, float* out, float* tmp, int C, int H, int W, int D, const cvx_smoother& sm, bool backward,
                    hipStream_t s) {
    const int nst = sm.kind == 1 ? 3 : sm.n_boxes;
    const float* src = in;
    for (int i = 0; i < nst; ++i) {
        float* dst = ((nst - 1 - i) & 1) ? tmp : out;
        const int st = backward ? nst - 1 - i : i;
        int rc;
        if (sm.kind == 1) rc = launch_gauss1d(src, dst, C, H, W, D, st, sm.gauss_w, backward, s);
        else rc = launch_box_zero(src, dst, C, H, W, D, sm.box_k[st], backward, s);
        if (rc) return rc;
        src = dst;
    }
    return CVX_OK;
}

__global__ __launch_bounds__(256) void k_mask_erode(const float* __restrict__ mask, int H, int W, int D, float thr,
                                                    float* __restrict__ out) {
    const size_t n = (size_t)H * W * D;
    const size_t i = (size_t)blockIdx.x * blockDim.x + threadIdx.x;
    if (i >= n) return;
    const int d = (int)(i % D), w = (int)((i / D) % W), h = (int)(i / ((size_t)D * W));
    float s = 0.0f;
    for (int a = -1; a <= 1; ++a)
        for (int b = -1; b <= 1; ++b)
            for (int c = -1; c <= 1; ++c)
                s += mask[((size_t)clampi(h + a, 0, H - 1) * W + clampi(w + b, 0, W - 1)) * D + clampi(d + c, 0, D - 1)];
    out[i] = fdiv(s, 27.0f) > thr ? 1.0f : 0.0f;
}
__global__ __launch_bounds__(256) void k_gather_index(const float* __restrict__ src, const int64_t* __restrict__ idx, size_t n,
                                                      float* __restrict__ out) {
    const size_t i = (size_t)blockIdx.x * blockDim.x + threadIdx.x;
    if (i < n) out[i] = src[idx[i]];
}
__global__ __launch_bounds__(256) void k_select(const float* __restrict__ m, const float* __restrict__ a, const float* __restrict__ b,
                                                size_t n, float* __restrict__ out) {
    const size_t i = (size_t)blockIdx.x * blockDim.x + threadIdx.x;
    if (i < n) out[i] = m[i] != 0.0f ? a[i] : b[i];
}

template <int CT>
__global__ __launch_bounds__(256) void k_resize(const float* __restrict__ in, int C, int h, int w, int d,
                                                float* __restrict__ out, int H, int W, int D, float pre_mul,
                                                float post_div) {
    const int x = (int)(blockIdx.x * blockDim.x + threadIdx.x), y = (int)blockIdx.y, z = (int)blockIdx.z;
    if (x >= D) return;
    const size_t n = (size_t)H * W * D;
    const size_t i = ((size_t)z * W + y) * D + x;
    int z0, z1, y0, y1, x0, x1;
    float lz0, lz1, ly0, ly1, lx0, lx1;
    lin_coef(z, h, H, z0, z1, lz0, lz1);
    lin_coef(y, w, W, y0, y1, ly0, ly1);
    lin_coef(x, d, D, x0, x1, lx0, lx1);
    const size_t o00 = ((size_t)z0 * w + y0) * d, o01 = ((size_t)z0 * w + y1) * d, o10 = ((size_t)z1 * w + y0) * d,
                 o11 = ((size_t)z1 * w + y1) * d;
    const size_t cs = (size_t)h * w * d;
    auto one = [&](const float (&v)[8]) {
        float r = resize_chain(v, pre_mul, lx0, lx1, ly0, ly1, lz0, lz1);
        if (post_div != 1.0f) r = fdiv(r, post_div);
        return r;
    };
    auto fetch = [&](const float* ic, float (&v)[8]) {
        v[0] = ic[o00 + x0]; v[1] = ic[o00 + x1]; v[2] = ic[o01 + x0]; v[3] = ic[o01 + x1];
        v[4] = ic[o10 + x0]; v[5] = ic[o10 + x1]; v[6] = ic[o11 + x0]; v[7] = ic[o11 + x1];
    };
    if (CT > 0) {
        float v[CT > 0 ? CT : 1][8];
#pragma unroll
        for (int c = 0; c < CT; ++c) fetch(in + (size_t)c * cs, v[c]);
#pragma unroll
        for (int c = 0; c < CT; ++c) out[(size_t)c * n + i] = one(v[c]);
    } else {
        for (int c = 0; c < C; ++c) {
            float v[8];
            fetch(in + (size_t)c * cs, v);
            out[(size_t)c * n + i] = one(v);
        }
    }
}
template <int CT>
__global__ __launch_bounds__(256) void k_resize_up2(const float* __restrict__ in, int h, int w, int d, float* __restrict__ out, float pre_mul,
                                                    float post_div) {
    const int kx = (int)(blockIdx.x * blockDim.x + threadIdx.x), ky = (int)blockIdx.y, kz = (int)blockIdx.z;
    if (kx >= d) return;
    const int H = 2 * h, W = 2 * w, D = 2 * d;
    struct Ax { int p0[2], p1[2]; float l0[2], l1[2]; };
    auto axis = [](int k, int n_in, Ax& a) {
#pragma unroll
        for (int t = 0; t < 2; ++t) {
            int i0, i1;
            lin_coef(2 * k + t, n_in, 2 * n_in, i0, i1, a.l0[t], a.l1[t]);
            a.p0[t] = i0 - k + 1;
            a.p1[t] = i1 - k + 1;
        }
    };
    Ax az, ay, ax;
    axis(kz, h, az); axis(ky, w, ay); axis(kx, d, ax);
    const int zi[3] = {kz > 0 ? kz - 1 : 0, kz, kz < h - 1 ? kz + 1 : h - 1}, yi[3] = {ky > 0 ? ky - 1 : 0, ky, ky < w - 1 ? ky + 1 : w - 1},
              xi[3] = {kx > 0 ? kx - 1 : 0, kx, kx < d - 1 ? kx + 1 : d - 1};
    auto sel = [](float v0, float v1, float v2, int p) { return p == 0 ? v0 : (p == 1 ? v1 : v2); };
    const size_t cs = (size_t)h * w * d, n = (size_t)H * W * D;
    float v[CT][3][3][3];
#pragma unroll
    for (int c = 0; c < CT; ++c)
#pragma unroll
        for (int a = 0; a < 3; ++a)
#pragma unroll
            for (int b = 0; b < 3; ++b)
#pragma unroll
                for (int e = 0; e < 3; ++e) v[c][a][b][e] = in[(size_t)c * cs + ((size_t)zi[a] * w + yi[b]) * d + xi[e]];
#pragma unroll
    for (int c = 0; c < CT; ++c) {
        float X[3][3][2], Y[3][2][2];
#pragma unroll
        for (int a = 0; a < 3; ++a)
#pragma unroll
            for (int b = 0; b < 3; ++b)
#pragma unroll
                for (int t = 0; t < 2; ++t) {
                    const float u0 = sel(v[c][a][b][0], v[c][a][b][1], v[c][a][b][2], ax.p0[t]), u1 = sel(v[c][a][b][0], v[c][a][b][1], v[c][a][b][2], ax.p1[t]);
                    X[a][b][t] = __builtin_fmaf(u0 * pre_mul, ax.l0[t], (u1 * pre_mul) * ax.l1[t]);
                }
#pragma unroll
        for (int a = 0; a < 3; ++a)
#pragma unroll
            for (int ty = 0; ty < 2; ++ty)
#pragma unroll
                for (int t = 0; t < 2; ++t) {
                    const float u0 = sel(X[a][0][t], X[a][1][t], X[a][2][t], ay.p0[ty]), u1 = sel(X[a][0][t], X[a][1][t], X[a][2][t], ay.p1[ty]);
                    Y[a][ty][t] = __builtin_fmaf(u0, ay.l0[ty], u1 * ay.l1[ty]);
                }
#pragma unroll
        for (int tz = 0; tz < 2; ++tz)
#pragma unroll
            for (int ty = 0; ty < 2; ++ty) {
                float r[2];
#pragma unroll
                for (int t = 0; t < 2; ++t) {
                    const float u0 = sel(Y[0][ty][t], Y[1][ty][t], Y[2][ty][t], az.p0[tz]), u1 = sel(Y[0][ty][t], Y[1][ty][t], Y[2][ty][t], az.p1[tz]);
                    r[t] = __builtin_fmaf(u0, az.l0[tz], u1 * az.l1[tz]);
                    if (post_div != 1.0f) r[t] = fdiv(r[t], post_div);
                }
                *reinterpret_cast<float2*>(out + (size_t)c * n + ((size_t)(2 * kz + tz) * W + (2 * ky + ty)) * D + 2 * kx) = make_float2(r[0], r[1]);
            }
    }
}
int launch_resize(const float* in, int C, int h, int w, int d, float* out, int H, int W, int D, float pre_mul,
                  float post_div, hipStream_t s) {
    if (H > 65535 || W > 65535) return fail(CVX_ERR_UNSUPPORTED, "resize_trilinear: output extent %dx%d exceeds the grid limits", H, W);
    if (C == 3 && H == 2 * h && W == 2 * w && D == 2 * d && (reinterpret_cast<uintptr_t>(out) & 7) == 0 && options().resize_up2 != 0) {
        const int bx = d > 128 ? 256 : (d > 64 ? 128 : 64);
        hipLaunchKernelGGL(k_resize_up2<3>, dim3((unsigned)cdiv(d, bx), (unsigned)w, (unsigned)h), dim3(bx), 0, s, in, h, w, d, out, pre_mul, post_div);
        return check_last("resize_trilinear");
    }
    const int bx = D > 128 ? 256 : (D > 64 ? 128 : 64);
    const dim3 grid((unsigned)cdiv(D, bx), (unsigned)W, (unsigned)H), block(bx);
    if (C == 3) hipLaunchKernelGGL(k_resize<3>, grid, block, 0, s, in, C, h, w, d, out, H, W, D, pre_mul, post_div);
    else if (C == 1) hipLaunchKernelGGL(k_resize<1>, grid, block, 0, s, in, C, h, w, d, out, H, W, D, pre_mul, post_div);
    else hipLaunchKernelGGL(k_resize<0>, grid, block, 0, s, in, C, h, w, d, out, H, W, D, pre_mul, post_div);
    return check_last("resize_trilinear");
}

template <int CT>
__global__ __launch_bounds__(256) void k_resize_yx(const float* __restrict__ in, int C, int h, int w, int d, float* __restrict__ T,
                                                   int W, int D) {
    const int x = (int)(blockIdx.x * blockDim.x + threadIdx.x), y = (int)blockIdx.y, z = (int)blockIdx.z;
    if (x >= D) return;
    const size_t n = (size_t)h * W * D;
    const size_t i = ((size_t)z * W + y) * D + x;
    int y0, y1, x0, x1;
    float ly0, ly1, lx0, lx1;
    lin_coef(y, w, W, y0, y1, ly0, ly1);
    lin_coef(x, d, D, x0, x1, lx0, lx1);
    auto one = [&](int c) {
        const float* r0 = in + (((size_t)c * h + z) * w + y0) * d;
        const float* r1 = in + (((size_t)c * h + z) * w + y1) * d;
        const float a = __builtin_fmaf(r0[x0], lx0, r0[x1] * lx1);
        const float b = __builtin_fmaf(r1[x0], lx0, r1[x1] * lx1);
        T[(size_t)c * n + i] = __builtin_fmaf(a, ly0, b * ly1);
    };
    if (CT > 0) {
#pragma unroll
        for (int c = 0; c < CT; ++c) one(c);
    } else
        for (int c = 0; c < C; ++c) one(c);
}
template <int CT>
__global__ __launch_bounds__(256) void k_resize2(const float* __restrict__ T, int C, int h, int H, int W, int D, float* __restrict__ out,
                                                 int h2, int w2, int d2, float post_div) {
    const int x = (int)(blockIdx.x * blockDim.x + threadIdx.x), y = (int)blockIdx.y, z = (int)blockIdx.z;
    if (x >= d2) return;
    const size_t n = (size_t)h2 * w2 * d2;
    const size_t i = ((size_t)z * w2 + y) * d2 + x;
    int Z[2], Y[2], X[2], cz[2][2];
    float LZ[2], LY[2], LX[2], wz[2][2];
    lin_coef(z, H, h2, Z[0], Z[1], LZ[0], LZ[1]);
    lin_coef(y, W, w2, Y[0], Y[1], LY[0], LY[1]);
    lin_coef(x, D, d2, X[0], X[1], LX[0], LX[1]);
#pragma unroll
    for (int a = 0; a < 2; ++a) lin_coef(Z[a], h, H, cz[a][0], cz[a][1], wz[a][0], wz[a][1]);
    const size_t plane = (size_t)W * D;
    const bool pairs = (D & 1) == 0 && (reinterpret_cast<uintptr_t>(T) & 7) == 0 && __all(X[1] == X[0] + 1 && (X[0] & 1) == 0);
    auto one = [&](int c) {
        const float* Tc = T + (size_t)c * h * plane;
        float v[2][2][2][2];
        if (pairs) {
#pragma unroll
            for (int a = 0; a < 2; ++a)
#pragma unroll
                for (int p = 0; p < 2; ++p)
#pragma unroll
                    for (int b = 0; b < 2; ++b) {
                        const float2 q = *reinterpret_cast<const float2*>(Tc + (size_t)cz[a][p] * plane + (size_t)Y[b] * D + X[0]);
                        v[a][p][b][0] = q.x; v[a][p][b][1] = q.y;
                    }
        } else {
#pragma unroll
        for (int a = 0; a < 2; ++a)
#pragma unroll
            for (int p = 0; p < 2; ++p)
#pragma unroll
                for (int b = 0; b < 2; ++b)
#pragma unroll
                    for (int e = 0; e < 2; ++e) v[a][p][b][e] = Tc[(size_t)cz[a][p] * plane + (size_t)Y[b] * D + X[e]];
        }
        float lev1[2];
#pragma unroll
        for (int a = 0; a < 2; ++a) {
            float lev2[2];
#pragma unroll
            for (int b = 0; b < 2; ++b) {
                const float m0 = __builtin_fmaf(v[a][0][b][0], wz[a][0], v[a][1][b][0] * wz[a][1]);
                const float m1 = __builtin_fmaf(v[a][0][b][1], wz[a][0], v[a][1][b][1] * wz[a][1]);
                lev2[b] = __builtin_fmaf(m0, LX[0], m1 * LX[1]);
            }
            lev1[a] = __builtin_fmaf(lev2[0], LY[0], lev2[1] * LY[1]);
        }
        float r = __builtin_fmaf(lev1[0], LZ[0], lev1[1] * LZ[1]);
        if (post_div != 1.0f) r = fdiv(r, post_div);
        out[(size_t)c * n + i] = r;
    };
    if (CT > 0) {
#pragma unroll
        for (int c = 0; c < CT; ++c) one(c);
    } else
        for (int c = 0; c < C; ++c) one(c);
}
int launch_resize2(const float* in, int C, int h, int w, int d, int H, int W, int D, float* scratch, float* out, int h2, int w2, int d2,
                   float post_div, hipStream_t s) {
    if (W > 65535 || h > 65535 || w2 > 65535 || h2 > 65535) return fail(CVX_ERR_UNSUPPORTED, "resize_trilinear2: extent exceeds the grid limits");
    auto bx = [](int n) { return n > 128 ? 256 : (n > 64 ? 128 : 64); };
    const dim3 g1((unsigned)cdiv(D, bx(D)), (unsigned)W, (unsigned)h), g2((unsigned)cdiv(d2, bx(d2)), (unsigned)w2, (unsigned)h2);
    if (C == 3) {
        hipLaunchKernelGGL(k_resize_yx<3>, g1, dim3(bx(D)), 0, s, in, C, h, w, d, scratch, W, D);
        hipLaunchKernelGGL(k_resize2<3>, g2, dim3(bx(d2)), 0, s, scratch, C, h, H, W, D, out, h2, w2, d2, post_div);
    } else {
        hipLaunchKernelGGL(k_resize_yx<0>, g1, dim3(bx(D)), 0, s, in, C, h, w, d, scratch, W, D);
        hipLaunchKernelGGL(k_resize2<0>, g2, dim3(bx(d2)), 0, s, scratch, C, h, H, W, D, out, h2, w2, d2, post_div);
    }
    return check_last("resize_trilinear2");
}

__global__ __launch_bounds__(256) void k_grid_sample(const float* __restrict__ vol, int C, int h, int w, int d,
                                                     const float* __restrict__ grid, size_t vo, float* __restrict__ out) {
    const size_t p = (size_t)blockIdx.x * blockDim.x + threadIdx.x;
    if (p >= vo) return;
    Tri t;
    tri_setup(t, grid[3 * p], grid[3 * p + 1], grid[3 * p + 2], h, w, d);
    const size_t vi = (size_t)h * w * d;
    for (int c = 0; c < C; ++c) out[(size_t)c * vo + p] = tri_sample(t, vol + (size_t)c * vi, h, w, d);
}

__global__ __launch_bounds__(256) void k_label_hist(const float* __restrict__ lab, int64_t V, int max_label,
                                                    unsigned long long* __restrict__ hist) {
    extern __shared__ unsigned int sh[];
    for (int i = threadIdx.x; i <= max_label; i += blockDim.x) sh[i] = 0;
    cvx_barrier();
    for (int64_t i = (int64_t)blockIdx.x * blockDim.x + threadIdx.x; i < V; i += (int64_t)gridDim.x * blockDim.x) {
        const int l = (int)lab[i];
        if (l >= 0 && l <= max_label) atomicAdd(&sh[l], 1u);
    }
    cvx_barrier();
    for (int i = threadIdx.x; i <= max_label; i += blockDim.x)
        if (sh[i]) atomicAdd(&hist[i], (unsigned long long)sh[i]);
}
__global__ __launch_bounds__(256) void k_label_features(const float* __restrict__ lab, int64_t V, int C,
                                                        const int* __restrict__ present,
                                                        const float* __restrict__ weights, float mult,
                                                        float* __restrict__ feat) {
    const int64_t i = (int64_t)blockIdx.x * blockDim.x + threadIdx.x;
    if (i >= V) return;
    const int l = (int)lab[i];
    for (int c = 0; c < C; ++c) {
        const float oh = (l == present[c]) ? 1.0f : 0.0f;
        feat[(size_t)c * V + i] = mult * (oh * weights[c]);
    }
}

}

using namespace cvx;

extern "C" int cvx_avgpool_f32(const float* in, int C, int H, int W, int D, int g, float* out, void* stream) {
    CVX_REQUIRE(in && out, "cvx_avgpool_f32: null pointer");
    CVX_REQUIRE(C > 0 && H > 0 && W > 0 && D > 0 && g > 0, "cvx_avgpool_f32: bad arguments");
    CVX_REQUIRE(H / g > 0 && W / g > 0 && D / g > 0, "cvx_avgpool_f32: pooling window %d larger than the volume", g);
    const size_t n = (size_t)C * (H / g) * (W / g) * (D / g);
    const dim3 grid((unsigned)cdiv64((int64_t)n, 256));
    const bool even = (D % 2 == 0) && (reinterpret_cast<uintptr_t>(in) & 7) == 0;
    if (even && g == 2) hipLaunchKernelGGL(k_avgpool_even<2>, grid, dim3(256), 0, as_stream(stream), in, C, H, W, D, out);
    else if (even && g == 4) hipLaunchKernelGGL(k_avgpool_even<4>, grid, dim3(256), 0, as_stream(stream), in, C, H, W, D, out);
    else if (even && g == 6) hipLaunchKernelGGL(k_avgpool_even<6>, grid, dim3(256), 0, as_stream(stream), in, C, H, W, D, out);
    else if (even && g == 8) hipLaunchKernelGGL(k_avgpool_even<8>, grid, dim3(256), 0, as_stream(stream), in, C, H, W, D, out);
    else hipLaunchKernelGGL(k_avgpool, grid, dim3(256), 0, as_stream(stream), in, C, H, W, D, g, out);
    return check_last("avgpool");
}

static int check_smoother(const cvx_smoother* sm) {
    CVX_REQUIRE(sm, "smoother: null");
    CVX_REQUIRE(sm->kind == 0 || sm->kind == 1, "smoother: kind must be 0 (box chain) or 1 (gaussian)");
    if (sm->kind == 0) {
        CVX_REQUIRE(sm->n_boxes >= 1 && sm->n_boxes <= 4, "smoother: n_boxes must be 1..4");
        for (int i = 0; i < sm->n_boxes; ++i) CVX_REQUIRE(sm->box_k[i] >= 1 && (sm->box_k[i] & 1), "smoother: box size must be odd");
    }
    return CVX_OK;
}
static float* smooth_layout(Carver& cv, int C, int H, int W, int D, bool tmp) { return tmp ? cv.take<float>((size_t)C * H * W * D) : nullptr; }
extern "C" size_t cvx_smooth_workspace_bytes(int C, int H, int W, int D) { Carver m; smooth_layout(m, C, H, W, D, true); return ws_query(m); }
extern "C" int cvx_smooth_f32(const float* in, int C, int H, int W, int D, const cvx_smoother* sm, int backward, float* out,
                              void* workspace, size_t workspace_bytes, void* stream) {
    CVX_REQUIRE(in && out && in != out && workspace, "cvx_smooth_f32: bad pointers");
    CVX_REQUIRE(C > 0 && H > 0 && W > 0 && D > 0, "cvx_smooth_f32: bad extent");
    int rc = check_smoother(sm);
    if (rc) return rc;
    if (workspace_bytes < cvx_smooth_workspace_bytes(C, H, W, D)) return fail(CVX_ERR_WORKSPACE, "cvx_smooth_f32: workspace too small");
    Carver cv(workspace);
    float* tmp = smooth_layout(cv, C, H, W, D, true);
    return launch_smoother(in, out, tmp, C, H, W, D, *sm, backward != 0, as_stream(stream));
}

extern "C" int cvx_mask_erode_f32(const float* mask, int H, int W, int D, float threshold, float* out, void* stream) {
    CVX_REQUIRE(mask && out && H > 0 && W > 0 && D > 0, "cvx_mask_erode_f32: bad arguments");
    const size_t n = (size_t)H * W * D;
    hipLaunchKernelGGL(k_mask_erode, dim3((unsigned)cdiv64((int64_t)n, 256)), dim3(256), 0, as_stream(stream), mask, H, W, D, threshold, out);
    return check_last("mask_erode");
}
extern "C" int cvx_gather_f32(const float* src, const int64_t* index, int64_t n, float* out, void* stream) {
    CVX_REQUIRE(src && index && out && n > 0, "cvx_gather_f32: bad arguments");
    hipLaunchKernelGGL(k_gather_index, dim3((unsigned)cdiv64(n, 256)), dim3(256), 0, as_stream(stream), src, index, (size_t)n, out);
    return check_last("gather");
}
extern "C" int cvx_select_f32(const float* mask, const float* a, const float* b, int64_t n, float* out, void* stream) {
    CVX_REQUIRE(mask && a && b && out && n > 0, "cvx_select_f32: bad arguments");
    hipLaunchKernelGGL(k_select, dim3((unsigned)cdiv64(n, 256)), dim3(256), 0, as_stream(stream), mask, a, b, (size_t)n, out);
    return check_last("select");
}

extern "C" size_t cvx_box_smooth_workspace_bytes(int C, int H, int W, int D, int passes) { Carver m; smooth_layout(m, C, H, W, D, passes > 1); return ws_query(m); }
extern "C" int cvx_box_smooth_f32(const float* in, int C, int H, int W, int D, int k, int passes, float* out,
                                  void* workspace, size_t workspace_bytes, void* stream) {
    CVX_REQUIRE(in && out, "cvx_box_smooth_f32: null pointer");
    CVX_REQUIRE(C > 0 && H > 0 && W > 0 && D > 0, "cvx_box_smooth_f32: bad extent");
    CVX_REQUIRE(k >= 1 && (k & 1), "cvx_box_smooth_f32: kernel %d must be odd (the reference's even-kernel path changes the "
                "volume size, convex_adam_MIND.py:185-191)", k);
    CVX_REQUIRE(passes >= 1, "cvx_box_smooth_f32: passes must be >= 1");
    if (workspace_bytes < cvx_box_smooth_workspace_bytes(C, H, W, D, passes))
        return fail(CVX_ERR_WORKSPACE, "cvx_box_smooth_f32: workspace too small");
    CVX_REQUIRE(in != out, "cvx_box_smooth_f32: in-place not supported");
    hipStream_t s = as_stream(stream);
    Carver cv(workspace);
    float* tmp = smooth_layout(cv, C, H, W, D, passes > 1);
    const float* src = in;
    for (int p = 0; p < passes; ++p) {
        float* dst = ((passes - 1 - p) & 1) ? tmp : out;
        int rc = launch_box_zero(src, dst, C, H, W, D, k, false, s);
        if (rc) return rc;
        src = dst;
    }
    return CVX_OK;
}

extern "C" int cvx_box_grow_f32(const float* in, int C, int H, int W, int D, int k, float* out, void* stream) {
    CVX_REQUIRE(in && out && in != out, "cvx_box_grow_f32: null pointer or in-place");
    CVX_REQUIRE(C > 0 && H > 0 && W > 0 && D > 0, "cvx_box_grow_f32: bad extent");
    CVX_REQUIRE(k >= 2 && !(k & 1) && k <= 64, "cvx_box_grow_f32: kernel %d must be even, 2 .. 64 (odd kernels: cvx_box_smooth_f32)", k);
    CVX_REQUIRE(k / 2 <= H && k / 2 <= W && k / 2 <= D, "cvx_box_grow_f32: padding %d exceeds the extent (avg_pool3d: pad <= kernel / 2 and input >= pad)", k / 2);
    const size_t n = (size_t)C * (H + 1) * (W + 1) * (D + 1);
    hipLaunchKernelGGL(k_box_grow, dim3((unsigned)cdiv64((int64_t)n, 256)), dim3(256), 0, as_stream(stream), in, out, C, H, W, D, k);
    return check_last("box_grow");
}

extern "C" int cvx_resize_trilinear_f32(const float* in, int C, int h, int w, int d, float* out, int H, int W, int D,
                                        void* stream) {
    CVX_REQUIRE(in && out, "cvx_resize_trilinear_f32: null pointer");
    CVX_REQUIRE(C > 0 && h > 0 && w > 0 && d > 0 && H > 0 && W > 0 && D > 0, "cvx_resize_trilinear_f32: bad extent");
    return launch_resize(in, C, h, w, d, out, H, W, D, 1.0f, 1.0f, as_stream(stream));
}

extern "C" int cvx_grid_sample_f32(const float* vol, int C, int h, int w, int d, const float* grid, int ho, int wo,
                                   int dd, float* out, void* stream) {
    CVX_REQUIRE(vol && grid && out, "cvx_grid_sample_f32: null pointer");
    CVX_REQUIRE(C > 0 && h > 0 && w > 0 && d > 0 && ho > 0 && wo > 0 && dd > 0, "cvx_grid_sample_f32: bad extent");
    const size_t vo = (size_t)ho * wo * dd;
    hipLaunchKernelGGL(k_grid_sample, dim3((unsigned)cdiv64((int64_t)vo, 256)), dim3(256), 0, as_stream(stream), vol, C,
                       h, w, d, grid, vo, out);
    return check_last("grid_sample");
}

extern "C" int cvx_label_histogram_i64(const float* lab, int64_t V, int max_label, int64_t* hist, void* stream) {
    CVX_REQUIRE(lab && hist && V > 0, "cvx_label_histogram_i64: bad arguments");
    CVX_REQUIRE(max_label >= 0 && max_label < 8192, "cvx_label_histogram_i64: max_label %d out of range", max_label);
    hipStream_t s = as_stream(stream);
    if (hipMemsetAsync(hist, 0, sizeof(int64_t) * (size_t)(max_label + 1), s) != hipSuccess)
        return fail(CVX_ERR_LAUNCH, "cvx_label_histogram_i64: memset failed");
    const int nb = (int)(cdiv64(V, 256 * 16) < 1024 ? cdiv64(V, 256 * 16) : 1024);
    hipLaunchKernelGGL(k_label_hist, dim3(nb), dim3(256), sizeof(unsigned) * (size_t)(max_label + 1), s, lab, V, max_label,
                       reinterpret_cast<unsigned long long*>(hist));
    return check_last("label_histogram");
}

namespace {
typedef struct { float x, y; } lw_f2;
static inline float lw_i2f(int32_t i) { float f; memcpy(&f, &i, 4); return f; }
static inline int32_t lw_f2i(float f) { int32_t i; memcpy(&i, &f, 4); return i; }
static inline lw_f2 lw_mk(float x, float y) { lw_f2 r = {x, y}; return r; }
static inline lw_f2 lw_dfadd2_f_f(float x, float y) { lw_f2 r; r.x = x + y; float v = r.x - x; r.y = (x - (r.x - v)) + (y - v); return r; }
static inline lw_f2 lw_dfadd2_f2_f(lw_f2 x, float y) { lw_f2 r; r.x = x.x + y; float v = r.x - x.x; r.y = (x.x - (r.x - v)) + (y - v); r.y = r.y + x.y; return r; }
static inline lw_f2 lw_dfadd2_f2_f2(lw_f2 x, lw_f2 y) { lw_f2 r; r.x = x.x + y.x; float v = r.x - x.x; r.y = (x.x - (r.x - v)) + (y.x - v); r.y = r.y + (x.y + y.y); return r; }
static inline lw_f2 lw_dfadd_f2_f2(lw_f2 x, lw_f2 y) { lw_f2 r; r.x = x.x + y.x; r.y = x.x - r.x + y.x + x.y + y.y; return r; }
static inline lw_f2 lw_dfadd_f_f2(float x, lw_f2 y) { lw_f2 r; r.x = x + y.x; r.y = x - r.x + y.x + y.y; return r; }
static inline lw_f2 lw_dfmul_f2_f(lw_f2 x, float y) { lw_f2 r; r.x = x.x * y; r.y = fmaf(x.y, y, fmaf(x.x, y, -r.x)); return r; }
static inline lw_f2 lw_dfmul_f2_f2(lw_f2 x, lw_f2 y) { lw_f2 r; r.x = x.x * y.x; r.y = fmaf(x.x, y.y, fmaf(x.y, y.x, fmaf(x.x, y.x, -r.x))); return r; }
static inline lw_f2 lw_dfsqu(lw_f2 x) { lw_f2 r; r.x = x.x * x.x; r.y = fmaf(x.x + x.x, x.y, fmaf(x.x, x.x, -r.x)); return r; }
static inline lw_f2 lw_dfdiv(lw_f2 n, lw_f2 d) {
    float t = 1.0f / d.x; lw_f2 q; q.x = n.x * t;
    float u = fmaf(t, n.x, -q.x);
    q.y = fmaf(-d.y, t, fmaf(-d.x, t, 1.0f));
    q.y = fmaf(q.x, q.y, fmaf(n.y, t, u));
    return q;
}
static inline lw_f2 lw_dfscale(lw_f2 d, float s) { return lw_mk(d.x * s, d.y * s); }
static inline lw_f2 lw_dfnormalize(lw_f2 t) { lw_f2 s; s.x = t.x + t.y; s.y = t.x - s.x + t.y; return s; }
static lw_f2 lw_logkf(float d) {
    int o = d < 1.17549435e-38f;
    if (o) d = d * (float)(1LL << 32) * (float)(1LL << 32);
    int e = ((lw_f2i(d * (1.0f / 0.75f)) >> 23) & 0xff) - 0x7f;
    float m = lw_i2f(lw_f2i(d) + ((-e) << 23));
    if (o) e -= 64;
    lw_f2 x = lw_dfdiv(lw_dfadd2_f_f(-1.0f, m), lw_dfadd2_f_f(1.0f, m));
    lw_f2 x2 = lw_dfsqu(x);
    float t = 0.240320354700088500976562f;
    t = fmaf(t, x2.x, 0.285112679004669189453125f);
    t = fmaf(t, x2.x, 0.400007992982864379882812f);
    lw_f2 c = lw_mk(0.66666662693023681640625f, 3.69183861259614332084311e-09f);
    lw_f2 s = lw_dfmul_f2_f(lw_mk(0.69314718246459960938f, -1.904654323148236017e-09f), (float)e);
    s = lw_dfadd_f2_f2(s, lw_dfscale(x, 2.0f));
    s = lw_dfadd_f2_f2(s, lw_dfmul_f2_f2(lw_dfmul_f2_f2(x2, x), lw_dfadd2_f2_f2(lw_dfmul_f2_f(x2, t), c)));
    return s;
}
static float lw_ldexpkf(float x, int q) {
    int m = q >> 31;
    m = (((m + q) >> 6) - m) << 4;
    q = q - (m << 2);
    m += 127; m = m < 0 ? 0 : m; m = m > 255 ? 255 : m;
    float u = lw_i2f(m << 23);
    x = x * u * u * u * u;
    u = lw_i2f((q + 0x7f) << 23);
    return x * u;
}
static float lw_expkf(lw_f2 d) {
    float u = (d.x + d.y) * 1.442695040888963407359924681001892137426645954152985934135449406931f;
    int q = (int)rintf(u);
    lw_f2 s = lw_dfadd2_f2_f(d, (float)q * -0.693145751953125f);
    s = lw_dfadd2_f2_f(s, (float)q * -1.428606765330187045e-06f);
    s = lw_dfnormalize(s);
    float t = 0.00136324646882712841033936f;
    t = fmaf(t, s.x, 0.00836596917361021041870117f);
    t = fmaf(t, s.x, 0.0416710823774337768554688f);
    t = fmaf(t, s.x, 0.166665524244308471679688f);
    t = fmaf(t, s.x, 0.499999850988388061523438f);
    lw_f2 tt = lw_dfadd_f2_f2(s, lw_dfmul_f2_f(lw_dfsqu(s), t));
    tt = lw_dfadd_f_f2(1.0f, tt);
    u = tt.x + tt.y;
    u = lw_ldexpkf(u, q);
    if (d.x < -104.0f) u = 0.0f;
    return u;
}
static float lw_sleef_powf(float x, float y) {
    return lw_expkf(lw_dfmul_f2_f(lw_logkf(fabsf(x)), y));
}
static float torch_sum_small(const float* x, int n) {
    auto strided = [](const float* v, int stride, int size) { float a = 0.0f; for (int i = 0; i < size; ++i) a += v[i * stride]; return a; };
    if (n < 8) {
        const int n4 = n / 4;
        float p[4];
        for (int k = 0; k < 4; ++k) p[k] = strided(x + k, 4, n4);
        for (int i = n4 * 4; i < n; ++i) p[0] += x[i];
        for (int k = 1; k < 4; ++k) p[0] += p[k];
        return 0.0f + p[0];
    }
    const int nv = n / 8, nv4 = nv / 4;
    float fin = 0.0f;
    for (int k = nv * 8; k < n; ++k) fin += x[k];
    for (int lane = 0; lane < 8; ++lane) {
        float p[4];
        for (int k = 0; k < 4; ++k) p[k] = strided(x + k * 8 + lane, 32, nv4);
        for (int i = nv4 * 4; i < nv; ++i) p[0] += x[i * 8 + lane];
        for (int k = 1; k < 4; ++k) p[0] += p[k];
        fin += p[0];
    }
    return 0.0f + fin;
}
}

extern "C" int cvx_label_weights_host(const int64_t* hist_fix_host, const int64_t* hist_mov_host, int max_label,
                                      int* present_host, float* weights_host) {
    int C = 0;
    for (int l = 0; l <= max_label; ++l)
        if (hist_fix_host[l] + hist_mov_host[l] > 0) present_host[C++] = l;
    for (int c = 0; c < C; ++c) {
        const float cnt = (float)(hist_fix_host[present_host[c]] + hist_mov_host[present_host[c]]) + 1e-32f;
        const int blk = options().label_pow_block > 0 ? (int)options().label_pow_block : 32;
        const float pw = c < (C / blk) * blk ? lw_sleef_powf(cnt, 0.3f) : (float)pow((double)cnt, 0.3);
        weights_host[c] = 1.0f / pw;
    }
    const float mean = torch_sum_small(weights_host, C) / (float)C;
    for (int c = 0; c < C; ++c) weights_host[c] = weights_host[c] / mean;
    return C;
}

extern "C" int cvx_label_features_f32(const float* lab, int64_t V, int C, const int* present, const float* weights,
                                      float mult, float* feat, void* stream) {
    CVX_REQUIRE(lab && present && weights && feat && V > 0 && C > 0, "cvx_label_features_f32: bad arguments");
    hipLaunchKernelGGL(k_label_features, dim3((unsigned)cdiv64(V, 256)), dim3(256), 0, as_stream(stream), lab, V, C, present,
                       weights, mult, feat);
    return check_last("label_features");
}


namespace cvx {
__global__ __launch_bounds__(256) void k_round_f16(float* __restrict__ x, int64_t n) {
    const int64_t i = (int64_t)blockIdx.x * blockDim.x + threadIdx.x;
    if (i < n) x[i] = __half2float(__float2half_rn(x[i]));
}
}
extern "C" int cvx_round_f16_f32(float* x, int64_t n, void* stream) {
    CVX_REQUIRE(x && n >= 0, "cvx_round_f16_f32: bad arguments");
    if (n > 0) hipLaunchKernelGGL(cvx::k_round_f16, dim3((unsigned)cvx::cdiv64(n, 256)), dim3(256), 0, cvx::as_stream(stream), x, n);
    return cvx::check_last("round_f16");
}


namespace cvx {
__global__ __launch_bounds__(256) void k_pack_field_f64(const float* __restrict__ f, size_t V, int quantize, double* __restrict__ out) {
    __shared__ float sv[768];
    const size_t p0 = (size_t)blockIdx.x * 256, p = p0 + threadIdx.x;
    if (p < V) {
        float a = f[p], b = f[V + p], c = f[2 * V + p];
        if (quantize == 1) { a = __half2float(__float2half_rn(a)); b = __half2float(__float2half_rn(b)); c = __half2float(__float2half_rn(c)); }
        sv[3 * threadIdx.x] = a; sv[3 * threadIdx.x + 1] = b; sv[3 * threadIdx.x + 2] = c;
    }
    cvx_barrier();
    const size_t n = min((size_t)768, 3 * (V - p0));
    double* o = out + 3 * p0;
#pragma unroll
    for (int r = 0; r < 3; ++r) {
        const unsigned i = threadIdx.x + 256 * r;
        if (i < n) o[i] = (double)sv[i];
    }
}
}
extern "C" int cvx_pack_field_f64(const float* field, int H, int W, int D, int quantize, double* out, void* stream) {
    CVX_REQUIRE(field && out && H > 0 && W > 0 && D > 0, "cvx_pack_field_f64: bad arguments");
    CVX_REQUIRE(quantize == 0 || quantize == 1, "cvx_pack_field_f64: quantize must be 0 (float32) or 1 (float16)");
    const size_t V = (size_t)H * W * D;
    hipLaunchKernelGGL(cvx::k_pack_field_f64, dim3((unsigned)cvx::cdiv64((int64_t)V, 256)), dim3(256), 0, cvx::as_stream(stream), field, V, quantize, out);
    return cvx::check_last("pack_field");
}
```

Baseline: 152.2.

## Fold certification arming, resolve/commit, IC prepare and IC finish into neighbouring kernels

Adds a default-on pair_front option under which several small kernel launches are merged into neighbours. The pair-setup kernel now arms the certification key/sec/count words, so k_cert_arm is skipped. The finalize kernel resolves flagged voxels in-wave, so the separate resolve launch goes away. Eval commits winners through a per-voxel countdown, replacing the commit kernel, and the gather kernel writes the IC-prepared fields so k_ic_prepare is skipped. The IC finish scaling is folded into the first resize pass. This cuts launch count and extra passes over volumes, at the cost of more complex atomic countdown logic, heavier finalize kernels with 40-entry register arrays, and ordering subtleties.

```diff
diff --git a/convexadam_amd/csrc/certify.hip b/convexadam_amd/csrc/certify.hip
--- a/convexadam_amd/csrc/certify.hip
+++ b/convexadam_amd/csrc/certify.hip
@@ -167,21 +167,93 @@
     }
 }
 
+template <bool RESOLVE>
 __global__ __launch_bounds__(256) void k_cert_plain_finalize(CertArgs A) {
+    __shared__ float smem[RESOLVE ? 4 : 1][RESOLVE ? 160 : 1];
     const CertProb& P = A.p[blockIdx.y];
     const size_t v = (size_t)A.g.h * A.g.w * A.g.d;
     const size_t x = (size_t)blockIdx.x * blockDim.x + threadIdx.x;
-    if (x >= v) return;
-    const unsigned long long key = P.key[x];
-    const unsigned b1 = (unsigned)(key >> 32), b2 = P.sec[x];
-    const int k1 = (int)(unsigned)(key & 0xffffffffull);
-    const float s1 = b1 == 0u ? __uint_as_float(0x7fc00000u) : from_ordered_bits(b1);
-    P.smin[x] = s1;
-    P.idx0[x] = k1;
-    if (P.argmin_out) P.argmin_out[x] = k1;
-    bool certain = b1 == 0u || b2 == 0xffffffffu;
-    if (!certain && b2 != 0u) certain = s1 == 0.0f || cert_lower(from_ordered_bits(b2)) > cert_upper(s1);
-    if (!certain) P.list[atomicAdd(&P.counts[0], 1)] = (unsigned)x;
+    if (!RESOLVE && x >= v) return;
+    bool certain = true;
+    float s1 = 0.0f;
+    if (x < v) {
+        const unsigned long long key = P.key[x];
+        const unsigned b1 = (unsigned)(key >> 32), b2 = P.sec[x];
+        const int k1 = (int)(unsigned)(key & 0xffffffffull);
+        s1 = b1 == 0u ? __uint_as_float(0x7fc00000u) : from_ordered_bits(b1);
+        P.smin[x] = s1;
+        certain = b1 == 0u || b2 == 0xffffffffu;
+        if (!certain && b2 != 0u) certain = s1 == 0.0f || cert_lower(from_ordered_bits(b2)) > cert_upper(s1);
+        if (!RESOLVE || certain) {
+            P.idx0[x] = k1;
+            if (P.argmin_out) P.argmin_out[x] = k1;
+        }
+        if (!certain) P.list[atomicAdd(&P.counts[0], 1)] = (unsigned)x;
+    }
+    if (!RESOLVE) return;
+    const int K = A.g.K, lane = threadIdx.x & 63;
+    float* sm = smem[threadIdx.x >> 6];
+    const float INF = __uint_as_float(0x7f800000u);
+    constexpr int NL = 40;
+    for (unsigned long long flagged = __ballot(!certain); flagged; flagged &= flagged - 1) {
+        const int fl = __ffsll((long long)flagged) - 1;
+        const unsigned xf = (unsigned)__shfl((int)(unsigned)x, fl);
+        const float U = cert_upper(__shfl(s1, fl));
+        const float* col = P.ssdu + xf;
+        unsigned long long bestkey = ~0ull;
+        int appended = 0;
+        for (int kb = 0; kb < K; kb += 64 * NL) {
+            float s[NL];
+            unsigned long long over = 0ull;
+#pragma unroll
+            for (int i = 0; i < NL; ++i) { const int k = kb + 64 * i + lane; s[i] = k < K ? col[(size_t)k * v] : INF; }
+#pragma unroll
+            for (int i = 0; i < NL; ++i) {
+                if (kb + 64 * i >= K) break;
+                const unsigned long long mz = __ballot(s[i] == 0.0f);
+                if (mz) {
+                    const unsigned long long key = pack_min_key(0.0f, (unsigned)(kb + 64 * i + __ffsll((long long)mz) - 1));
+                    bestkey = key < bestkey ? key : bestkey;
+                }
+                const bool mine = kb + 64 * i + lane < K && s[i] != 0.0f && cert_lower(s[i]) <= U;
+                const unsigned long long m = __ballot(mine);
+                if (m) {
+                    const int nm = __popcll(m);
+                    int base = 0;
+                    if (lane == 0) base = atomicAdd(&P.counts[8], nm);
+                    base = __shfl(base, 0);
+                    const int slot = base + __popcll(m & ((1ull << lane) - 1ull));
+                    const bool listed = mine && (unsigned)slot < P.work_cap;
+                    if (listed) P.work[slot] = ((unsigned long long)xf << 32) | (unsigned)(kb + 64 * i + lane);
+                    appended += __popcll(__ballot(listed));
+                    if (mine && !listed) over |= 1ull << i;
+                }
+            }
+            if (__ballot(over != 0ull)) {
+#pragma unroll 1
+                for (int i = 0; i < NL; ++i) {
+                    unsigned long long rest = __ballot(((over >> i) & 1ull) != 0ull);
+                    while (rest) {
+                        const int l = __ffsll((long long)rest) - 1;
+                        rest &= rest - 1;
+                        const int kk = kb + 64 * i + l;
+                        const float ex = cert_exact_entry_wave(A.g, P, kk, (int)xf, sm, lane);
+                        const unsigned long long key = pack_min_key(ex, (unsigned)kk);
+                        bestkey = key < bestkey ? key : bestkey;
+                    }
+                }
+            }
+        }
+        if (lane == 0) {
+            P.key[xf] = bestkey;
+            P.sec[xf] = (unsigned)appended;
+            if (appended == 0) {
+                const int kw = (int)(unsigned)(bestkey & 0xffffffffull);
+                P.idx0[xf] = kw;
+                if (P.argmin_out) P.argmin_out[xf] = kw;
+            }
+        }
+    }
 }
 
 __global__ __launch_bounds__(64) void k_cert_plain_resolve(CertArgs A) {
@@ -230,6 +302,7 @@
         if (lane == 0) P.key[x] = bestkey;
     }
 }
+template <bool COMMIT>
 __global__ __launch_bounds__(256) void k_cert_plain_eval(CertArgs A) {
     __shared__ float smem[4][160];
     const CertProb& P = A.p[blockIdx.y];
@@ -240,7 +313,18 @@
         const unsigned x = (unsigned)(it >> 32);
         const int kk = (int)(unsigned)(it & 0xffffffffull);
         const float ex = cert_exact_entry_wave(A.g, P, kk, (int)x, smem[wv], lane);
-        if (lane == 0) atomicMin(&P.key[x], pack_min_key(ex, (unsigned)kk));
+        if (lane == 0) {
+            atomicMin(&P.key[x], pack_min_key(ex, (unsigned)kk));
+            if (COMMIT) {
+                __threadfence();
+                if (atomicSub(&P.sec[x], 1u) == 1u) {
+                    __threadfence();
+                    const int kw = (int)(unsigned)(__hip_atomic_load(&P.key[x], __ATOMIC_RELAXED, __HIP_MEMORY_SCOPE_AGENT) & 0xffffffffull);
+                    P.idx0[x] = kw;
+                    if (P.argmin_out) P.argmin_out[x] = kw;
+                }
+            }
+        }
     }
 }
 __global__ __launch_bounds__(256) void k_cert_plain_commit(CertArgs A) {
@@ -517,7 +601,7 @@
     }
 }
 
-__global__ __launch_bounds__(256) void k_cert_gather(CertArgs A) {
+__global__ __launch_bounds__(256) void k_cert_gather(CertArgs A, float* __restrict__ prep0, float* __restrict__ prep1) {
     const CertProb& P = A.p[blockIdx.y];
     const size_t v = (size_t)A.g.h * A.g.w * A.g.d;
     const size_t i = (size_t)blockIdx.x * blockDim.x + threadIdx.x;
@@ -528,6 +612,11 @@
     float o0, o1, o2;
     cert_smooth_winner(prev, M, A.g.h, A.g.w, A.g.d, i, o0, o1, o2);
     P.u[i] = o0; P.u[v + i] = o1; P.u[2 * v + i] = o2;
+    float* prep = blockIdx.y ? prep1 : prep0;
+    if (prep) {
+        const float sc[3] = {(float)(A.g.h - 1) / 2.0f, (float)(A.g.w - 1) / 2.0f, (float)(A.g.d - 1) / 2.0f};
+        prep[i] = fdiv(o2, sc[2]); prep[v + i] = fdiv(o1, sc[1]); prep[2 * v + i] = fdiv(o0, sc[0]);
+    }
 }
 
 __global__ __launch_bounds__(256) void k_cert_arm(CertArgs A, int nprob) {
@@ -575,10 +664,10 @@
     return CertProb{ssdu, fix, mov, c.tail, c.key, c.sec, c.idx0, c.idxA, c.idxB, c.smin, c.list, c.counts, c.work, c.work_cap, c.rec, u, argmin_out};
 }
 
-static void cert_arm(CertArgs& A, int nprob, hipStream_t s) {
+static void cert_arm(CertArgs& A, int nprob, hipStream_t s, bool armed = false) {
     const CertGeo& g = A.g;
     const size_t v = (size_t)g.h * g.w * g.d;
-    hipLaunchKernelGGL(k_cert_arm, dim3((unsigned)cdiv64((int64_t)(v > 16 ? v : 16), 256)), dim3(256), 0, s, A, nprob);
+    if (!armed) hipLaunchKernelGGL(k_cert_arm, dim3((unsigned)cdiv64((int64_t)(v > 16 ? v : 16), 256)), dim3(256), 0, s, A, nprob);
     for (int q = 0; q < nprob; ++q)
         if (g.ntail > 0) launch_corr_tail_compact(A.p[q].fix, A.p[q].mov, g.C, g.h, g.w, g.d, g.hw, 0, const_cast<float*>(A.p[q].tail), s);
 }
@@ -599,9 +688,14 @@
 }
 static int cert_finish(CertArgs& A, int nprob, hipStream_t s) {
     const size_t v = (size_t)A.g.h * A.g.w * A.g.d;
-    hipLaunchKernelGGL(k_cert_plain_finalize, dim3((unsigned)cdiv64((int64_t)v, 256), nprob), dim3(256), 0, s, A);
+    if (options().pair_front != 0) {
+        hipLaunchKernelGGL(k_cert_plain_finalize<true>, dim3((unsigned)cdiv64((int64_t)v, 256), nprob), dim3(256), 0, s, A);
+        hipLaunchKernelGGL(k_cert_plain_eval<true>, dim3(256, nprob), dim3(256), 0, s, A);
+        return check_last("certified argmin");
+    }
+    hipLaunchKernelGGL(k_cert_plain_finalize<false>, dim3((unsigned)cdiv64((int64_t)v, 256), nprob), dim3(256), 0, s, A);
     hipLaunchKernelGGL(k_cert_plain_resolve, dim3(256, nprob), dim3(64), 0, s, A);
-    hipLaunchKernelGGL(k_cert_plain_eval, dim3(256, nprob), dim3(256), 0, s, A);
+    hipLaunchKernelGGL(k_cert_plain_eval<false>, dim3(256, nprob), dim3(256), 0, s, A);
     hipLaunchKernelGGL(k_cert_plain_commit, dim3(8, nprob), dim3(256), 0, s, A);
     return check_last("certified argmin");
 }
@@ -623,9 +717,15 @@
     return cert_plain(A, 1, true, s);
 }
 
+CertArmWords cert_arm_words(void* workspace, int h, int w, int d, int hw) {
+    Carver cv(workspace);
+    const CertCarve c = cert_layout(cv, h, w, d, hw, false);
+    return CertArmWords{c.key, c.sec, c.counts};
+}
+
 int coupled_convex_cert_impl(const float* ssduA, const float* fixA, const float* movA, float* outA, void* wsA, const float* ssduB, const float* fixB,
                              const float* movB, float* outB, void* wsB, const float* mesh, int C, int h, int w, int d, int hw, size_t workspace_bytes,
-                             hipStream_t s, int stage) {
+                             hipStream_t s, int stage, const CertFront& front) {
     if (workspace_bytes < corr_certify_workspace_bytes(C, h, w, d, hw, false)) return fail(CVX_ERR_WORKSPACE, "certified coupled convex: workspace too small");
     const int nprob = ssduB ? 2 : 1;
     CertArgs A{};
@@ -636,7 +736,7 @@
     A.p[0] = cert_prob(ssduA, fixA, movA, ca, outA, nullptr);
     A.p[1] = A.p[0];
     if (ssduB) { const CertCarve cb = cert_layout(cvb, h, w, d, hw, false); A.p[1] = cert_prob(ssduB, fixB, movB, cb, outB, nullptr); }
-    if (stage == 1) { cert_arm(A, nprob, s); return check_last("certified argmin"); }
+    if (stage == 1) { cert_arm(A, nprob, s, front.armed); return check_last("certified argmin"); }
     if (stage == 2) { cert_stream(A, 0, 1, s); return check_last("certified argmin"); }
     if (stage == 3) { if (nprob > 1) cert_stream(A, 1, 1, s); return check_last("certified argmin"); }
     if (stage == 4) return cert_finish(A, nprob, s);
@@ -658,7 +758,7 @@
         }
     }
     A.pass = 7;
-    hipLaunchKernelGGL(k_cert_gather, dim3((unsigned)cdiv64((int64_t)v, 256), nprob), dim3(256), 0, s, A);
+    hipLaunchKernelGGL(k_cert_gather, dim3((unsigned)cdiv64((int64_t)v, 256), nprob), dim3(256), 0, s, A, front.prepA, nprob > 1 ? front.prepB : nullptr);
     return check_last("certified coupled convex");
 }
 
diff --git a/convexadam_amd/csrc/correlate.hip b/convexadam_amd/csrc/correlate.hip
--- a/convexadam_amd/csrc/correlate.hip
+++ b/convexadam_amd/csrc/correlate.hip
@@ -374,3 +374,15 @@
     if (argmin) return launch_argmin(ssd, false, nullptr, nullptr, 0.0f, false, (int)K, (size_t)h * w * d, r.keys, argmin, s);
     return CVX_OK;
 }
+
+extern "C" __attribute__((visibility("default"))) int cvx_test_correlate_cert_counters(int C, int h, int w, int d, int disp_hw, void* workspace,
+                                                                                           int* counts_host, void* stream) {
+    CVX_REQUIRE(workspace && counts_host && C > 0 && h > 0 && w > 0 && d > 0 && disp_hw >= 0 && disp_hw <= CVX_MAX_DISP_HW, "cvx_test_correlate_cert_counters: bad arguments");
+    Carver cv(workspace);
+    const PartsWs c = certified_layout(cv, C, h, w, d, disp_hw);
+    const int* counts = cert_arm_words(c.b, h, w, d, disp_hw).counts;
+    hipStream_t s = as_stream(stream);
+    if (hipStreamSynchronize(s) != hipSuccess || hipMemcpy(counts_host, counts, 16 * sizeof(int), hipMemcpyDeviceToHost) != hipSuccess)
+        return check_last("cvx_test_correlate_cert_counters");
+    return CVX_OK;
+}
diff --git a/convexadam_amd/csrc/cvx_common.h b/convexadam_amd/csrc/cvx_common.h
--- a/convexadam_amd/csrc/cvx_common.h
+++ b/convexadam_amd/csrc/cvx_common.h
@@ -91,7 +91,8 @@
     X(box_tile_sync,       "CVX_BOX_TILE_SYNC",         0)   \
     X(box_prediv,          "CVX_BOX_PREDIV",            1)   \
     X(tile_census_ptr,     nullptr,                     0)   \
-    X(adam_wt,             "CVX_ADAM_WT",               1)
+    X(adam_wt,             "CVX_ADAM_WT",               1)   \
+    X(pair_front,          "CVX_PAIR_FRONT",            1)
 #define X(name, env, dflt) long long name;
 struct Options { CVX_OPTIONS(X) };
 #undef X
@@ -342,7 +343,7 @@
 int launch_resize(const float* in, int C, int h, int w, int d, float* out, int H, int W, int D, float pre_mul,
                   float post_div, hipStream_t s);
 int launch_resize2(const float* in, int C, int h, int w, int d, int H, int W, int D, float* scratch, float* out, int h2, int w2,
-                   int d2, float post_div, hipStream_t s);
+                   int d2, float post_div, hipStream_t s, float ic_finish_gs = 0.0f);
 struct AdamConsts { float w1, b2, omb2; ConstDiv bc2s; float neg_step; const unsigned* sqrt_tbl; };
 __device__ __forceinline__ float adam_sqrt(float x, const unsigned* __restrict__ tbl) {
     float r = fsqrt(x);
@@ -443,9 +444,12 @@
 size_t corr_certify_workspace_bytes(int C, int h, int w, int d, int hw, bool plain = false);
 int corr_certified_argmin(const float* ssdu, const float* fix, const float* mov, int C, int h, int w, int d, int hw, int64_t* argmin,
                           void* workspace, size_t workspace_bytes, hipStream_t s);
+struct CertFront { bool armed = false; float* prepA = nullptr; float* prepB = nullptr; };
+struct CertArmWords { unsigned long long* key; unsigned* sec; int* counts; };
+CertArmWords cert_arm_words(void* workspace, int h, int w, int d, int hw);
 int coupled_convex_cert_impl(const float* ssduA, const float* fixA, const float* movA, float* outA, void* wsA, const float* ssduB, const float* fixB,
                              const float* movB, float* outB, void* wsB, const float* mesh, int C, int h, int w, int d, int hw, size_t workspace_bytes,
-                             hipStream_t s, int stage = 0);
+                             hipStream_t s, int stage = 0, const CertFront& front = CertFront{});
 bool box3_march_supported(int d);
 int launch_box3_march(const float* in, float* out, int h, int w, int d, bool backward, float* P, float* m, float* v,
                       AdamConsts ac, float* gsave, hipStream_t s);
diff --git a/convexadam_amd/csrc/pipeline.hip b/convexadam_amd/csrc/pipeline.hip
--- a/convexadam_amd/csrc/pipeline.hip
+++ b/convexadam_amd/csrc/pipeline.hip
@@ -33,7 +33,8 @@
     BaseTables t;
     int hw; float* mesh;
     unsigned long long* keys[2]; size_t v;
-    int* counts[2];
+    unsigned* sec[2];
+    int* counts[2]; int ncounts;
     float4* zero[2]; size_t nzero4;
 };
 __global__ __launch_bounds__(256) void k_pair_setup(PairSetup a) {
@@ -55,7 +56,8 @@
 #pragma unroll
     for (int q = 0; q < 2; ++q) {
         if (a.keys[q]) for (size_t x = gid; x < a.v; x += gsz) a.keys[q][x] = ~0ull;
-        if (a.counts[q] && gid < 2) a.counts[q][gid] = 0;
+        if (a.sec[q]) for (size_t x = gid; x < a.v; x += gsz) a.sec[q][x] = 0xffffffffu;
+        if (a.counts[q] && gid < (size_t)a.ncounts) a.counts[q][gid] = 0;
         if (a.zero[q]) for (size_t i = gid; i < a.nzero4; i += gsz) a.zero[q][i] = make_float4(0.f, 0.f, 0.f, 0.f);
     }
 }
@@ -270,12 +272,12 @@
 
 struct IcScratch { float *in1, *in2, *ic1, *ic2; void* ws; size_t ws_bytes; };
 static int ic_tail(const float* soft, const float* soft2, int h, int w, int d, int iters, const float* bh, const float* bw, const float* bd,
-                   const IcScratch& t, float gs, float* dst, hipStream_t s) {
+                   const IcScratch& t, float gs, float* dst, hipStream_t s, bool prepared = false) {
     const dim3 gv((unsigned)cdiv64((int64_t)h * w * d, 256));
-    hipLaunchKernelGGL(k_ic_prepare, dim3(gv.x, 2), dim3(256), 0, s, soft, soft2, h, w, d, t.in1, t.in2);
+    if (!prepared) hipLaunchKernelGGL(k_ic_prepare, dim3(gv.x, 2), dim3(256), 0, s, soft, soft2, h, w, d, t.in1, t.in2);
     const int rc = cvx_inverse_consistency_f32(t.in1, t.in2, h, w, d, iters, bh, bw, bd, t.ic1, t.ic2, t.ws, t.ws_bytes, s);
     if (rc) return rc;
-    hipLaunchKernelGGL(k_ic_finish, gv, dim3(256), 0, s, t.ic1, h, w, d, gs, dst);
+    if (dst) hipLaunchKernelGGL(k_ic_finish, gv, dim3(256), 0, s, t.ic1, h, w, d, gs, dst);
     return CVX_OK;
 }
 
@@ -292,7 +294,16 @@
     bool pooled_mind = false, mind_records = false;
     CoupledWs cw1{}, cw2{};
 
+    bool front = false;
+    bool cert_armed = false;
+    bool ic_prepared = false;
+    bool ic_unfinished = false;
+
     bool pooled() const { return pooled_mind || labels != nullptr; }
+    CorrPlan plan() const {
+        const bool variant = p->cost || p->n_box == 1 || p->corr_fast || f16();
+        return corr_plan(L.C, L.h, L.w, L.d, p->disp_hw, CorrUse{variant, p->ic != 0, no_prune()});
+    }
     bool no_prune() const { return options().no_prune != 0; }
     bool f16() const { return p->fp16_storage != 0; }
     float* F(size_t off) const { return reinterpret_cast<float*>(ws + off); }
@@ -345,9 +356,15 @@
         const bool zero_state = adam_tables && (3 * L.V2) % 4 == 0;
         PairSetup a = {{{L.h, L.w, L.d, L.h2, L.w2, L.d2},
                         {F(L.bh), F(L.bw), F(L.bd), adam_tables ? F(L.bh2) : nullptr, adam_tables ? F(L.bw2) : nullptr, adam_tables ? F(L.bd2) : nullptr}},
-                       p->disp_hw, F(L.mesh), {cw1.keys[0], cw2.keys[0]}, L.v,
-                       {no_prune() ? nullptr : cw1.counts, no_prune() ? nullptr : cw2.counts},
+                       p->disp_hw, F(L.mesh), {cw1.keys[0], cw2.keys[0]}, L.v, {nullptr, nullptr},
+                       {no_prune() ? nullptr : cw1.counts, no_prune() ? nullptr : cw2.counts}, 2,
                        {zero_state ? reinterpret_cast<float4*>(ws + L.m) : nullptr, zero_state ? reinterpret_cast<float4*>(ws + L.v_) : nullptr}, 3 * L.V2 / 4};
+        if (front && plan().pair_cert) {
+            const CertArmWords c1 = cert_arm_words(ws + L.cert_ws, L.h, L.w, L.d, p->disp_hw);
+            const CertArmWords c2 = p->ic ? cert_arm_words(ws + L.cert_ws2, L.h, L.w, L.d, p->disp_hw) : CertArmWords{nullptr, nullptr, nullptr};
+            a.keys[0] = c1.key; a.keys[1] = c2.key; a.sec[0] = c1.sec; a.sec[1] = c2.sec; a.counts[0] = c1.counts; a.counts[1] = c2.counts; a.ncounts = 16;
+            cert_armed = true;
+        }
         hipLaunchKernelGGL(k_pair_setup, dim3(zero_state ? 1024 : 64), dim3(256), 0, s, a);
         if (adam_tables && !zero_state) {
             (void)hipMemsetAsync(F(L.m), 0, sizeof(float) * 3 * L.V2, s);
@@ -375,12 +392,14 @@
         if (p->fp16_storage) {
             if ((rc = cvx_round_f16_f32(F(L.fs), (int64_t)L.C * L.v, s)) || (rc = cvx_round_f16_f32(F(L.ms), (int64_t)L.C * L.v, s))) return rc;
         }
-        const CorrPlan plan = corr_plan(L.C, L.h, L.w, L.d, p->disp_hw, CorrUse{variant, p->ic != 0, no_prune()});
+        const CorrPlan plan = this->plan();
         if (plan.pair_cert) {
+            const CertFront cf = {cert_armed, front && p->ic ? F(L.in1) : nullptr, front && p->ic ? F(L.in2) : nullptr};
+            ic_prepared = cf.prepA != nullptr;
             const size_t fws = corr_certfast_workspace_bytes(L.C, L.h, L.w, L.d, p->disp_hw), qws = corr_certify_workspace_bytes(L.C, L.h, L.w, L.d, p->disp_hw);
             auto cert_stage = [&](int stage) {
                 return coupled_convex_cert_impl(F(L.ssd), F(L.fs), F(L.ms), F(L.soft), ws + L.cert_ws, p->ic ? F(L.ssd2) : nullptr, F(L.ms), F(L.fs),
-                                                p->ic ? F(L.soft2) : nullptr, p->ic ? ws + L.cert_ws2 : nullptr, F(L.mesh), L.C, L.h, L.w, L.d, p->disp_hw, qws, s, stage);
+                                                p->ic ? F(L.soft2) : nullptr, p->ic ? ws + L.cert_ws2 : nullptr, F(L.mesh), L.C, L.h, L.w, L.d, p->disp_hw, qws, s, stage, cf);
             };
             if ((rc = cert_stage(1))) return rc;
             if ((rc = launch_corr_certfast(F(L.fs), F(L.ms), L.C, L.h, L.w, L.d, p->disp_hw, F(L.ssd), ws + L.corr_ws, fws, s))) return rc;
@@ -426,7 +445,8 @@
             if ((rc = cvx_avgpool_f32(featF, L.C, p->H, p->W, p->D, p->grid_sp_adam, F(L.F2), s))) return rc;
             if ((rc = cvx_avgpool_f32(featM, L.C, p->H, p->W, p->D, p->grid_sp_adam, F(L.M2), s))) return rc;
         }
-        if (p->ic) rc = launch_resize2(F(L.upin), 3, L.h, L.w, L.d, p->H, p->W, p->D, F(L.disp_hr), F(L.P), L.h2, L.w2, L.d2, (float)p->grid_sp_adam, s);
+        if (p->ic) rc = launch_resize2(ic_unfinished ? F(L.ic1) : F(L.upin), 3, L.h, L.w, L.d, p->H, p->W, p->D, F(L.disp_hr), F(L.P), L.h2, L.w2, L.d2, (float)p->grid_sp_adam, s,
+                                       ic_unfinished ? (float)p->grid_sp : 0.0f);
         else rc = launch_resize(F(L.soft), 3, L.h, L.w, L.d, F(L.P), L.h2, L.w2, L.d2, 1.0f, (float)p->grid_sp_adam, s);
         if (rc) return rc;
         mark("adam_setup", s);
@@ -470,6 +490,7 @@
     struct HookReset { ~HookReset() { corr_fused_set_prep_hook(nullptr); } } hook_reset;
 
     PairRun run = {p, L, static_cast<char*>(workspace), s, feat_fixed, feat_moving, labels};
+    run.front = options().pair_front != 0;
     const bool adam = p->lambda_weight > 0;
     if ((rc = run.features(img_fixed, img_moving))) return rc;
     run.setup();
@@ -477,8 +498,9 @@
     if ((rc = run.convex())) return rc;
     mark("coupled_convex", s);
     if (p->ic) {
+        run.ic_unfinished = run.front && adam;
         const IcScratch t = {run.F(L.in1), run.F(L.in2), run.F(L.ic1), run.F(L.ic2), run.ws + L.ic_ws, cvx_inverse_consistency_workspace_bytes(L.h, L.w, L.d)};
-        if ((rc = ic_tail(run.F(L.soft), run.F(L.soft2), L.h, L.w, L.d, 15, run.F(L.bh), run.F(L.bw), run.F(L.bd), t, (float)p->grid_sp, run.F(L.upin), s))) return rc;
+        if ((rc = ic_tail(run.F(L.soft), run.F(L.soft2), L.h, L.w, L.d, 15, run.F(L.bh), run.F(L.bw), run.F(L.bd), t, (float)p->grid_sp, run.ic_unfinished ? nullptr : run.F(L.upin), s, run.ic_prepared))) return rc;
         if (!adam && (rc = launch_resize(run.F(L.upin), 3, L.h, L.w, L.d, out_field, p->H, p->W, p->D, 1.0f, 1.0f, s))) return rc;
         mark("inverse_consistency", s);
     }
diff --git a/convexadam_amd/csrc/pool.hip b/convexadam_amd/csrc/pool.hip
--- a/convexadam_amd/csrc/pool.hip
+++ b/convexadam_amd/csrc/pool.hip
@@ -408,9 +408,9 @@
     return check_last("resize_trilinear");
 }
 
-template <int CT>
+template <int CT, bool FIN = false>
 __global__ __launch_bounds__(256) void k_resize_yx(const float* __restrict__ in, int C, int h, int w, int d, float* __restrict__ T,
-                                                   int W, int D) {
+                                                   int W, int D, float fin_gs = 1.0f) {
     const int x = (int)(blockIdx.x * blockDim.x + threadIdx.x), y = (int)blockIdx.y, z = (int)blockIdx.z;
     if (x >= D) return;
     const size_t n = (size_t)h * W * D;
@@ -420,10 +420,16 @@
     lin_coef(y, w, W, y0, y1, ly0, ly1);
     lin_coef(x, d, D, x0, x1, lx0, lx1);
     auto one = [&](int c) {
-        const float* r0 = in + (((size_t)c * h + z) * w + y0) * d;
-        const float* r1 = in + (((size_t)c * h + z) * w + y1) * d;
-        const float a = __builtin_fmaf(r0[x0], lx0, r0[x1] * lx1);
-        const float b = __builtin_fmaf(r1[x0], lx0, r1[x1] * lx1);
+        const int cs = FIN ? 2 - c : c;
+        const float* r0 = in + (((size_t)cs * h + z) * w + y0) * d;
+        const float* r1 = in + (((size_t)cs * h + z) * w + y1) * d;
+        float t00 = r0[x0], t01 = r0[x1], t10 = r1[x0], t11 = r1[x1];
+        if (FIN) {
+            const float sc = (float)((c == 0 ? h : (c == 1 ? w : d)) - 1) / 2.0f;
+            t00 = (t00 * sc) * fin_gs; t01 = (t01 * sc) * fin_gs; t10 = (t10 * sc) * fin_gs; t11 = (t11 * sc) * fin_gs;
+        }
+        const float a = __builtin_fmaf(t00, lx0, t01 * lx1);
+        const float b = __builtin_fmaf(t10, lx0, t11 * lx1);
         T[(size_t)c * n + i] = __builtin_fmaf(a, ly0, b * ly1);
     };
     if (CT > 0) {
@@ -494,15 +500,17 @@
         for (int c = 0; c < C; ++c) one(c);
 }
 int launch_resize2(const float* in, int C, int h, int w, int d, int H, int W, int D, float* scratch, float* out, int h2, int w2, int d2,
-                   float post_div, hipStream_t s) {
+                   float post_div, hipStream_t s, float ic_finish_gs) {
     if (W > 65535 || h > 65535 || w2 > 65535 || h2 > 65535) return fail(CVX_ERR_UNSUPPORTED, "resize_trilinear2: extent exceeds the grid limits");
     auto bx = [](int n) { return n > 128 ? 256 : (n > 64 ? 128 : 64); };
     const dim3 g1((unsigned)cdiv(D, bx(D)), (unsigned)W, (unsigned)h), g2((unsigned)cdiv(d2, bx(d2)), (unsigned)w2, (unsigned)h2);
+    if (ic_finish_gs > 0.0f && C != 3) return fail(CVX_ERR_UNSUPPORTED, "resize_trilinear2: the folded inverse-consistency finish is a 3-channel field's");
     if (C == 3) {
-        hipLaunchKernelGGL(k_resize_yx<3>, g1, dim3(bx(D)), 0, s, in, C, h, w, d, scratch, W, D);
+        if (ic_finish_gs > 0.0f) hipLaunchKernelGGL((k_resize_yx<3, true>), g1, dim3(bx(D)), 0, s, in, C, h, w, d, scratch, W, D, ic_finish_gs);
+        else hipLaunchKernelGGL((k_resize_yx<3, false>), g1, dim3(bx(D)), 0, s, in, C, h, w, d, scratch, W, D, 1.0f);
         hipLaunchKernelGGL(k_resize2<3>, g2, dim3(bx(d2)), 0, s, scratch, C, h, H, W, D, out, h2, w2, d2, post_div);
     } else {
-        hipLaunchKernelGGL(k_resize_yx<0>, g1, dim3(bx(D)), 0, s, in, C, h, w, d, scratch, W, D);
+        hipLaunchKernelGGL((k_resize_yx<0, false>), g1, dim3(bx(D)), 0, s, in, C, h, w, d, scratch, W, D, 1.0f);
         hipLaunchKernelGGL(k_resize2<0>, g2, dim3(bx(d2)), 0, s, scratch, C, h, H, W, D, out, h2, w2, d2, post_div);
     }
     return check_last("resize_trilinear2");
```

Result: no change. 153.0 (median of 6 runs) (+0.5%).
